# zjc263/GPU_SDR

Measured on AMD Instinct MI355X. Metric: IQ Msamples/s ingested (one synthetic 200 Msps stream per GPU), higher is better.
Workload: dtype f32 (f16 hi/lo-split MFMA, f32 accumulate)

## Files before the change

### gpu_sdr_amd/csrc/ddc_kernels.h

```cpp
#pragma once
#include <hip/hip_runtime.h>

#include <vector>

#include "dev_owner.h"

#ifndef GSDR_NO_PK
#define GSDR_NO_PK __attribute__((target("no-packed-fp32-ops")))
#endif

namespace gsdr {

struct Switches {
    bool ddc_mfma = true;
    bool ddc_few = true;
    bool ddc_pipe = true;
    int ddc_k = -1;
    int ddc_waves = 0;
    int ddc_nch = 0;
    unsigned ddc_lds = 0;
    int ddc_prefetch = 1;
    bool ddc_autotune = true;
    int mfma_asm = 4;
    int mfma_tt = 1;
    int mfma_pk = 32;
    int mfma_w = 4;
    int mfma_rt = 0;
    bool mfma_w8 = true;
    int mfma_prec = -1;
    int mfma_3m = -1;
    int mfma_3m_rot = -1;
    int mfma_fold = -1;
    int mfma_timing = 0;
    bool noise_fft = true;
    bool tones_fft = true;
    bool pfb_lds = true;
    int pfb_bluestein = -1;
    int pfb_cu = -1;
    bool pfb_direct = true;
    int pfb_col = -1;
    int pfb_cu_nt = 0;
    bool pfb_teams = true;
    bool pfb_radix8 = true;
    int pfb_fr = 0;
    int pfb_wide = -1;
    int mix_few = 32;
    bool chirp_split = true;
    bool pipe_queues = true;
    bool pipe_overlap = true;
    int pipe_streams = 3;
};
Switches read_switches();

struct DdcShape {
    int N;
    int Npad;
    int TW;
    int M;
    int nblk;
    int nch;
    int cbase, crem;
    int g_off;
    unsigned rate;
    unsigned long long idx0;
    unsigned long long rate_magic;
    double inv_rate;
    unsigned m_mod_rate;
    long long total;
    long long xlast;
    int prefetch;
};

struct DdcLaunch {
    const float2 *x;
    const float *taps_t;
    const float *taps_p;
    const float2 *btab;
    const double2 *wk;
    const double2 *wrem;
    const unsigned *fmod;
    float2 *out;
    float2 *tails;
    int tails_nch;
    const float2 *carry_in;
    float2 *carry_out;
    DdcShape sh;
    unsigned lds_bytes;
    bool pipe;
    bool few;
};

hipError_t launch_ddc(int F, int K, const DdcLaunch &a, hipStream_t st, hipEvent_t stop);
const char *ddc_few_kernel_name();
hipError_t launch_mix(int K, const DdcLaunch &a, int mix_few, hipStream_t st);

hipError_t launch_ddc_flat_main(int F, int PK, const DdcLaunch &a, hipStream_t st);
const char *ddc_kernel_name();
const char *ddc_flat_kernel_name();
const char *mix_kernel_name(int n_tones, int tw, long long total, int K, int mix_few);
hipError_t launch_widen_sc16(const void *in, float2 *out, long long n, float scale, int cus, hipStream_t st);
hipError_t launch_narrow_sc16(const float2 *in, void *out, long long n, float gain, unsigned long long *clipped, int cus,
                              hipStream_t st);

struct MfmaShape {
    int N;
    int NT32;
    int ntg;
    int ntq;
    int ngt;
    int M;
    int MF;
    int F;
    int nk8;
    int nout;
    int woff;
    int carry_len;
    long long tail0;
    long long nx;
    unsigned rate;
    unsigned long long rate_magic;
    double inv_rate;
    unsigned m_mod_rate;
    unsigned idx_base;
    int seg_k;
    float unscale;
    int rt;
    int timing_mode;
};

struct MfmaLaunch {
    const float2 *x;
    const float2 *head;
    const float2 *tail;
    const float *taps;
    const uint4 *bfrag;
    const float2 *ptab;
    const float2 *dtab;
    const unsigned *fmod;
    const unsigned *segmax;
    float2 *out;
    const uint4 *img;
    const uint4 *bfrag3;
    const float4 *ptab3;
    MfmaShape sh;
};

struct MfmaPlan {
    int TT, PK;
    int ntg, nk8, MF, M;
    unsigned rate;
    bool x16;
};

void mfma_build_tables(const MfmaPlan &pl, const std::vector<unsigned> &fmod_in, const float *window,
                       std::vector<uint4> &bfrag, std::vector<float2> &ptab,
                       std::vector<float2> &dtab, std::vector<float> &taps,
                       std::vector<unsigned> &fmod, float &unscale);
void mfma_build_tables3(const MfmaPlan &pl, int span, const std::vector<unsigned> &fmod, std::vector<uint4> &bfrag3,
                        std::vector<float4> &ptab3);
void mfma_build_tables3f(const MfmaPlan &pl, const std::vector<unsigned> &fmod, std::vector<uint4> &bfrag3,
                         std::vector<float4> &ptab3);
struct StageLaunch {
    const float2 *x;
    long long n;
    const float2 *b;
    long long nb;
    float2 *b_dst;
    unsigned *seg, *seg_clear;
    int nseg_alloc;
    long long seg_len;
    float2 *head_cur;
    long long head_n;
    float2 *head_next;
    int carry_len;
    float2 *tail;
    long long tail0;
};
hipError_t launch_absmax(const StageLaunch &s, hipStream_t st);
enum class MfmaKernel { AsmRing, Cxx, AsmRing16, AsmRing16W8, AsmRing16P, AsmRing16P3, AsmRing16P3R2, AsmRing16P3F };
hipError_t launch_ddc_mfma(MfmaKernel kind, int TT, int PK, int W, const MfmaLaunch &a, hipStream_t st);
const char *ddc_mfma_kernel_name(MfmaKernel kind);

struct FftPlan {
    int n = 0;
    int m = 0;
    int n_radices = 0;
    int radices[32] = {};
    DevBuf<float2> d_tw;
    DevBuf<float2> d_chirp;
    DevBuf<float2> d_bhat;
};
int fft_plan_build(FftPlan &pl, int n);
hipError_t fft_forward(const FftPlan &pl, float2 *src, float2 *dst, float2 *tmp, int batch, hipStream_t st);
hipError_t launch_pfb_filter(const float2 *raw, const float *window, int nfft, int avg, int frames_n, float2 *frames,
                             hipStream_t st);
hipError_t launch_pfb_select(const float2 *spectra, int nfft, int frames_n, const int *sel, int n_out, float2 *out, hipStream_t st);
hipError_t launch_pfb_average(const float2 *frames, long long n_frames, int n_ch, int k, int kind, int count, const float2 *acc_in,
                              float2 *acc_out, float2 *out, hipStream_t st);
const char *fft_kernel_name();
constexpr int kPfbLdsMaxN = 8192;
constexpr int kPfbLdsMaxPrime = 127;
constexpr int kPfbLdsTwMaxN = 4096;
constexpr int kPfbLdsMaxBytes = (2 * kPfbLdsMaxN + kPfbLdsMaxPrime + 1) * 8;
int pfb_lds_plan(int n, int *radices16, bool radix8);
hipError_t launch_pfb_lds(const float2 *carry, int new_0, const float2 *in, const float *window, const float2 *tw,
                          int nfft, int avg, int frames_n, const int *sel, int n_out, float2 *out,
                          float2 *carry_out, int spare_begin, int spare_n, long long window_len, hipStream_t st,
                          const FftPlan *blue, const Switches &sw, const char **kernel);
bool pfb_cu_fits(int nfft, int avg, int len, const Switches &sw);
struct PfbChoice {
    bool cu;
    int threads;
    int G;
    int twl;
    size_t lds;
    int b_off, b_len, col, direct, dir_s, dir_gs, teams;
};
PfbChoice pfb_choose(int nfft, int avg, const FftPlan *blue, int frames_n, int n_out, int cus, const Switches &sw);
const char *pfb_kernel_name(const PfbChoice &c);

struct ChirpShape {
    unsigned long long num_steps, length, period;
    unsigned chirpness;
    int f0;
};

hipError_t launch_chirp_demod(const float2 *in, float2 *out, long long n,
                              unsigned long long index0, const ChirpShape &cs, hipStream_t st);
hipError_t launch_chirp_lockin(const float2 *carry, int carry_len, const float2 *in,
                               const float *profile, int ppt, int valid, float2 *out,
                               unsigned long long index0, const ChirpShape &cs, hipStream_t st,
                               bool split, float2 *partial, int partial_cap);
hipError_t launch_warm(hipStream_t st);
hipError_t launch_tones_synth(float2 *out, long long n, unsigned long long start, unsigned rate, const unsigned *fmod,
                              const float2 *q0, const float2 *btab, const float2 *ctab, int n_tones, hipStream_t st);
hipError_t launch_tones_synth_sc16(void *out, long long n, unsigned long long start, unsigned rate, const unsigned *fmod,
                                   const float2 *q0, const float2 *btab, const float2 *ctab, int n_tones, float gain,
                                   unsigned long long *clipped, hipStream_t st);
const char *chirp_demod_kernel_name();
const char *chirp_lockin_kernel_name();

hipError_t launch_source_tones(float2 *out, long long n, long long start, unsigned rate,
                               const unsigned *fmod_dev, const float *ampl_dev,
                               const float *phase_dev, int n_tones, float sigma,
                               unsigned long long seed, hipStream_t st);
hipError_t launch_source_chirp(float2 *out, long long n, unsigned long long index0,
                               const ChirpShape &cs, float scale, hipStream_t st);
hipError_t launch_source_chirp_sc16(void *out, long long n, unsigned long long index0, const ChirpShape &cs, float scale,
                                    float gain, unsigned long long *clipped, hipStream_t st);

}
```

### gpu_sdr_amd/csrc/ddc_mfma.hip

```cpp
#include <cmath>
#include <cstdlib>
#include <type_traits>
#include <vector>

#include "ddc_device.h"
#include "ddc_mfma_ring_gen.h"
#include "ddc_mfma_ring16_gen.h"
#include "ddc_mfma_ring16w8_gen.h"
#include "ddc_mfma_ring16p_gen.h"
#include "ddc_mfma_ring16p3_gen.h"
#include "ddc_mfma_ring16p3r2_gen.h"
#include "ddc_mfma_ring16p3f_gen.h"

namespace gsdr {

typedef _Float16 half2v __attribute__((ext_vector_type(2)));
typedef _Float16 half4v __attribute__((ext_vector_type(4)));
typedef _Float16 half8 __attribute__((ext_vector_type(8)));
typedef float float2v __attribute__((ext_vector_type(2)));
typedef float float4u __attribute__((ext_vector_type(4), aligned(8)));
typedef float float4v __attribute__((ext_vector_type(4)));
typedef float float16v __attribute__((ext_vector_type(16)));

namespace {

struct Frag {
    half8 hi, lo;
};

__device__ __forceinline__ float mul_legacy(float x, float h) {
    float r;
    asm("v_mul_legacy_f32 %0, %1, %2" : "=v"(r) : "v"(x), "v"(h));
    return r;
}

__device__ __forceinline__ void split_pair(float xr, float xi, float hs, half2v &hi, half2v &lo) {
#pragma clang fp contract(off)
    const float2v v = {mul_legacy(xr, hs), mul_legacy(xi, hs)};
    hi = __builtin_convertvector(v, half2v);
    const float2v res = v - __builtin_convertvector(hi, float2v);
    lo = __builtin_convertvector(res, half2v);
}

__device__ __forceinline__ Frag make_frag(const float4v xa, const float4v xb, const float4v hs) {
    half2v h0, h1, h2, h3, l0, l1, l2, l3;
    split_pair(xa.x, xa.y, hs.x, h0, l0);
    split_pair(xa.z, xa.w, hs.y, h1, l1);
    split_pair(xb.x, xb.y, hs.z, h2, l2);
    split_pair(xb.z, xb.w, hs.w, h3, l3);
    Frag f;
    const half4v ha = __builtin_shufflevector(h0, h1, 0, 1, 2, 3);
    const half4v hb = __builtin_shufflevector(h2, h3, 0, 1, 2, 3);
    const half4v la = __builtin_shufflevector(l0, l1, 0, 1, 2, 3);
    const half4v lb = __builtin_shufflevector(l2, l3, 0, 1, 2, 3);
    f.hi = __builtin_shufflevector(ha, hb, 0, 1, 2, 3, 4, 5, 6, 7);
    f.lo = __builtin_shufflevector(la, lb, 0, 1, 2, 3, 4, 5, 6, 7);
    return f;
}

}

__device__ __forceinline__ float bits_to_float(unsigned u) { return __builtin_bit_cast(float, u); }
__device__ __forceinline__ unsigned float_to_bits(float f) { return __builtin_bit_cast(unsigned, f); }
__device__ __forceinline__ void workgroup_sync() {
    __builtin_amdgcn_fence(__ATOMIC_RELEASE, "workgroup");
    __builtin_amdgcn_s_barrier();
    __builtin_amdgcn_fence(__ATOMIC_ACQUIRE, "workgroup");
}
__device__ __forceinline__ unsigned lane_xor(unsigned v, int d) {
    const int lane = (int)__builtin_amdgcn_mbcnt_hi(~0u, __builtin_amdgcn_mbcnt_lo(~0u, 0u));
    return (unsigned)__builtin_amdgcn_ds_bpermute((lane ^ d) << 2, (int)v);
}

__device__ __forceinline__ unsigned fresh_tid() {
    unsigned tid = threadIdx.x;
    asm volatile("" : "+v"(tid));
    return tid;
}
#define GSDR_SGPR(v) "s"(__builtin_amdgcn_readfirstlane((int)(v)))
#define GSDR_SGPR_PAIR(name, v) [name##_lo] GSDR_SGPR((unsigned)(v)), [name##_hi] GSDR_SGPR((unsigned)((v) >> 32))

#ifdef GSDR_TIMING_BUILD
__device__ __forceinline__ bool timing_no_stores(const MfmaShape &sh) { return (sh.timing_mode & 1) != 0; }
__device__ __forceinline__ bool timing_one_block(const MfmaShape &sh) { return (sh.timing_mode & 2) != 0; }
#else
__device__ __forceinline__ bool timing_no_stores(const MfmaShape &) { return false; }
__device__ __forceinline__ bool timing_one_block(const MfmaShape &) { return false; }
#endif

#ifdef GSDR_STAMP_BUILD
__device__ unsigned long long *g_stamp_buf = nullptr;
__device__ __forceinline__ void stamp(int slot) {
    if (g_stamp_buf && threadIdx.x == 0) {
        unsigned long long t = __builtin_amdgcn_s_memrealtime();
        if (slot == 2) {
            unsigned xcc, hwid;
            asm volatile("s_getreg_b32 %0, hwreg(HW_REG_XCC_ID)" : "=s"(xcc));
            asm volatile("s_getreg_b32 %0, hwreg(HW_REG_HW_ID)" : "=s"(hwid));
            t = (xcc & 0xfu) | ((unsigned long long)hwid << 8);
        }
        g_stamp_buf[8 * (size_t)blockIdx.x + slot] = t;
    }
}
#else
__device__ __forceinline__ void stamp(int) {}
#endif

__device__ __forceinline__ unsigned wave_max_u32(unsigned v) {
    int x = (int)v;
#define GSDR_DPP_MAX(ctrl, row_mask)                                                          \
    {                                                                                         \
        const unsigned o = (unsigned)__builtin_amdgcn_update_dpp(0, x, ctrl, row_mask, 0xf, false); \
        x = (int)((unsigned)x > o ? (unsigned)x : o);                                         \
    }
    GSDR_DPP_MAX(0xB1, 0xf);
    GSDR_DPP_MAX(0x4E, 0xf);
    GSDR_DPP_MAX(0x141, 0xf);
    GSDR_DPP_MAX(0x140, 0xf);
    GSDR_DPP_MAX(0x142, 0xa);
    GSDR_DPP_MAX(0x143, 0xc);
#undef GSDR_DPP_MAX
    return (unsigned)__builtin_amdgcn_readlane(x, 63);
}

__device__ __forceinline__ void row_segments(const MfmaShape &sh, int o, int &q0, int &q1) {
    const int oc = o < sh.nout ? o : sh.nout - 1;
    q0 = oc;
    q1 = oc + sh.F - 1;
    if (sh.seg_k > 1) {
        q0 /= sh.seg_k;
        q1 /= sh.seg_k;
    }
}
__device__ __forceinline__ unsigned row_max_bits(const MfmaLaunch &a, int o) {
    int q0, q1;
    row_segments(a.sh, o, q0, q1);
    const int span = q1 - q0;
    unsigned v[8];
#pragma unroll
    for (int i = 0; i < 8; ++i) v[i] = a.segmax[q0 + (i < span ? i : span)];
    unsigned m = 0;
#pragma unroll
    for (int i = 0; i < 8; ++i) m = m > v[i] ? m : v[i];
    return m;
}
__device__ __forceinline__ int scale_exp_of(unsigned m) {
    int se = 140 - (int)((m >> 23) & 0xffu);
    return se > 100 ? 100 : (se < -100 ? -100 : se);
}
__device__ __forceinline__ int row_scale_exp(const MfmaLaunch &a, int o) { return scale_exp_of(row_max_bits(a, o)); }
constexpr int kScaleFromTable = 0x7fffffff;
__device__ __forceinline__ float exp2_bits(int e) { return __builtin_bit_cast(float, (unsigned)(127 + e) << 23); }

__device__ __forceinline__ float2 tile_phasor(const MfmaLaunch &a, int gt, unsigned fm) {
    const MfmaShape &sh = a.sh;
    const unsigned long long s_tile = mod_rate(
        (unsigned long long)sh.idx_base + (unsigned long long)(gt * 32) * sh.m_mod_rate, sh.rate, sh.rate_magic);
    const unsigned long long ph = mod_rate((unsigned long long)fm * s_tile, sh.rate, sh.rate_magic);
    double bre, bim;
    exact_phasor(ph, sh.inv_rate, bre, bim);
    return make_float2((float)bre, (float)bim);
}

__device__ __forceinline__ void store_tile(const MfmaLaunch &a, int gt, int n, int hh, int se_self,
                                           const float16v &accr, const float16v &acci) {
    const MfmaShape &sh = a.sh;
    const int Np = sh.NT32 * 32;
    const unsigned fm = a.fmod[n];
    float2 d[16];
#pragma unroll
    for (int i = 0; i < 16; ++i) d[i] = a.dtab[(size_t)((i & 3) + 8 * (i >> 2) + 4 * hh) * Np + n];
    asm volatile("" ::: "memory");
    const float2 base = tile_phasor(a, gt, fm);
#pragma unroll
    for (int i = 0; i < 16; ++i) {
        const int row = (i & 3) + 8 * (i >> 2) + 4 * hh;
        const int se = __builtin_amdgcn_ds_bpermute(row << 2, se_self);
        const float inv = exp2_bits(-se) * sh.unscale;
        const float dx = d[i].x * inv, dy = d[i].y * inv;
        const float rr = base.x * dx - base.y * dy, ri = base.x * dy + base.y * dx;
        float2 y;
        y.x = accr[i] * rr - acci[i] * ri;
        y.y = accr[i] * ri + acci[i] * rr;
        const int orow = gt * 32 + row;
        if (orow < sh.nout && n < sh.N) a.out[(size_t)orow * sh.N + n] = y;
    }
}

template <int TT>
__device__ __forceinline__ void store_rows(const MfmaLaunch &a, int gt, int n0, int hh, int se_self,
                                           const float16v (&accr)[TT], const float16v (&acci)[TT]) {
#pragma unroll
    for (int tt = 0; tt < TT; ++tt) {
        const int n = n0 + tt * 32;
        store_tile(a, gt, n, hh, se_self, accr[tt], acci[tt]);
    }
}

__device__ __forceinline__ void wg_barrier() {
    asm volatile("s_waitcnt lgkmcnt(0)\n\ts_barrier" ::: "memory");
}

template <int TT, int PK, int W>
__global__ __launch_bounds__(64 * W, TT == 1 ? 2 : 1) void ddc_mfma_kernel(const MfmaLaunch a) {
    constexpr int KS = PK / 8;
    constexpr int SPW = KS / W;
    static_assert(KS % W == 0 && SPW >= 1, "every wave produces whole k-steps");
    __shared__ uint4 ring[2][KS][2][64];
    const MfmaShape &sh = a.sh;
    const int lane = threadIdx.x & 63;
    const int wave = __builtin_amdgcn_readfirstlane((int)(threadIdx.x >> 6));
    const int r = lane & 31, hh = lane >> 5;
    const int xcd = blockIdx.x & 7, q = blockIdx.x >> 3;
    const int gt = (q / sh.ntq) * 8 + xcd;
    if (gt >= sh.ngt) return;
    const int tg_raw = (q % sh.ntq) * W + wave;
    const bool active = tg_raw < sh.ntg;
    const int tg = active ? tg_raw : sh.ntg - 1;

    half8 Bf[TT][KS][2][2];
#pragma unroll
    for (int tt = 0; tt < TT; ++tt)
#pragma unroll
        for (int ks = 0; ks < KS; ++ks)
#pragma unroll
            for (int c = 0; c < 2; ++c)
#pragma unroll
                for (int sp = 0; sp < 2; ++sp) {
                    const size_t at = ((((size_t)(tg * TT + tt) * KS + ks) * 2 + c) * 2 + sp) * 64 + lane;
                    const uint4 v = a.bfrag[at];
                    Bf[tt][ks][c][sp] = __builtin_bit_cast(half8, v);
                }

    const int o = gt * 32 + r;
    const int se = row_scale_exp(a, o);
    const float S = exp2_bits(se);
    const int oc = o < sh.nout ? o : sh.nout - 1;
    const float2 *xbase = gt == 0 ? a.head + sh.carry_len
                                  : (gt == sh.ngt - 1 ? a.tail - sh.tail0 : a.x);
    const float2 *xrow = xbase + ((long long)(oc + sh.woff) * sh.M + 4 * hh);
    const float *tp = a.taps + 4 * hh;

    const int nhi = (sh.nk8 + KS - 1) / KS;
    float4v xa[SPW], xb[SPW], hv[SPW];
    auto gload = [&](int blk) {
        const int bc = blk < nhi ? blk : nhi - 1;
#pragma unroll
        for (int j = 0; j < SPW; ++j) {
            const int k = bc * KS + wave + j * W;
            hv[j] = *reinterpret_cast<const float4v *>(tp + 8 * k);
            const float4u *p = reinterpret_cast<const float4u *>(xrow + 8 * k);
            xa[j] = p[0];
            xb[j] = p[1];
        }
    };
    auto produce = [&](int slot) {
#pragma unroll
        for (int j = 0; j < SPW; ++j) {
            const int ks = wave + j * W;
            const Frag f = make_frag(xa[j], xb[j], hv[j] * S);
            ring[slot][ks][0][lane] = __builtin_bit_cast(uint4, f.hi);
            ring[slot][ks][1][lane] = __builtin_bit_cast(uint4, f.lo);
        }
    };

    float16v accr[TT], acci[TT];
#pragma unroll
    for (int tt = 0; tt < TT; ++tt)
#pragma unroll
        for (int i = 0; i < 16; ++i) accr[tt][i] = acci[tt][i] = 0.f;

    const int Np = sh.NT32 * 32;
    const int n0 = tg * TT * 32 + r;
    const float2 *pp = a.ptab + n0;

    gload(0);
    produce(0);
    gload(1);
    for (int hi = 0; hi < nhi; ++hi) {
        const int slot = hi & 1;
        wg_barrier();
        half8 fh[KS], fl[KS];
#pragma unroll
        for (int ks = 0; ks < KS; ++ks) {
            fh[ks] = __builtin_bit_cast(half8, ring[slot][ks][0][lane]);
            fl[ks] = __builtin_bit_cast(half8, ring[slot][ks][1][lane]);
        }
        float2 P[TT];
#pragma unroll
        for (int tt = 0; tt < TT; ++tt) P[tt] = pp[(size_t)hi * Np + tt * 32];
        produce(slot ^ 1);
        gload(hi + 2);
        __builtin_amdgcn_sched_barrier(0);
        float16v Cr[TT], Ci[TT];
#pragma unroll
        for (int ks = 0; ks < KS; ++ks) {
            const float16v zero = {0};
#pragma unroll
            for (int tt = 0; tt < TT; ++tt) {
                float16v cr = ks == 0 ? zero : Cr[tt], ci = ks == 0 ? zero : Ci[tt];
                cr = __builtin_amdgcn_mfma_f32_32x32x16_f16(fh[ks], Bf[tt][ks][0][0], cr, 0, 0, 0);
                ci = __builtin_amdgcn_mfma_f32_32x32x16_f16(fh[ks], Bf[tt][ks][1][0], ci, 0, 0, 0);
                cr = __builtin_amdgcn_mfma_f32_32x32x16_f16(fh[ks], Bf[tt][ks][0][1], cr, 0, 0, 0);
                ci = __builtin_amdgcn_mfma_f32_32x32x16_f16(fh[ks], Bf[tt][ks][1][1], ci, 0, 0, 0);
                cr = __builtin_amdgcn_mfma_f32_32x32x16_f16(fl[ks], Bf[tt][ks][0][0], cr, 0, 0, 0);
                ci = __builtin_amdgcn_mfma_f32_32x32x16_f16(fl[ks], Bf[tt][ks][1][0], ci, 0, 0, 0);
                Cr[tt] = cr;
                Ci[tt] = ci;
            }
        }
        __builtin_amdgcn_sched_barrier(0);
        asm volatile("s_nop 15\n\ts_nop 15");
        __builtin_amdgcn_sched_barrier(0);
#pragma unroll
        for (int tt = 0; tt < TT; ++tt)
// ... 204 lines not shown
                 :
                 : [xo] "v"(xo), [to] "v"(to), [po] "v"(po), [bo] "v"(bo), [lane16] "v"(rd16), [wr16] "v"(wr16),
                   [accaddr] "v"(accaddr), GSDR_SGPR_PAIR(xb, xb), GSDR_SGPR_PAIR(tp, tpb), GSDR_SGPR_PAIR(pp, ppb),
                   GSDR_SGPR_PAIR(bf, bfb), [pstride] GSDR_SGPR((unsigned)Np * 8u), [nhi] GSDR_SGPR(nhi),
                   [first] GSDR_SGPR(first), [sgo] "v"(sgo), [sgn] "v"(sgn), [seaddr] "v"(seaddr),
                   GSDR_SGPR_PAIR(sg, sgb)
                 : GSDR_MFMA_RING16_CLOBBERS);
    stamp(3);
    if (active && !timing_no_stores(sh)) {
        const unsigned tid2 = fresh_tid();
        const int lane2 = (int)(tid2 & 63u);
        ring16_epilogue(a, lds, gt, tg, wave, lane2, (int)(lds_scale[tid2] >> 23) - 127);
    }
}

__global__ __launch_bounds__(256, 2) __attribute__((target("no-packed-fp32-ops"))) void ddc_mfma_ring16_kernel(
    const MfmaLaunch a) {
    constexpr int W = 4;
    __shared__ uint4 lds[2048];
    __shared__ unsigned lds_scale[256];
    static_assert(sizeof(uint4) * 2048 >= GSDR_MFMA_RING16_BYTES, "ring fits");
    const MfmaShape &sh = a.sh;
    const int wave = __builtin_amdgcn_readfirstlane((int)(threadIdx.x >> 6));
    const int xcd = blockIdx.x & 7, q = blockIdx.x >> 3;
    const int rt = sh.rt > 1 ? 2 : 1;
    const int gt0 = (q / sh.ntq) * rt * 8 + xcd;
    if (gt0 >= sh.ngt) return;
    const int tg_raw = (q % sh.ntq) * W + wave;
    const bool active = tg_raw < sh.ntg;
    const int tg = active ? tg_raw : sh.ntg - 1;
    stamp(0);
    stamp(2);
    ring16_tile(a, lds, lds_scale, gt0, 1, tg, wave, active);
    if (rt > 1 && gt0 + 8 < sh.ngt) {
        workgroup_sync();
        ring16_tile(a, lds, lds_scale, gt0 + 8, 0, tg, wave, active);
    }
    stamp(1);
}

#ifdef GSDR_STAMP_BUILD
extern "C" int gsdr_debug_set_stamp_buffer(void *dev_ptr) {
    unsigned long long *p = (unsigned long long *)dev_ptr;
    return hipMemcpyToSymbol(HIP_SYMBOL(g_stamp_buf), &p, sizeof(p)) == hipSuccess ? 0 : -1;
}
#endif

__global__ __launch_bounds__(512, 2) __attribute__((target("no-packed-fp32-ops"))) void ddc_mfma_ring16w8_kernel(
    const MfmaLaunch a) {
    constexpr int KS = 4, W = 8;
    __shared__ uint4 lds[4096];
    __shared__ unsigned lds_scale[512];
    static_assert(sizeof(uint4) * 4096 >= GSDR_MFMA_RING16W8_BYTES, "ring fits");
    const MfmaShape &sh = a.sh;
    const int wave = __builtin_amdgcn_readfirstlane((int)(threadIdx.x >> 6));
    const int ntq8 = (sh.ntg + W - 1) / W;
    const int xcd = blockIdx.x & 7, q = blockIdx.x >> 3;
    const int gt = (q / ntq8) * 8 + xcd;
    if (gt >= sh.ngt) return;
    stamp(0);
    stamp(2);
    const int tg_raw = (q % ntq8) * W + wave;
    const bool active = tg_raw < sh.ntg;
    const int tg = active ? tg_raw : sh.ntg - 1;
    const int Np = sh.NT32 * 32;
    const int nhi = timing_one_block(sh) ? 1 : (sh.nk8 + KS - 1) / KS;
    const unsigned tid = fresh_tid();
    const int lane = (int)(tid & 63u);
    const int r = lane & 31, hh = lane >> 5;
    const int kw = wave & 3;
    int q0, q1;
    row_segments(sh, gt * 32 + r, q0, q1);
    const unsigned sgo = (unsigned)q0 * 4u, sgn = (unsigned)(q1 - q0);
    const unsigned long long sgb = (unsigned long long)a.segmax;
    const unsigned seaddr = (unsigned)(unsigned long long)(__attribute__((address_space(3))) char *)lds_scale + tid * 4u;
    const unsigned to = (unsigned)((4 * hh + 8 * kw) * 4);
    const unsigned po = (unsigned)(tg * 32 + (lane & 15)) * 8u;
    const unsigned bo = (unsigned)tg * (KS * 4 * 1024u) + (unsigned)lane * 16u;
    const unsigned lds_base = (unsigned)(unsigned long long)(__attribute__((address_space(3))) char *)lds;
    const unsigned rd16 = lds_base + (unsigned)(lane >> 5) * 2048u + (unsigned)(lane & 15) * 16u +
                          (unsigned)((lane >> 4) & 1) * 512u;
    const unsigned wr16 = lds_base + (unsigned)lane * 16u + (unsigned)kw * 2048u;
    const unsigned accaddr = lds_base + (unsigned)wave * 8192u + (unsigned)lane * 16u;
    const unsigned long long tpb = (unsigned long long)a.taps, ppb = (unsigned long long)a.ptab,
                             bfb = (unsigned long long)a.bfrag;
    const int o = gt * 32 + r;
    const int oc = o < sh.nout ? o : sh.nout - 1;
    const float2 *xbase;
    long long xshift;
    if (gt == 0) {
        xbase = a.head;
        xshift = sh.carry_len;
    } else if (gt == sh.ngt - 1) {
        xbase = a.tail;
        xshift = -sh.tail0;
    } else {
        xbase = a.x;
        xshift = 0;
    }
    const unsigned xo = (unsigned)((((long long)(oc + sh.woff) * sh.M + xshift) + 4 * hh + 8 * kw) * 8);
    const unsigned long long xb = (unsigned long long)xbase;
    asm volatile(GSDR_MFMA_RING16W8_TEXT
                 :
                 : [xo] "v"(xo), [to] "v"(to), [po] "v"(po), [bo] "v"(bo), [lane16] "v"(rd16), [wr16] "v"(wr16),
                   [accaddr] "v"(accaddr), GSDR_SGPR_PAIR(xb, xb), GSDR_SGPR_PAIR(tp, tpb), GSDR_SGPR_PAIR(pp, ppb),
                   GSDR_SGPR_PAIR(bf, bfb), [pstride] GSDR_SGPR((unsigned)Np * 8u), [nhi] GSDR_SGPR(nhi),
                   [role] GSDR_SGPR(wave >> 2), [sgo] "v"(sgo), [sgn] "v"(sgn), [seaddr] "v"(seaddr),
                   GSDR_SGPR_PAIR(sg, sgb)
                 : GSDR_MFMA_RING16W8_CLOBBERS);
    if (active && !timing_no_stores(sh)) {
        const unsigned tid2 = fresh_tid();
        const int lane2 = (int)(tid2 & 63u);
        const int se_self = (int)(lds_scale[tid2] >> 23) - 127;
        float16v accr, acci;
        const float4v *acc = reinterpret_cast<const float4v *>(lds) + wave * 512 + lane2;
#pragma unroll
        for (int qd = 0; qd < 4; ++qd) {
            const float4v vr = acc[qd * 64], vi = acc[(qd + 4) * 64];
#pragma unroll
            for (int j = 0; j < 4; ++j) {
                accr[qd * 4 + j] = vr[j];
                acci[qd * 4 + j] = vi[j];
            }
        }
        store_tile16(a, gt, tg, lane2, se_self, accr, acci);
    }
    stamp(1);
}

__global__ __launch_bounds__(256) __attribute__((target("no-packed-fp32-ops"))) void ddc_convert_kernel(const MfmaLaunch a, uint4 *__restrict__ img, int nhi) {
    const MfmaShape &sh = a.sh;
    const int lane = threadIdx.x & 63, wave = threadIdx.x >> 6;
    const int r = lane & 31, hh = lane >> 5;
    const int gt = blockIdx.x / nhi, blk = blockIdx.x - gt * nhi;
    const int o = gt * 32 + r;
    const float S = exp2_bits(row_scale_exp(a, o));
    const int oc = o < sh.nout ? o : sh.nout - 1;
    const float2 *xbase = gt == 0 ? a.head + sh.carry_len : (gt == sh.ngt - 1 ? a.tail - sh.tail0 : a.x);
    const int k = blk * 4 + wave;
    const float4u *px = reinterpret_cast<const float4u *>(xbase + ((long long)(oc + sh.woff) * sh.M + 4 * hh + 8 * k));
    const float4v xa = px[0], xb = px[1];
    const float4v hv = *reinterpret_cast<const float4v *>(a.taps + 8 * k + 4 * hh);
    const Frag f = make_frag(xa, xb, hv * S);
    uint4 *dst = img + ((size_t)blockIdx.x * 8 + 2 * wave) * 64 + lane;
    dst[0] = __builtin_bit_cast(uint4, f.hi);
    dst[64] = __builtin_bit_cast(uint4, f.lo);
}

__device__ __forceinline__ __attribute__((target("no-packed-fp32-ops"))) void ring16p_tile(
    const MfmaLaunch &a, uint4 *lds, int gt, int first, int tg, int wave, bool active) {
    constexpr int KS = 4;
    const MfmaShape &sh = a.sh;
    const int Np = sh.NT32 * 32;
    const int nhi = (sh.nk8 + KS - 1) / KS;
    const int lane = (int)(fresh_tid() & 63u);
    const unsigned po = (unsigned)(tg * 32 + (lane & 15)) * 8u;
    const unsigned bo = (unsigned)tg * (KS * 4 * 1024u) + (unsigned)lane * 16u;
    const unsigned lds_base = (unsigned)(unsigned long long)(__attribute__((address_space(3))) char *)lds;
    const unsigned rd16 = lds_base + (unsigned)(lane >> 5) * 2048u + (unsigned)(lane & 15) * 16u +
                          (unsigned)((lane >> 4) & 1) * 512u;
    const unsigned io_hi = (unsigned)wave * 2048u + (unsigned)lane * 16u, io_lo = io_hi + 1024u;
    const unsigned wrs = lds_base + (unsigned)wave * 2048u;
    const unsigned accaddr = lds_base + (unsigned)wave * 8192u + (unsigned)lane * 16u;
    const unsigned long long ibb = (unsigned long long)(a.img + (size_t)gt * nhi * 512), ppb = (unsigned long long)a.ptab,
                             bfb = (unsigned long long)a.bfrag;
    asm volatile(GSDR_MFMA_RING16P_TEXT
                 :
                 : [io_hi] "v"(io_hi), [io_lo] "v"(io_lo), [po] "v"(po), [bo] "v"(bo), [lane16] "v"(rd16),
                   [accaddr] "v"(accaddr), GSDR_SGPR_PAIR(ib, ibb), [wrs] GSDR_SGPR(wrs), GSDR_SGPR_PAIR(pp, ppb),
                   GSDR_SGPR_PAIR(bf, bfb), [pstride] GSDR_SGPR((unsigned)Np * 8u), [nhi] GSDR_SGPR(nhi),
                   [first] GSDR_SGPR(first)
                 : GSDR_MFMA_RING16P_CLOBBERS);
    if (active) ring16_epilogue(a, lds, gt, tg, wave, (int)(fresh_tid() & 63u), kScaleFromTable);
}

__global__ __launch_bounds__(256, 2) __attribute__((target("no-packed-fp32-ops"))) void ddc_mfma_ring16p_kernel(
    const MfmaLaunch a) {
    constexpr int W = 4;
    __shared__ uint4 lds[2048];
    static_assert(sizeof(uint4) * 2048 >= GSDR_MFMA_RING16P_BYTES, "ring fits");
    const MfmaShape &sh = a.sh;
    const int wave = __builtin_amdgcn_readfirstlane((int)(threadIdx.x >> 6));
    const int xcd = blockIdx.x & 7, q = blockIdx.x >> 3;
    const int gt0 = (q / sh.ntq) * 8 + xcd;
    if (gt0 >= sh.ngt) return;
    const int tg_raw = (q % sh.ntq) * W + wave;
    const bool active = tg_raw < sh.ntg;
    const int tg = active ? tg_raw : sh.ntg - 1;
    ring16p_tile(a, lds, gt0, 1, tg, wave, active);
}

__device__ __forceinline__ void split_one(float v, _Float16 &hi, _Float16 &lo) {
#pragma clang fp contract(off)
    hi = (_Float16)v;
    lo = (_Float16)(v - (float)hi);
}

__global__ __launch_bounds__(128) __attribute__((target("no-packed-fp32-ops"))) void ddc_convert3_kernel(const MfmaLaunch a, uint4 *__restrict__ img, int nhi) {
    const MfmaShape &sh = a.sh;
    const int l = threadIdx.x & 63, rh = threadIdx.x >> 6;
    const int r = 16 * rh + (l & 15), g = l >> 4;
    const int gt = blockIdx.x / nhi, blk = blockIdx.x - gt * nhi;
    const int o = gt * 32 + r;
    const float S = exp2_bits(row_scale_exp(a, o));
    const int oc = o < sh.nout ? o : sh.nout - 1;
    const float2 *xbase = gt == 0 ? a.head + sh.carry_len : (gt == sh.ngt - 1 ? a.tail - sh.tail0 : a.x);
    const int k0 = blk * 32 + 8 * g;
    const float4u *px = reinterpret_cast<const float4u *>(xbase + ((long long)(oc + sh.woff) * sh.M + k0));
    const float4v x0 = px[0], x1 = px[1], x2 = px[2], x3 = px[3];
    const float4v h0 = *reinterpret_cast<const float4v *>(a.taps + k0) * S;
    const float4v h1 = *reinterpret_cast<const float4v *>(a.taps + k0 + 4) * S;
    const float xr[8] = {x0.x, x0.z, x1.x, x1.z, x2.x, x2.z, x3.x, x3.z};
    const float xi[8] = {x0.y, x0.w, x1.y, x1.w, x2.y, x2.w, x3.y, x3.w};
    const float hs[8] = {h0.x, h0.y, h0.z, h0.w, h1.x, h1.y, h1.z, h1.w};
    half8 hi[3], lo[3];
#pragma unroll
    for (int j = 0; j < 8; ++j) {
#pragma clang fp contract(off)
        const float pa = mul_legacy(xr[j], hs[j]), pb = mul_legacy(xi[j], hs[j]);
        const float ps = pa + pb;
        _Float16 h, w;
        split_one(ps, h, w);
        hi[0][j] = h;
        lo[0][j] = w;
        split_one(pa, h, w);
        hi[1][j] = h;
        lo[1][j] = w;
        split_one(pb, h, w);
        hi[2][j] = h;
        lo[2][j] = w;
    }
    uint4 *dst = img + (size_t)blockIdx.x * (GSDR_MFMA_RING16P3_SLOT / 16) + rh * 64 + l;
#pragma unroll
    for (int c = 0; c < 3; ++c) {
        dst[(4 * c) * 64] = __builtin_bit_cast(uint4, hi[c]);
        dst[(4 * c + 2) * 64] = __builtin_bit_cast(uint4, lo[c]);
    }
}

static_assert(GSDR_MFMA_RING16P3R2_SLOT == GSDR_MFMA_RING16P3_SLOT, "one image format for both three-product loops");

template <bool kPairs>
__device__ __forceinline__ __attribute__((target("no-packed-fp32-ops"))) void ring16p3_tile(
    const MfmaLaunch &a, uint4 *lds, int gt, int tg, int wave, bool active) {
    constexpr int KS = 4;
    constexpr unsigned kImages = kPairs ? 24 : 12;
    const MfmaShape &sh = a.sh;
    const int Np = sh.NT32 * 32;
    const int nhi = (sh.nk8 + KS - 1) / KS;
    const int lane = (int)(fresh_tid() & 63u);
    const unsigned po = (unsigned)(tg * 32 + (lane & 15)) * 16u;
    const unsigned bo = (unsigned)tg * (kImages * 1024u) + (unsigned)lane * 16u;
    const unsigned lds_base = (unsigned)(unsigned long long)(__attribute__((address_space(3))) char *)lds;
    const unsigned rd16 = lds_base + (unsigned)lane * 16u;
    const unsigned io0 = (unsigned)wave * 3072u + (unsigned)lane * 16u, io1 = io0 + 1024u, io2 = io0 + 2048u;
    const unsigned wrs = lds_base + (unsigned)wave * 3072u;
    const unsigned accaddr = lds_base + (unsigned)wave * 8192u + (unsigned)lane * 16u;
    const unsigned long long ibb = (unsigned long long)(a.img + (size_t)gt * nhi * (GSDR_MFMA_RING16P3_SLOT / 16)),
                             ppb = (unsigned long long)a.ptab3, bfb = (unsigned long long)a.bfrag3;
#define GSDR_RING16P3_OPERANDS                                                                                     \
    [io0] "v"(io0), [io1] "v"(io1), [io2] "v"(io2), [po] "v"(po), [bo] "v"(bo), [lane16] "v"(rd16),                \
        [accaddr] "v"(accaddr), GSDR_SGPR_PAIR(ib, ibb), [wrs] GSDR_SGPR(wrs), GSDR_SGPR_PAIR(pp, ppb),            \
        GSDR_SGPR_PAIR(bf, bfb), [pstride] GSDR_SGPR((unsigned)Np * 16u), [nhi] GSDR_SGPR(nhi)
    if constexpr (kPairs)
        asm volatile(GSDR_MFMA_RING16P3R2_TEXT : : GSDR_RING16P3_OPERANDS : GSDR_MFMA_RING16P3R2_CLOBBERS);
    else
        asm volatile(GSDR_MFMA_RING16P3_TEXT : : GSDR_RING16P3_OPERANDS : GSDR_MFMA_RING16P3_CLOBBERS);
#undef GSDR_RING16P3_OPERANDS
    if (active) ring16_epilogue(a, lds, gt, tg, wave, (int)(fresh_tid() & 63u), kScaleFromTable);
}

__global__ __launch_bounds__(256, 2) __attribute__((target("no-packed-fp32-ops"))) void ddc_mfma_ring16p3_kernel(
    const MfmaLaunch a) {
    constexpr int W = 4;
    __shared__ uint4 lds[GSDR_MFMA_RING16P3_BYTES / 16];
    static_assert(GSDR_MFMA_RING16P3_BYTES >= 4 * 8192, "the accumulators fit");
    const MfmaShape &sh = a.sh;
    const int wave = __builtin_amdgcn_readfirstlane((int)(threadIdx.x >> 6));
    const int xcd = blockIdx.x & 7, q = blockIdx.x >> 3;
    const int gt0 = (q / sh.ntq) * 8 + xcd;
    if (gt0 >= sh.ngt) return;
    const int tg_raw = (q % sh.ntq) * W + wave;
    const bool active = tg_raw < sh.ntg;
    const int tg = active ? tg_raw : sh.ntg - 1;
    ring16p3_tile<false>(a, lds, gt0, tg, wave, active);
}

__global__ __launch_bounds__(256, 2) __attribute__((target("no-packed-fp32-ops"))) void ddc_mfma_ring16p3r2_kernel(
    const MfmaLaunch a) {
    constexpr int W = 4;
    __shared__ uint4 lds[GSDR_MFMA_RING16P3R2_BYTES / 16];
    static_assert(GSDR_MFMA_RING16P3R2_BYTES >= 4 * 8192, "the accumulators fit");
    const MfmaShape &sh = a.sh;
    const int wave = __builtin_amdgcn_readfirstlane((int)(threadIdx.x >> 6));
    const int xcd = blockIdx.x & 7, q = blockIdx.x >> 3;
    const int gt0 = (q / sh.ntq) * 8 + xcd;
    if (gt0 >= sh.ngt) return;
    const int tg_raw = (q % sh.ntq) * W + wave;
    const bool active = tg_raw < sh.ntg;
    const int tg = active ? tg_raw : sh.ntg - 1;
    ring16p3_tile<true>(a, lds, gt0, tg, wave, active);
}

__global__ __launch_bounds__(128) __attribute__((target("no-packed-fp32-ops"))) void ddc_convert3f_kernel(const MfmaLaunch a, uint4 *__restrict__ img, int nhi, int nspan) {
    const MfmaShape &sh = a.sh;
    const int l = threadIdx.x & 63, rh = threadIdx.x >> 6;
    const int r = 16 * rh + (l & 15), g = l >> 4;
    const int gt = blockIdx.x / nspan, sp = blockIdx.x - gt * nspan;
    const int o = gt * 32 + r;
    const float S = exp2_bits(row_scale_exp(a, o));
    const int oc = o < sh.nout ? o : sh.nout - 1;
    const float2 *xbase = gt == 0 ? a.head + sh.carry_len : (gt == sh.ngt - 1 ? a.tail - sh.tail0 : a.x);
    const float2 *xrow = xbase + (long long)(oc + sh.woff) * sh.M;
    const int k0 = sp * 64 + 8 * g;
    const int k1 = sp * 64 + 56 - 8 * g;
    const bool whole = 2 * sp + 1 < nhi;
    const float4u *px = reinterpret_cast<const float4u *>(xrow + k0);
    const float4v x0 = px[0], x1 = px[1], x2 = px[2], x3 = px[3];
    const float4v h0 = *reinterpret_cast<const float4v *>(a.taps + k0) * S;
    const float4v h1 = *reinterpret_cast<const float4v *>(a.taps + k0 + 4) * S;
    const float4v zero = {0.f, 0.f, 0.f, 0.f};
    float4v y0 = zero, y1 = zero, y2 = zero, y3 = zero, g0 = zero, g1 = zero;
    if (whole) {
        const float4u *py = reinterpret_cast<const float4u *>(xrow + k1);
        y0 = py[0], y1 = py[1], y2 = py[2], y3 = py[3];
        g0 = *reinterpret_cast<const float4v *>(a.taps + k1) * S;
        g1 = *reinterpret_cast<const float4v *>(a.taps + k1 + 4) * S;
    }
    const float xr[8] = {x0.x, x0.z, x1.x, x1.z, x2.x, x2.z, x3.x, x3.z};
    const float xi[8] = {x0.y, x0.w, x1.y, x1.w, x2.y, x2.w, x3.y, x3.w};
    const float hs[8] = {h0.x, h0.y, h0.z, h0.w, h1.x, h1.y, h1.z, h1.w};
    const float yr[8] = {y0.x, y0.z, y1.x, y1.z, y2.x, y2.z, y3.x, y3.z};
    const float yi[8] = {y0.y, y0.w, y1.y, y1.w, y2.y, y2.w, y3.y, y3.w};
    const float gs[8] = {g0.x, g0.y, g0.z, g0.w, g1.x, g1.y, g1.z, g1.w};
    half8 hi[4], lo[4];
#pragma unroll
    for (int j = 0; j < 8; ++j) {
#pragma clang fp contract(off)
        const float pa = mul_legacy(xr[j], hs[j]), pb = mul_legacy(xi[j], hs[j]);
        const float qa = whole ? mul_legacy(yr[7 - j], gs[7 - j]) : 0.f, qb = whole ? mul_legacy(yi[7 - j], gs[7 - j]) : 0.f;
        const float u[4] = {pa + qa, pb - qb, pa + pb, qa + qb};
#pragma unroll
        for (int c = 0; c < 4; ++c) {
            _Float16 h, w;
            split_one(u[c], h, w);
            hi[c][j] = h;
            lo[c][j] = w;
        }
    }
    uint4 *dst = img + (size_t)blockIdx.x * (GSDR_MFMA_RING16P3F_SLOT / 16) + rh * 64 + l;
#pragma unroll
    for (int c = 0; c < 4; ++c) {
        dst[(4 * c) * 64] = __builtin_bit_cast(uint4, hi[c]);
        dst[(4 * c + 2) * 64] = __builtin_bit_cast(uint4, lo[c]);
    }
}

__device__ __forceinline__ __attribute__((target("no-packed-fp32-ops"))) void ring16p3f_tile(
    const MfmaLaunch &a, uint4 *lds, int gt, int tg, int wave, bool active) {
    const MfmaShape &sh = a.sh;
    const int Np = sh.NT32 * 32;
    const int nspan = ((sh.nk8 + 3) / 4 + 1) / 2;
    const int lane = (int)(fresh_tid() & 63u);
    const unsigned po = (unsigned)(tg * 32 + (lane & 15)) * 16u;
    const unsigned bo = (unsigned)tg * (16u * 1024u) + (unsigned)lane * 16u;
    const unsigned lds_base = (unsigned)(unsigned long long)(__attribute__((address_space(3))) char *)lds;
    const unsigned rd16 = lds_base + (unsigned)lane * 16u;
    const unsigned io0 = (unsigned)wave * 4096u + (unsigned)lane * 16u, io1 = io0 + 1024u, io2 = io0 + 2048u, io3 = io0 + 3072u;
    const unsigned wrs = lds_base + (unsigned)wave * 4096u;
    const unsigned accaddr = lds_base + (unsigned)wave * 8192u + (unsigned)lane * 16u;
    const unsigned long long ibb = (unsigned long long)(a.img + (size_t)gt * nspan * (GSDR_MFMA_RING16P3F_SLOT / 16)),
                             ppb = (unsigned long long)a.ptab3, bfb = (unsigned long long)a.bfrag3;
    asm volatile(GSDR_MFMA_RING16P3F_TEXT
                 :
                 : [io0] "v"(io0), [io1] "v"(io1), [io2] "v"(io2), [io3] "v"(io3), [po] "v"(po), [bo] "v"(bo),
                   [lane16] "v"(rd16), [accaddr] "v"(accaddr), GSDR_SGPR_PAIR(ib, ibb), [wrs] GSDR_SGPR(wrs),
                   GSDR_SGPR_PAIR(pp, ppb), GSDR_SGPR_PAIR(bf, bfb), [pstride] GSDR_SGPR((unsigned)Np * 16u),
                   [nhi] GSDR_SGPR(nspan)
                 : GSDR_MFMA_RING16P3F_CLOBBERS);
    if (active) ring16_epilogue(a, lds, gt, tg, wave, (int)(fresh_tid() & 63u), kScaleFromTable);
}

__global__ __launch_bounds__(256, 2) __attribute__((target("no-packed-fp32-ops"))) void ddc_mfma_ring16p3f_kernel(
    const MfmaLaunch a) {
    constexpr int W = 4;
    __shared__ uint4 lds[GSDR_MFMA_RING16P3F_BYTES / 16];
    static_assert(GSDR_MFMA_RING16P3F_BYTES >= 4 * 8192, "the accumulators fit");
    static_assert(2 * GSDR_MFMA_RING16P3F_BYTES <= 160 * 1024, "two workgroups per compute unit");
    const MfmaShape &sh = a.sh;
    const int wave = __builtin_amdgcn_readfirstlane((int)(threadIdx.x >> 6));
    const int xcd = blockIdx.x & 7, q = blockIdx.x >> 3;
    const int gt0 = (q / sh.ntq) * 8 + xcd;
    if (gt0 >= sh.ngt) return;
    const int tg_raw = (q % sh.ntq) * W + wave;
    const bool active = tg_raw < sh.ntg;
    const int tg = active ? tg_raw : sh.ntg - 1;
    ring16p3f_tile(a, lds, gt0, tg, wave, active);
}

constexpr int kStageChunk = 2048;
constexpr int kStageSlots = kStageChunk / 64 + 3;
struct StageShape {
    unsigned seg_len;
    unsigned seg_magic;
    unsigned main_blocks;
};

__device__ __forceinline__ unsigned finite_bits(float v) {
    const unsigned b = __builtin_bit_cast(unsigned, v) & 0x7fffffffu;
    return b < 0x7f800000u ? b : 0u;
}

__global__ __launch_bounds__(256) void absmax_kernel(const StageLaunch s, const StageShape g) {
    constexpr int kStageCopies = 8;
    __shared__ unsigned slot[kStageSlots * kStageCopies];
    for (long long i = (long long)blockIdx.x * 256 + threadIdx.x; i < s.nseg_alloc; i += (long long)gridDim.x * 256)
        s.seg_clear[i] = 0u;
    for (int i = threadIdx.x; i < kStageSlots * kStageCopies; i += 256) slot[i] = 0u;
    const bool region_a = blockIdx.x < g.main_blocks;
    const float2 *src = region_a ? s.x : s.b;
    const long long cnt = region_a ? s.n : s.nb;
    const long long tbase = region_a ? s.nb : 0;
    const long long c0 = (long long)(region_a ? blockIdx.x : blockIdx.x - g.main_blocks) * kStageChunk;
    const long long c1 = c0 + kStageChunk < cnt ? c0 + kStageChunk : cnt;
    const int lane = threadIdx.x & 63, wave = threadIdx.x >> 6;
    const unsigned long long t0 = (unsigned long long)(tbase + c0);
    const unsigned seg0 = (unsigned)(t0 / g.seg_len);
    const unsigned rem0 = (unsigned)(t0 - (unsigned long long)seg0 * g.seg_len);
    const bool copies = region_a ? ((s.head_cur && c0 < s.head_n) || (s.head_next && c1 > s.n - s.carry_len) ||
                                    (s.tail && c1 > s.tail0))
                                 : s.b_dst != nullptr;
    __syncthreads();
    const long long w0 = c0 + 512 * wave;
    float4u v[4];
#pragma unroll
    for (int k = 0; k < 4; ++k) {
        const long long i = w0 + 2 * lane + 128 * k;
        if (i + 1 < c1) {
            v[k] = *reinterpret_cast<const float4u *>(src + i);
        } else if (i < c1) {
            const float2 w = src[i];
            v[k] = float4u{w.x, w.y, 0.f, 0.f};
        } else {
            v[k] = float4u{0.f, 0.f, 0.f, 0.f};
        }
    }
    const bool long_segments = g.seg_len >= 512u;
    unsigned m_lo = 0, m_hi = 0;
    const unsigned wrem = rem0 + 512u * (unsigned)wave;
#pragma unroll
    for (int k = 0; k < 4; ++k) {
        const long long i = w0 + 2 * lane + 128 * k;
        const unsigned b0 = finite_bits(v[k].x), b1 = finite_bits(v[k].y), b2 = finite_bits(v[k].z), b3 = finite_bits(v[k].w);
        const unsigned ma = b0 > b1 ? b0 : b1, mb = b2 > b3 ? b2 : b3;
        const unsigned oa = wrem + 2u * (unsigned)lane + 128u * (unsigned)k, ob = oa + 1u;
        if (long_segments) {
            const unsigned first = wrem / g.seg_len;
            const unsigned edge = (first + 1u) * g.seg_len;
            if (oa < edge) m_lo = m_lo > ma ? m_lo : ma; else m_hi = m_hi > ma ? m_hi : ma;
            if (ob < edge) m_lo = m_lo > mb ? m_lo : mb; else m_hi = m_hi > mb ? m_hi : mb;
        } else {
            if (ma) atomicMax(&slot[__umulhi(oa, g.seg_magic) * kStageCopies + (lane & (kStageCopies - 1))], ma);
            if (mb) atomicMax(&slot[__umulhi(ob, g.seg_magic) * kStageCopies + (lane & (kStageCopies - 1))], mb);
        }
        if (copies) {
#pragma unroll
            for (int e = 0; e < 2; ++e) {
                const long long ie = i + e;
                if (ie < c1) {
                    const float2 w2 = e ? make_float2(v[k].z, v[k].w) : make_float2(v[k].x, v[k].y);
                    if (region_a) {
                        if (s.head_cur && ie < s.head_n) s.head_cur[s.carry_len + ie] = w2;
                        if (s.head_next && ie >= s.n - s.carry_len) s.head_next[ie - (s.n - s.carry_len)] = w2;
                        if (s.tail && ie >= s.tail0) s.tail[ie - s.tail0] = w2;
                    } else {
                        s.b_dst[ie] = w2;
                    }
                }
            }
        }
    }
    if (long_segments) {
        const unsigned first = wrem / g.seg_len;
        m_lo = wave_max_u32(m_lo);
        m_hi = wave_max_u32(m_hi);
        if (lane == 0) {
            if (m_lo) atomicMax(&slot[first * kStageCopies], m_lo);
            if (m_hi) atomicMax(&slot[(first + 1u) * kStageCopies], m_hi);
        }
    }
    __syncthreads();
    if (threadIdx.x < kStageSlots) {
        unsigned m = 0;
#pragma unroll
        for (int c = 0; c < kStageCopies; ++c) {
            const unsigned t = slot[threadIdx.x * kStageCopies + c];
            m = m > t ? m : t;
        }
        if (m) atomicMax(&s.seg[seg0 + threadIdx.x], m);
    }
}

namespace {

unsigned short to_half_bits(float v) {
    const _Float16 h = (_Float16)v;
    unsigned short b;
    __builtin_memcpy(&b, &h, 2);
    return b;
}
float from_half_bits(unsigned short b) {
    _Float16 h;
    __builtin_memcpy(&h, &b, 2);
    return (float)h;
}

void host_phasor(unsigned long long ph, unsigned rate, double &re, double &im) {
    const double ang = 2.0 * M_PI * ((double)ph / (double)rate);
    re = std::cos(ang);
    im = -std::sin(ang);
}

unsigned ring_grid(int ngt, int cols, int rt) {
    const int gt8 = ((ngt + 7) / 8 + rt - 1) / rt;
    const long long grid = (long long)gt8 * 8 * cols;
    return grid < 1 || grid > 0x7fffffffLL ? 0u : (unsigned)grid;
}

template <int TT, int PK, int W>
hipError_t launch_tpw(const MfmaLaunch &a, hipStream_t st) {
    const unsigned grid = ring_grid(a.sh.ngt, a.sh.ntq, 1);
    if (!grid) return hipErrorInvalidValue;
    hipLaunchKernelGGL((ddc_mfma_kernel<TT, PK, W>), dim3(grid), dim3(64 * W), 0, st, a);
    return hipGetLastError();
}

template <int TT, int PK>
hipError_t launch_tp(int W, const MfmaLaunch &a, hipStream_t st) {
    switch (W) {
        case 2: return launch_tpw<TT, PK, 2>(a, st);
        case 4: if constexpr (PK >= 32) return launch_tpw<TT, PK, 4>(a, st);
        default: return hipErrorInvalidValue;
    }
}

}

void mfma_build_tables(const MfmaPlan &pl, const std::vector<unsigned> &fmod_in, const float *window,
                       std::vector<uint4> &bfrag, std::vector<float2> &ptab,
                       std::vector<float2> &dtab, std::vector<float> &taps,
                       std::vector<unsigned> &fmod, float &unscale) {
    const int KS = pl.PK / 8;
    const int tiles = pl.ntg * pl.TT, Np = tiles * 32;
    const unsigned rate = pl.rate;
    fmod.assign(Np, 0u);
    for (size_t n = 0; n < fmod_in.size() && n < (size_t)Np; ++n) fmod[n] = fmod_in[n];
    bfrag.assign((size_t)tiles * KS * 4 * 64, uint4{0, 0, 0, 0});
    if (pl.x16) {
        for (int T = 0; T < tiles; ++T)
            for (int k2 = 0; k2 < 2; ++k2)
                for (int th = 0; th < 2; ++th)
                    for (int lane = 0; lane < 64; ++lane) {
                        const unsigned long long fm = fmod[(size_t)T * 32 + 16 * th + (lane & 15)];
                        unsigned short img[2][2][8];
                        for (int j = 0; j < 8; ++j) {
                            const int lo = 16 * k2 + 4 * (lane >> 4) + (j >> 1);
                            double wr, wi;
                            host_phasor((fm * (unsigned long long)lo) % rate, rate, wr, wi);
                            const float v[2] = {(j & 1) ? (float)-wi : (float)wr, (j & 1) ? (float)wr : (float)wi};
                            for (int c = 0; c < 2; ++c) {
                                const unsigned short hb = to_half_bits(v[c]);
                                img[c][0][j] = hb;
                                img[c][1][j] = to_half_bits(v[c] - from_half_bits(hb));
                            }
                        }
                        for (int c = 0; c < 2; ++c)
                            for (int sp = 0; sp < 2; ++sp) {
                                uint4 w;
                                __builtin_memcpy(&w, img[c][sp], 16);
                                const int f = ((k2 * 2 + th) * 2 + c) * 2 + sp;
                                bfrag[((size_t)T * 16 + f) * 64 + lane] = w;
                            }
                    }
    } else
    for (int T = 0; T < tiles; ++T)
        for (int ks = 0; ks < KS; ++ks)
            for (int lane = 0; lane < 64; ++lane) {
                const int r = lane & 31, hh = lane >> 5;
                const unsigned long long fm = fmod[(size_t)T * 32 + r];
                unsigned short img[2][2][8];
                for (int j = 0; j < 8; ++j) {
                    const int lo = 8 * ks + 4 * hh + (j >> 1);
                    double wr, wi;
                    host_phasor((fm * (unsigned long long)lo) % rate, rate, wr, wi);
                    const float v[2] = {(j & 1) ? (float)-wi : (float)wr, (j & 1) ? (float)wr : (float)wi};
                    for (int c = 0; c < 2; ++c) {
                        const unsigned short hb = to_half_bits(v[c]);
                        img[c][0][j] = hb;
                        img[c][1][j] = to_half_bits(v[c] - from_half_bits(hb));
                    }
                }
                for (int c = 0; c < 2; ++c)
                    for (int sp = 0; sp < 2; ++sp) {
                        uint4 w;
                        __builtin_memcpy(&w, img[c][sp], 16);
                        bfrag[((((size_t)T * KS + ks) * 2 + c) * 2 + sp) * 64 + lane] = w;
                    }
            }
    const int nhi = (pl.nk8 + KS - 1) / KS;
    ptab.resize((size_t)nhi * Np);
    for (int hi = 0; hi < nhi; ++hi)
        for (int n = 0; n < Np; ++n) {
            double re, im;
            host_phasor(((unsigned long long)fmod[n] * (((unsigned long long)hi * pl.PK) % rate)) % rate, rate, re, im);
            ptab[(size_t)hi * Np + n] = make_float2((float)re, (float)im);
        }
    dtab.resize((size_t)32 * Np);
    for (int row = 0; row < 32; ++row)
        for (int n = 0; n < Np; ++n) {
            double re, im;
            host_phasor(((unsigned long long)fmod[n] * (((unsigned long long)row * pl.M) % rate)) % rate, rate, re, im);
            dtab[(size_t)row * Np + n] = make_float2((float)re, (float)im);
        }
    float hmax = 0.f;
    for (int t = 0; t < pl.MF; ++t) hmax = std::fmax(hmax, std::fabs(window[t]));
    int eh = 0;
    if (hmax > 0.f) {
        (void)std::frexp(hmax, &eh);
    }
    unscale = std::ldexp(1.f, eh);
    taps.assign((size_t)nhi * pl.PK + 8, 0.f);
    for (int t = 0; t < pl.MF; ++t) taps[t] = std::ldexp(window[t], -eh);
}

void mfma_build_tables3(const MfmaPlan &pl, int span, const std::vector<unsigned> &fmod, std::vector<uint4> &bfrag3,
                        std::vector<float4> &ptab3) {
    const int tiles = pl.ntg * pl.TT, Np = tiles * 32;
    const unsigned rate = pl.rate;
    const int nimg = 12 * span;
    bfrag3.assign((size_t)tiles * nimg * 64, uint4{0, 0, 0, 0});
    for (int T = 0; T < tiles; ++T)
        for (int half = 0; half < span; ++half)
            for (int th = 0; th < 2; ++th)
                for (int lane = 0; lane < 64; ++lane) {
                    const unsigned long long fm = fmod[(size_t)T * 32 + 16 * th + (lane & 15)];
                    unsigned short img[3][2][8];
                    for (int j = 0; j < 8; ++j) {
                        const int lo = 32 * half + 8 * (lane >> 4) + j;
                        double wr, wi;
                        host_phasor((fm * (unsigned long long)lo) % rate, rate, wr, wi);
                        const float v[3] = {(float)wr, (float)(wi - wr), (float)(wr + wi)};
                        for (int c = 0; c < 3; ++c) {
                            const unsigned short hb = to_half_bits(v[c]);
                            img[c][0][j] = hb;
                            img[c][1][j] = to_half_bits(v[c] - from_half_bits(hb));
                        }
                    }
                    for (int c = 0; c < 3; ++c)
                        for (int sp = 0; sp < 2; ++sp) {
                            uint4 w;
                            __builtin_memcpy(&w, img[c][sp], 16);
                            const int f = half * 12 + (c * 2 + th) * 2 + sp;
                            bfrag3[((size_t)T * nimg + f) * 64 + lane] = w;
                        }
                }
    const int nrow = ((pl.nk8 + 3) / 4 + span - 1) / span;
    ptab3.assign((size_t)(nrow + 1) * Np, make_float4(0.f, 0.f, 0.f, 0.f));
    for (int row = 0; row < nrow; ++row)
        for (int n = 0; n < Np; ++n) {
            double re, im;
            host_phasor(((unsigned long long)fmod[n] * (((unsigned long long)row * 32 * span) % rate)) % rate, rate, re, im);
            ptab3[(size_t)row * Np + n] = make_float4((float)re, (float)im, (float)(re - im), (float)(re + im));
        }
}

void mfma_build_tables3f(const MfmaPlan &pl, const std::vector<unsigned> &fmod, std::vector<uint4> &bfrag3,
                         std::vector<float4> &ptab3) {
    const int tiles = pl.ntg * pl.TT, Np = tiles * 32;
    const unsigned long long rate2 = 2ULL * pl.rate;
    auto half_phasor = [&](unsigned long long ph2, double &re, double &im) {
        const double ang = M_PI * ((double)ph2 / (double)pl.rate);
        re = std::cos(ang);
        im = -std::sin(ang);
    };
    bfrag3.assign((size_t)tiles * 16 * 64, uint4{0, 0, 0, 0});
    for (int T = 0; T < tiles; ++T)
        for (int th = 0; th < 2; ++th)
            for (int lane = 0; lane < 64; ++lane) {
                const unsigned long long fm = fmod[(size_t)T * 32 + 16 * th + (lane & 15)];
                unsigned short img[4][2][8];
                for (int jj = 0; jj < 8; ++jj) {
                    const int j = 8 * (lane >> 4) + jj;
                    double wr, wi;
                    half_phasor((fm * (unsigned long long)(63 - 2 * j)) % rate2, wr, wi);
                    const double c = wr, d = -wi;
                    const float v[4] = {(float)c, (float)d, (float)(c + d), (float)(c - d)};
                    for (int u = 0; u < 4; ++u) {
                        const unsigned short hb = to_half_bits(v[u]);
                        img[u][0][jj] = hb;
                        img[u][1][jj] = to_half_bits(v[u] - from_half_bits(hb));
                    }
                }
                for (int u = 0; u < 4; ++u)
                    for (int sp = 0; sp < 2; ++sp) {
                        uint4 w;
                        __builtin_memcpy(&w, img[u][sp], 16);
                        bfrag3[((size_t)T * 16 + (u * 2 + th) * 2 + sp) * 64 + lane] = w;
                    }
            }
    const int nrow = ((pl.nk8 + 3) / 4 + 1) / 2;
    ptab3.assign((size_t)(nrow + 1) * Np, make_float4(0.f, 0.f, 0.f, 0.f));
    for (int row = 0; row < nrow; ++row)
        for (int n = 0; n < Np; ++n) {
            const unsigned long long t2 = (128ULL * (unsigned long long)row + 63ULL) % rate2;
            double re, im;
            half_phasor((unsigned long long)(((unsigned __int128)fmod[n] * t2) % rate2), re, im);
            ptab3[(size_t)row * Np + n] = make_float4((float)re, (float)im, (float)(im - re), (float)(re + im));
        }
}

hipError_t launch_absmax(const StageLaunch &s, hipStream_t st) {
    if (!s.x || s.n < 1 || s.nb < 0 || (s.nb > 0 && !s.b) || s.carry_len < 0 || s.carry_len > s.n || s.head_n < 0 ||
        s.head_n > s.n || s.tail0 < 0 || s.tail0 > s.n || !s.seg || !s.seg_clear || s.seg_len < 64 ||
        s.seg_len > 0x7fffffffLL || s.nseg_alloc < 1)
        return hipErrorInvalidValue;
    const long long nseg = (s.nb + s.n + s.seg_len - 1) / s.seg_len;
    if (nseg > s.nseg_alloc) return hipErrorInvalidValue;
    StageShape g{};
    g.seg_len = (unsigned)s.seg_len;
    g.seg_magic = (unsigned)(0x100000000ULL / (unsigned long long)s.seg_len + 1ULL);
    const long long ba = (s.n + kStageChunk - 1) / kStageChunk, bb = (s.nb + kStageChunk - 1) / kStageChunk;
    if (ba + bb > 0x7fffffffLL) return hipErrorInvalidValue;
    g.main_blocks = (unsigned)ba;
    hipLaunchKernelGGL(absmax_kernel, dim3((unsigned)(ba + bb)), dim3(256), 0, st, s, g);
    return hipGetLastError();
}

hipError_t launch_ddc_mfma(MfmaKernel kind, int TT, int PK, int W, const MfmaLaunch &a, hipStream_t st) {
    const MfmaShape &sh = a.sh;
    if (sh.N < 1 || sh.nout < 1 || sh.M < 1 || sh.MF < 1 || sh.nk8 != (sh.MF + 7) / 8 ||
        sh.ngt != (sh.nout + 31) / 32 || sh.ntg < 1 || W < 1 || sh.ntq != (sh.ntg + W - 1) / W ||
        sh.NT32 != sh.ntg * TT || sh.N > sh.NT32 * 32 || sh.rate < 1 ||
        (long long)(sh.nout - 1 + sh.woff) * sh.M + sh.MF > sh.nx ||
        (long long)sh.woff * sh.M + sh.carry_len < 0 || (sh.woff < 0 && -sh.woff > 32) ||
        !a.x || !a.head || !a.tail || !a.out || !a.bfrag || !a.ptab || !a.dtab || !a.taps ||
        !a.fmod || !a.segmax || sh.seg_k < 1 || sh.F < 1 || sh.F > 8 || sh.MF != sh.M * sh.F)
        return hipErrorInvalidValue;
    const long long reach = (long long)((sh.nk8 + PK / 8 - 1) / (PK / 8)) * PK;
    if (a.x != a.tail && sh.ngt > 2 && (long long)(32 * (sh.ngt - 1) - 1 + sh.woff) * sh.M + reach > sh.nx)
        return hipErrorInvalidValue;
    if (sh.ngt > 1 && (long long)(32 * (sh.ngt - 1) + sh.woff) * sh.M < sh.tail0) return hipErrorInvalidValue;
    if (kind == MfmaKernel::Cxx) {
        if (TT == 2 && PK == 32) return launch_tp<2, 32>(W, a, st);
        if (TT == 1 && PK == 32) return launch_tp<1, 32>(W, a, st);
        if (TT == 2 && PK == 16) return launch_tp<2, 16>(W, a, st);
        if (TT == 1 && PK == 16) return launch_tp<1, 16>(W, a, st);
        return hipErrorInvalidValue;
    }
    if (TT != 1 || PK != 32 || W != 4) return hipErrorInvalidValue;
    unsigned grid = 0;
    switch (kind) {
        case MfmaKernel::AsmRing16P:
        case MfmaKernel::AsmRing16P3:
        case MfmaKernel::AsmRing16P3R2: {
            const bool three = kind != MfmaKernel::AsmRing16P;
            if (!a.img || (three && (!a.bfrag3 || !a.ptab3))) return hipErrorInvalidValue;
            const int nhi = (sh.nk8 + 3) / 4;
            const long long cgrid = (long long)sh.ngt * nhi;
            grid = ring_grid(sh.ngt, sh.ntq, 1);
            if (cgrid < 1 || cgrid > 0x7fffffffLL || !grid) return hipErrorInvalidValue;
            uint4 *img = const_cast<uint4 *>(a.img);
            if (three)
                hipLaunchKernelGGL(ddc_convert3_kernel, dim3((unsigned)cgrid), dim3(128), 0, st, a, img, nhi);
            else
                hipLaunchKernelGGL(ddc_convert_kernel, dim3((unsigned)cgrid), dim3(256), 0, st, a, img, nhi);
            const hipError_t e = hipGetLastError();
            if (e != hipSuccess) return e;
            if (kind == MfmaKernel::AsmRing16P3R2)
                hipLaunchKernelGGL(ddc_mfma_ring16p3r2_kernel, dim3(grid), dim3(256), 0, st, a);
            else if (three)
                hipLaunchKernelGGL(ddc_mfma_ring16p3_kernel, dim3(grid), dim3(256), 0, st, a);
            else
                hipLaunchKernelGGL(ddc_mfma_ring16p_kernel, dim3(grid), dim3(256), 0, st, a);
            return hipGetLastError();
        }
        case MfmaKernel::AsmRing16P3F: {
            if (!a.img || !a.bfrag3 || !a.ptab3) return hipErrorInvalidValue;
            const int nhi = (sh.nk8 + 3) / 4, nspan = (nhi + 1) / 2;
            const long long cgrid = (long long)sh.ngt * nspan;
            grid = ring_grid(sh.ngt, sh.ntq, 1);
            if (cgrid < 1 || cgrid > 0x7fffffffLL || !grid) return hipErrorInvalidValue;
            hipLaunchKernelGGL(ddc_convert3f_kernel, dim3((unsigned)cgrid), dim3(128), 0, st, a, const_cast<uint4 *>(a.img),
                               nhi, nspan);
            const hipError_t e = hipGetLastError();
            if (e != hipSuccess) return e;
            hipLaunchKernelGGL(ddc_mfma_ring16p3f_kernel, dim3(grid), dim3(256), 0, st, a);
            return hipGetLastError();
        }
        case MfmaKernel::AsmRing16W8:
            if (!(grid = ring_grid(sh.ngt, (sh.ntg + 7) / 8, 1))) return hipErrorInvalidValue;
            hipLaunchKernelGGL(ddc_mfma_ring16w8_kernel, dim3(grid), dim3(512), 0, st, a);
            return hipGetLastError();
        case MfmaKernel::AsmRing16:
        case MfmaKernel::AsmRing:
            if (sh.rt < 0 || sh.rt > 8 || !(grid = ring_grid(sh.ngt, sh.ntq, sh.rt > 1 ? sh.rt : 1)))
                return hipErrorInvalidValue;
            if (kind == MfmaKernel::AsmRing16)
                hipLaunchKernelGGL(ddc_mfma_ring16_kernel, dim3(grid), dim3(256), 0, st, a);
            else
                hipLaunchKernelGGL(ddc_mfma_ring_kernel, dim3(grid), dim3(256), 0, st, a);
            return hipGetLastError();
        default:
            return hipErrorInvalidValue;
    }
}

const char *ddc_mfma_kernel_name(MfmaKernel kind) {
    switch (kind) {
        case MfmaKernel::AsmRing16P:
        case MfmaKernel::AsmRing16P3:
        case MfmaKernel::AsmRing16P3R2:
        case MfmaKernel::AsmRing16P3F: return "ddc_mfma_ring16p_kernel";
        case MfmaKernel::AsmRing16W8: return "ddc_mfma_ring16w8_kernel";
        case MfmaKernel::AsmRing16: return "ddc_mfma_ring16_kernel";
        case MfmaKernel::AsmRing: return "ddc_mfma_ring_kernel";
        default: return "ddc_mfma_kernel";
    }
}

}
```

### gpu_sdr_amd/csrc/demod.cpp

```cpp
#include <hip/hip_runtime.h>

#include <cmath>
#include <cstdio>
#include <cstdlib>
#include <cstring>
#include <string>
#include <utility>
#include <vector>

#include <unistd.h>

#include "host_util.h"

extern char **environ;

using gsdr::ChirpShape;
using gsdr::chirp_shape;
using gsdr::create_error;
using gsdr::DdcLaunch;
using gsdr::DdcShape;
using gsdr::device_cus;
using gsdr::mod_rate;
using gsdr::phasor;

std::string &gsdr::create_error() {
    thread_local std::string msg;
    return msg;
}

namespace {

constexpr int kMaxF = 8;
constexpr int kMaxEvents = 8192;
constexpr int kPipeStreams = 3;
constexpr int kChirpPartials = 16384;
constexpr int kStageSets = kPipeStreams + 1;
constexpr int kScaleSlots = kPipeStreams + 2;

}

gsdr::Switches gsdr::read_switches() {
    auto is_set = [](const char *name) {
        const char *v = std::getenv(name);
        return v && *v ? v : nullptr;
    };
    auto env = [&](const char *name, int unset) {
        const char *v = is_set(name);
        return v ? std::atoi(v) : unset;
    };
    Switches s;
    s.ddc_mfma = env("GSDR_DDC_MFMA", 1) != 0;
    s.ddc_few = env("GSDR_DDC_FEW", 1) != 0;
    s.ddc_pipe = env("GSDR_DDC_PIPE", 1) != 0;
    s.ddc_k = env("GSDR_DDC_K", -1);
    s.ddc_waves = env("GSDR_DDC_WAVES_PER_SIMD", 0);
    if (s.ddc_waves <= 0 && is_set("GSDR_DDC_WAVES_PER_SIMD")) s.ddc_waves = 4;
    s.ddc_nch = env("GSDR_DDC_NCH", 0);
    s.ddc_lds = (unsigned)env("GSDR_DDC_LDS", 0);
    s.ddc_prefetch = env("GSDR_DDC_PREFETCH", 1);
    s.ddc_autotune = env("GSDR_DDC_AUTOTUNE", 1) != 0;
    s.mfma_asm = env("GSDR_MFMA_ASM", 4);
    s.mfma_tt = env("GSDR_MFMA_TT", 1) == 2 ? 2 : 1;
    s.mfma_pk = env("GSDR_MFMA_PK", 32) == 16 ? 16 : 32;
    s.mfma_w = env("GSDR_MFMA_W", 4) == 2 ? 2 : 4;
    s.mfma_rt = env("GSDR_MFMA_RT", 0);
    if (s.mfma_rt < 0 || s.mfma_rt > 2) s.mfma_rt = 0;
    s.mfma_w8 = env("GSDR_MFMA_W8", 1) != 0;
    s.mfma_prec = env("GSDR_MFMA_PREC", -1);
    s.mfma_3m = env("GSDR_MFMA_3M", -1);
    s.mfma_3m_rot = env("GSDR_MFMA_3M_ROT", -1);
    s.mfma_fold = env("GSDR_MFMA_FOLD", -1);
    s.mfma_timing = env("GSDR_MFMA_TIMING", 0);
    s.noise_fft = env("GSDR_NOISE_FFT", 1) != 0;
    s.tones_fft = env("GSDR_TONES_FFT", 1) != 0;
    s.pfb_lds = env("GSDR_PFB_LDS", 1) != 0;
    s.pfb_bluestein = is_set("GSDR_PFB_BLUESTEIN") ? env("GSDR_PFB_BLUESTEIN", 0) != 0 : -1;
    s.pfb_cu = env("GSDR_PFB_CU", -1);
    s.pfb_direct = env("GSDR_PFB_DIRECT", 1) != 0;
    s.pfb_col = env("GSDR_PFB_COL", -1);
    if (s.pfb_col > 0) s.pfb_col = 1;
    s.pfb_cu_nt = env("GSDR_PFB_CU_NT", 0);
    s.pfb_teams = env("GSDR_PFB_TEAMS", 1) != 0;
    s.pfb_radix8 = env("GSDR_PFB_RADIX8", 1) != 0;
    s.pfb_fr = env("GSDR_PFB_FR", 0);
    s.pfb_wide = env("GSDR_PFB_WIDE", -1);
    s.mix_few = env("GSDR_MIX_FEW", 32);
    s.chirp_split = env("GSDR_CHIRP_SPLIT", 1) != 0;
    s.pipe_queues = env("GSDR_PIPE_QUEUES", 1) != 0;
    s.pipe_overlap = env("GSDR_PIPE_OVERLAP", 1) != 0;
    s.pipe_streams = env("GSDR_PIPE_STREAMS", kPipeStreams);
    if (s.pipe_streams < 1 || s.pipe_streams > kPipeStreams) s.pipe_streams = kPipeStreams;
    return s;
}

struct gsdr_demod {
    gsdr::Switches sw;
    int mode = GSDR_NODSP;
    int device = -1;
    std::string err;
    gsdr::Stream stream;
    gsdr::Stream s_up, s_down;
    gsdr::Stream s_main[kPipeStreams];

    int N = 0;
    int ddc_channels = 0;
    long long L = 0;
    long long decim = 0;
    long long capacity = 0;
    float fcut = 0.f;

    gsdr::DevBuf<float2> d_in, d_out;
    float sc16_scale = 1.0f / 32768.0f;
    gsdr::DevBuf<gsdr_sc16> d_in16;
    gsdr::DevBuf<float2> d_wide;
    int cus = 256;
    struct Slot {
        gsdr::DevBuf<float2> d_in, d_out;
        gsdr::DevBuf<gsdr_sc16> d_in16;
        gsdr::Event up, done, down;
        hipEvent_t wait_ev = nullptr;
        int n = 0;
    } slot[GSDR_PIPELINE_DEPTH];
    bool pipe_ready = false;
    int pipe_head = 0, pipe_count = 0;

    int F = 0, K = 16, M = 0, Npad = 0, TW = 0, R = 0;
    unsigned nco_rate = 1;
    unsigned long long idx = 0;
    int target_waves = 4096;
    int simds = 1024;
    int nch_max = 1;
    int tails_nch = 0;
    double waves_ratio = 1.3;
    std::vector<float> window;
    gsdr::DevBuf<float> d_taps_t;
    gsdr::DevBuf<float> d_taps_p;
    bool pipe = false;
    int pad = 0;
    gsdr::DevBuf<float2> d_stage;
    gsdr::DevBuf<float2> d_btab;
    gsdr::DevBuf<double2> d_wk, d_wrem;
    gsdr::DevBuf<unsigned> d_fmod;
    gsdr::DevBuf<float2> d_tails;
    gsdr::DevBuf<float2> d_carry[2];
    int parity = 0;
    bool mfma = false;
    bool few = false;
    int mf_TT = 1, mf_PK = 32, mf_W = 4;
    gsdr::MfmaKernel mf_kind = gsdr::MfmaKernel::AsmRing;
    gsdr::MfmaShape mf{};
    int last_rt = 0;
    bool prec = false;
    gsdr::DevBuf<uint4> d_img[kStageSets];
    bool mac3 = false;
    bool rot2 = false;
    bool fold = false;
    gsdr::DevBuf<uint4> d_bfrag3;
    gsdr::DevBuf<float4> d_ptab3;
    gsdr::DevBuf<uint4> d_bfrag;
    gsdr::DevBuf<float2> d_ptab, d_dtab;
    gsdr::DevBuf<float> d_mtaps;
    gsdr::DevBuf<unsigned> d_mfmod;
    gsdr::DevBuf<unsigned> d_segmax;
    int seg_k = 1, nseg_alloc = 0;
    gsdr::DevBuf<float2> d_head[kStageSets];
    gsdr::DevBuf<float2> d_tail[kStageSets];
    gsdr::Event ev_abs[4];
    std::vector<hipStream_t> dirty;
    gsdr::Event ev_join;
    bool pipe_overlap = false;
    unsigned long long pipe_seq = 0;
    unsigned long long call_no = 0;
    std::vector<int> bins;
    int nfft = 0, batching = 0;
    gsdr_buffer_helper bh{};
    gsdr::DevBuf<float2> d_win[kStageSets];
    unsigned long long win_seq = 0;
    long long prev_spare_begin = 0, prev_spare_samples = 0;
    bool noise_fft = false;
    gsdr::FftPlan fft{};
    gsdr::DevBuf<float2> d_fft_a, d_fft_b;
    gsdr::DevBuf<float2> d_fft_c;
    gsdr::DevBuf<float> d_fft_win;
    gsdr_param_c pc{};
    std::vector<int> pc_wave_type, pc_freq, pc_chirp_f, pc_swipe_s;
    std::vector<float> pc_chirp_t;
    bool pfb_lds = false;
    bool pfb_blue = false;
    gsdr::DevBuf<float2> d_pfb_tw;
    gsdr::DevBuf<int> d_pfb_sel;
    gsdr::DevBuf<float2> d_pfb_carry[kStageSets];
    int avg_k = 1, avg_kind = GSDR_AVERAGE_COMPLEX;
    int avg_count = 0;
    unsigned long long avg_seq = 0;
    gsdr::DevBuf<float2> d_avg_frames;
    gsdr::DevBuf<float2> d_avg_acc[2];
    ChirpShape cs{};
    int ppt = 0;
    gsdr_vna_helper vh{};
    gsdr::DevBuf<float> d_profile;
    gsdr::DevBuf<float2> d_chirp_part;
    gsdr::DevBuf<float2> d_ccarry[2];
    int cparity = 0;
    int carry_len = 0;
    unsigned long long last_index = 0;

    bool prof = false;
    int prof_every = 1;
    unsigned long long prof_seen = 0;
    std::vector<std::pair<gsdr::Event, gsdr::Event>> ev_pool;
    size_t ev_used = 0;
    const char *kernel_name = "none";
};

namespace {

#define HIPCHK(h, expr)                                                                   \
    do {                                                                                  \
        hipError_t e_ = (expr);                                                           \
        if (e_ != hipSuccess) {                                                           \
            (h)->err = std::string(#expr) + ": " + hipGetErrorString(e_);                 \
            return -1;                                                                    \
        }                                                                                 \
    } while (0)

int fail_create(gsdr_demod *h, const std::string &msg) {
    create_error() = msg;
    if (h) gsdr_demod_close(h);
    return -1;
}

int build_nco_tables(gsdr_demod *h, const std::vector<long long> &tone, unsigned rate) {
    const int Npad = h->Npad, K = h->K;
    std::vector<unsigned> fmod(Npad, 0u);
    std::vector<float2> btab((size_t)K * Npad);
    std::vector<double2> wk(Npad), wrem(Npad);
    for (int n = 0; n < Npad; ++n) {
        const unsigned long long fm = n < h->ddc_channels ? mod_rate(tone[n], rate) : 0u;
        fmod[n] = (unsigned)fm;
        for (int lo = 0; lo < K; ++lo) {
            double re, im;
            phasor((fm * (unsigned long long)lo) % rate, rate, re, im);
            btab[(size_t)lo * Npad + n] = make_float2((float)re, (float)im);
        }
        double re, im;
        phasor((fm * (unsigned long long)K) % rate, rate, re, im);
        wk[n] = make_double2(re, im);
        phasor((fm * (unsigned long long)h->R) % rate, rate, re, im);
        wrem[n] = make_double2(re, im);
    }
    HIPCHK(h, h->d_fmod.upload(fmod));
    HIPCHK(h, h->d_btab.upload(btab));
    HIPCHK(h, h->d_wk.upload(wk));
    HIPCHK(h, h->d_wrem.upload(wrem));
    return 0;
}

int upload_taps_transposed(gsdr_demod *h) {
    std::vector<float> t((size_t)h->M * h->F);
    for (int j = 0; j < h->F; ++j)
        for (int m = 0; m < h->M; ++m) t[(size_t)m * h->F + j] = h->window[(size_t)j * h->M + m];
    HIPCHK(h, h->d_taps_t.upload(t));
    if (h->pipe) {
        const int FP = h->F == 3 ? 4 : h->F;
        std::vector<float> p((size_t)(h->M + h->pad + 2) * FP, 0.f);
        for (int j = 0; j < h->F; ++j)
            for (int m = 0; m < h->M; ++m) p[(size_t)m * FP + j] = h->window[(size_t)j * h->M + m];
        HIPCHK(h, h->d_taps_p.upload(p));
    }
    return 0;
}

long long balanced_near(long long want, int nblk, long long cap) {
    if (want < 1) want = 1;
    if (want > cap) want = cap;
    long long lo = want - want / 5, hi = want + want / 5;
    if (lo < 1) lo = 1;
    if (hi > cap) hi = cap;
    long long best_nch = want;
    double best = -1.0;
    for (long long nch = lo; nch <= hi; ++nch) {
        const long long longest = (nblk + nch - 1) / nch;
        const double balance = ((double)nblk / (double)nch) / (double)longest;
        const double score = balance - 0.05 * std::fabs((double)(nch - want)) / (double)want;
        if (score > best) {
            best = score;
            best_nch = nch;
        }
    }
    return best_nch;
}

int pick_chunks(const gsdr_demod *h, int nblk) {
    if (nblk <= 0) return 1;
    const int TW = h->TW > 0 ? h->TW : 1;
    const long long cap = (h->F > 1) ? nblk / (h->F - 1) : nblk;
    if (cap < 1) return 1;
    long long nch = h->sw.ddc_nch > 0
                        ? (h->sw.ddc_nch < cap ? h->sw.ddc_nch : cap)
                        : balanced_near((long long)(h->waves_ratio * h->target_waves) / TW, nblk, cap);
    if (h->tails_nch > 0 && nch > h->tails_nch) nch = h->tails_nch;
    return (int)(nch < 1 ? 1 : nch);
}

int setup_ddc_common(gsdr_demod *h, int F, int M, unsigned rate,
                     const std::vector<long long> &tone, int max_nblk, bool allow_flat = true) {
    h->F = F;
    h->M = M;
    h->nco_rate = rate;
    if (h->ddc_channels <= 0) h->ddc_channels = h->N;
    h->Npad = ((h->ddc_channels + 63) / 64) * 64;
    h->TW = h->Npad / 64;
    h->pipe = allow_flat && h->sw.ddc_pipe && F <= 4 && !h->sw.ddc_mfma;
    if (h->pipe) {
        int forced = h->sw.ddc_k;
        if (forced != 12 && forced != 16 && forced != 20 && forced != 40) forced = 0;
        double best = 1e300;
        for (int k : {40, 20, 16, 12}) {
            if (forced && forced != k) continue;
            const long long nsub = (M + k - 1) / k;
            const double cost = (double)nsub * (k + 3.3);
            if (cost < best) {
                best = cost;
                h->K = k;
            }
        }
        const int nsub = (M + h->K - 1) / h->K;
        h->pad = nsub * h->K - M;
        h->R = M - (nsub - 1) * h->K;
    } else {
        h->K = h->sw.ddc_k == 32 ? 32 : 16;
        h->R = M % h->K;
    }
    h->simds = device_cus() * 4;
    h->target_waves = h->simds * (h->sw.ddc_waves > 0 ? h->sw.ddc_waves : h->pipe ? 6 : 4);
    {
        const long long cap = (F > 1) ? max_nblk / (F - 1) : max_nblk;
        long long worst = (long long)(1.7 * 1.2 * h->target_waves) / h->TW + 2;
        if (h->sw.ddc_nch > worst) worst = h->sw.ddc_nch;
        if (worst > cap) worst = cap;
        h->tails_nch = (int)(worst < 1 ? 1 : worst);
    }
    h->waves_ratio = 1.3;
    h->nch_max = pick_chunks(h, max_nblk);
    if (build_nco_tables(h, tone, rate)) return -1;
    if (upload_taps_transposed(h)) return -1;
    const size_t tail_elems = (size_t)(h->tails_nch + 1) * (size_t)(F > 1 ? F - 1 : 1) * h->Npad;
    HIPCHK(h, h->d_tails.alloc_zeroed(tail_elems));
    return 0;
}

void set_tables(const gsdr_demod *h, DdcLaunch &a) {
    a.taps_t = h->d_taps_t;
    a.taps_p = h->d_taps_p;
    a.btab = h->d_btab;
    a.wk = h->d_wk;
    a.wrem = h->d_wrem;
    a.fmod = h->d_fmod;
    a.lds_bytes = h->sw.ddc_lds;
    a.sh.prefetch = h->sw.ddc_prefetch;
}

void finish_shape(DdcShape &sh) {
    sh.cbase = sh.nblk / (sh.nch > 0 ? sh.nch : 1);
    sh.crem = sh.nblk % (sh.nch > 0 ? sh.nch : 1);
    sh.rate_magic = 0xffffffffffffffffULL / sh.rate;
    sh.inv_rate = 1.0 / (double)sh.rate;
    sh.m_mod_rate = (unsigned)sh.M % sh.rate;
}

bool prec_pays(const gsdr_demod *h, long long ngt, bool overlap) {
    const long long wgs4 = ((ngt + 7) / 8) * 8 * h->mf.ntq;
    const long long nhi = (h->mf.nk8 + 3) / 4;
    return h->sw.mfma_prec == 1 ||
           (h->sw.mfma_prec < 0 && (wgs4 >= 4LL * (h->simds / 2) || (overlap && wgs4 >= h->simds / 4 && nhi >= 32)));
}

constexpr long long kMac3MinBlocks = 94;
bool mac3_chosen(const gsdr_demod *h, bool images, long long nhi) {
    return images && (h->sw.mfma_3m == 1 || (h->sw.mfma_3m < 0 && nhi >= kMac3MinBlocks));
}

constexpr long long kRot2MinBlocks = 94;
bool rot2_chosen(const gsdr_demod *h, bool mac3, long long nhi) {
    return mac3 && nhi >= 1 && (h->sw.mfma_3m_rot == 2 || (h->sw.mfma_3m_rot < 0 && nhi >= kRot2MinBlocks));
}

constexpr long long kFoldMinBlocks = 94;
bool fold_chosen(const gsdr_demod *h, bool rot2, long long nhi) {
    return rot2 && (h->sw.mfma_fold == 1 || (h->sw.mfma_fold < 0 && nhi >= kFoldMinBlocks));
}

int setup_mfma(gsdr_demod *h, bool direct, const std::vector<long long> &tone) {
    const int F = h->F, M = h->M;
    const unsigned rate = h->nco_rate;
    h->mf_TT = h->sw.mfma_tt;
    h->mf_PK = h->sw.mfma_pk;
    h->mf_W = h->sw.mfma_w;
    if (h->mf_W > h->mf_PK / 8) h->mf_W = h->mf_PK / 8;
    const int asm_kind = h->sw.mfma_asm;
    const bool asm_shape = h->mf_TT == 1 && h->mf_PK == 32 && h->mf_W == 4;
    h->mf_kind = gsdr::MfmaKernel::Cxx;
    if (asm_kind == 2 && asm_shape) h->mf_kind = gsdr::MfmaKernel::AsmRing;
    if (asm_kind == 4 && asm_shape) h->mf_kind = gsdr::MfmaKernel::AsmRing16;
    if (asm_kind == 5 && asm_shape) h->mf_kind = gsdr::MfmaKernel::AsmRing16W8;
    gsdr::MfmaPlan pl{};
    pl.TT = h->mf_TT;
    pl.PK = h->mf_PK;
    pl.M = M;
    pl.MF = M * F;
    pl.nk8 = (pl.MF + 7) / 8;
    pl.rate = rate;
    pl.x16 = h->mf_kind == gsdr::MfmaKernel::AsmRing16 || h->mf_kind == gsdr::MfmaKernel::AsmRing16W8;
    const int nt32 = (h->ddc_channels + 31) / 32;
    pl.ntg = (nt32 + pl.TT - 1) / pl.TT;
    std::vector<unsigned> fmod_in(h->ddc_channels);
    for (int n = 0; n < h->ddc_channels; ++n) fmod_in[n] = mod_rate(tone[n], rate);
    std::vector<uint4> bfrag;
    std::vector<float2> ptab, dtab;
    std::vector<float> taps;
    std::vector<unsigned> fmod;
    float unscale = 1.f;
    gsdr::mfma_build_tables(pl, fmod_in, h->window.data(), bfrag, ptab, dtab, taps, fmod, unscale);
    HIPCHK(h, h->d_bfrag.upload(bfrag));
    HIPCHK(h, h->d_ptab.upload(ptab));
    HIPCHK(h, h->d_dtab.upload(dtab));
    HIPCHK(h, h->d_mtaps.upload(taps));
    HIPCHK(h, h->d_mfmod.upload(fmod));
    {
        h->seg_k = M >= 64 ? 1 : (64 + M - 1) / M;
        const long long t_max = direct ? (long long)(F - 1) * M + h->L : 2LL * h->nfft * h->batching;
        const long long seg_len = (long long)h->seg_k * M;
        h->nseg_alloc = (int)((t_max + seg_len - 1) / seg_len) + 2;
        HIPCHK(h, h->d_segmax.alloc_zeroed((size_t)kScaleSlots * h->nseg_alloc));
    }
    gsdr::MfmaShape &sh = h->mf;
    sh.N = h->ddc_channels;
    sh.NT32 = pl.ntg * pl.TT;
    sh.ntg = pl.ntg;
    sh.ntq = (pl.ntg + h->mf_W - 1) / h->mf_W;
    sh.M = M;
    sh.MF = pl.MF;
    sh.F = F;
    sh.nk8 = pl.nk8;
    sh.woff = direct ? -(F - 1) : 0;
    sh.carry_len = direct ? (F - 1) * M : 0;
    sh.rate = rate;
    sh.rate_magic = 0xffffffffffffffffULL / rate;
    sh.inv_rate = 1.0 / (double)rate;
    sh.m_mod_rate = (unsigned)M % rate;
    sh.unscale = unscale;
#ifdef GSDR_TIMING_BUILD
    sh.timing_mode = h->sw.mfma_timing;
#else
    sh.timing_mode = 0;
#endif
    sh.rt = h->sw.mfma_rt;
    if (direct) {
        const size_t reach = (size_t)((pl.nk8 + pl.PK / 8 - 1) / (pl.PK / 8)) * pl.PK;
        const size_t head_n = (size_t)sh.carry_len + 32u * (size_t)M + reach + 8;
        const size_t tail_n = (size_t)(32 + F) * (size_t)M + reach + 8;
        for (int i = 0; i < kStageSets; ++i) {
            HIPCHK(h, h->d_head[i].alloc_zeroed(head_n));
            HIPCHK(h, h->d_tail[i].alloc_zeroed(tail_n));
        }
    }
    if (h->mf_kind == gsdr::MfmaKernel::AsmRing16) {
        const long long max_rows = direct ? h->L / M : (long long)h->batching;
        const long long ngt_max = (max_rows + 31) / 32;
        const long long nhi = (pl.nk8 + 3) / 4;
        bool want = prec_pays(h, ngt_max, true);
        const bool mac3 = mac3_chosen(h, want, nhi);
        const bool fold = fold_chosen(h, rot2_chosen(h, mac3, nhi), nhi);
        const size_t img_n = fold ? (size_t)ngt_max * (size_t)((nhi + 1) / 2) * 1024
                                  : (size_t)ngt_max * (size_t)nhi * (mac3 ? 768 : 512);
        if (want && img_n * sizeof(uint4) > (size_t)8 << 30) want = false;
        for (int i = 0; i < kStageSets && want; ++i) HIPCHK(h, h->d_img[i].alloc(img_n));
        h->prec = want;
        h->mac3 = want && mac3;
        h->rot2 = rot2_chosen(h, h->mac3, nhi);
        h->fold = fold_chosen(h, h->rot2, nhi);
        if (h->mac3) {
            std::vector<uint4> bfrag3;
            std::vector<float4> ptab3;
            if (h->fold)
                gsdr::mfma_build_tables3f(pl, fmod, bfrag3, ptab3);
            else
                gsdr::mfma_build_tables3(pl, h->rot2 ? 2 : 1, fmod, bfrag3, ptab3);
            HIPCHK(h, h->d_bfrag3.upload(bfrag3));
            HIPCHK(h, h->d_ptab3.upload(ptab3));
        }
    }
    h->mfma = true;
    h->kernel_name = gsdr::ddc_mfma_kernel_name(h->mac3 ? gsdr::MfmaKernel::AsmRing16P3 : h->mf_kind);
    return 0;
}

int enqueue_mfma(gsdr_demod *h, const float2 *in, float2 *raw, long long raw_new0, long long nx,
                 int nout, unsigned idx_base, float2 *out, hipStream_t st, const float2 *spare_src = nullptr,
                 long long spare_n = 0);

template <typename Keep>
int join_streams(gsdr_demod *h, hipStream_t st, Keep keep) {
    size_t w = 0;
    for (size_t i = 0; i < h->dirty.size(); ++i) {
        hipStream_t s = h->dirty[i];
        if (s == st || keep(s)) {
            h->dirty[w++] = s;
            continue;
        }
        if (!h->ev_join) HIPCHK(h, hipEventCreateWithFlags(h->ev_join.out(), hipEventDisableTiming));
        if (hipEventRecord(h->ev_join, s) != hipSuccess) {
            (void)hipGetLastError();
            continue;
        }
        HIPCHK(h, hipStreamWaitEvent(st, h->ev_join, 0));
    }
    h->dirty.resize(w);
    bool have = false;
    for (hipStream_t s : h->dirty) have |= (s == st);
    if (!have) h->dirty.push_back(st);
    return 0;
}

int record_begin(gsdr_demod *h, hipStream_t st, hipEvent_t *stop) {
    *stop = nullptr;
    if (!h->prof || h->ev_used >= (size_t)kMaxEvents) return 0;
    if (h->prof_seen++ % (unsigned long long)h->prof_every != 0) return 0;
    if (h->ev_used == h->ev_pool.size()) {
        gsdr::Event a, b;
        HIPCHK(h, hipEventCreate(a.out()));
        HIPCHK(h, hipEventCreate(b.out()));
        h->ev_pool.emplace_back(std::move(a), std::move(b));
    }
    HIPCHK(h, hipEventRecord(h->ev_pool[h->ev_used].first, st));
    *stop = h->ev_pool[h->ev_used].second;
    h->ev_used++;
    return 0;
}


int autotune_chunks(gsdr_demod *h, int nblk) {
    h->waves_ratio = 1.3;
    if (!h->pipe || h->sw.ddc_nch > 0 || !h->sw.ddc_autotune || nblk < 1) {
        h->nch_max = pick_chunks(h, nblk);
        return 0;
    }
    const size_t n_in = (size_t)nblk * h->M + h->pad + 8;
    const size_t n_out = (size_t)nblk * h->ddc_channels;
    gsdr::DevBuf<float2> x, y;
    HIPCHK(h, x.alloc(n_in));
    if (y.alloc(n_out) != hipSuccess) {
        h->err = "autotune scratch allocation failed";
        return -1;
    }
    (void)hipMemset(x, 0x3c, n_in * sizeof(float2));
    gsdr::Event e0, e1;
    (void)hipEventCreate(e0.out());
    (void)hipEventCreate(e1.out());
    const double cand[] = {0.8, 1.0, 1.3, 1.7};
    double best_ms = 1e30, best_ratio = 1.3;
    int rc = 0;
    for (double r : cand) {
        h->waves_ratio = r;
        DdcLaunch a{};
        a.x = x;
        set_tables(h, a);
        a.out = y;
        a.tails = h->d_tails;
        a.tails_nch = h->tails_nch;
        a.pipe = true;
        a.sh.N = h->ddc_channels;
        a.sh.Npad = h->Npad;
        a.sh.TW = h->TW;
        a.sh.rate = h->nco_rate;
        a.sh.M = h->M;
        a.sh.nblk = nblk;
        a.sh.nch = pick_chunks(h, nblk);
        a.sh.xlast = (long long)nblk * h->M + h->pad - 4;
        finish_shape(a.sh);
        float ms = 0.f;
        for (int it = 0; it < 4 && !rc; ++it) {
            if (it == 1) rc |= hipEventRecord(e0, h->stream) != hipSuccess;
            rc |= gsdr::launch_ddc(h->F, h->K, a, h->stream, nullptr) != hipSuccess;
        }
        rc |= hipEventRecord(e1, h->stream) != hipSuccess;
        rc |= hipEventSynchronize(e1) != hipSuccess;
        if (rc || hipEventElapsedTime(&ms, e0, e1) != hipSuccess) {
            rc = 1;
            break;
        }
        if (ms < best_ms) {
            best_ms = ms;
            best_ratio = r;
        }
    }
    if (rc) {
        h->err = "autotune launch failed";
        return -1;
    }
    h->waves_ratio = best_ratio;
    h->nch_max = pick_chunks(h, nblk);
    return 0;
}

int enqueue_mfma(gsdr_demod *h, const float2 *in, float2 *raw, long long raw_new0, long long nx,
                 int nout, unsigned idx_base, float2 *out, hipStream_t st, const float2 *spare_src,
                 long long spare_n) {
    const int cur = (int)(h->call_no % kScaleSlots), next = (int)((h->call_no + 1) % kScaleSlots);
    const int hs = (int)(h->call_no % kStageSets), hs_next = (int)((h->call_no + 1) % kStageSets);
    gsdr::MfmaLaunch a{};
    a.sh = h->mf;
    a.sh.nout = nout;
    a.sh.ngt = (nout + 31) / 32;
    a.sh.nx = nx;
    a.sh.idx_base = idx_base;
    a.sh.seg_k = h->seg_k;
    gsdr::StageLaunch sg{};
    sg.x = in;
    sg.n = h->L;
    sg.seg = h->d_segmax + (size_t)cur * h->nseg_alloc;
    sg.seg_clear = h->d_segmax + (size_t)next * h->nseg_alloc;
    sg.nseg_alloc = h->nseg_alloc;
    sg.seg_len = (long long)h->seg_k * a.sh.M;
    if (h->mac3) a.sh.rt = 1;
    if (a.sh.rt == 0) {
        const int nblk = (a.sh.nk8 + 3) / 4;
        const long long wgs = (long long)a.sh.ngt * a.sh.ntq;
        a.sh.rt = h->pipe_overlap && nblk <= 32 && wgs >= 512 && wgs < 1024 ? 2 : 1;
    }
    h->last_rt = a.sh.rt;
    if (raw) {
        if (spare_n != raw_new0) {
            h->err = "raw window bookkeeping out of step";
            return -1;
        }
        sg.b = spare_src;
        sg.nb = spare_n;
        sg.b_dst = raw;
        sg.head_cur = raw + raw_new0;
        sg.head_n = h->L;
        sg.tail0 = h->L;
        HIPCHK(h, gsdr::launch_absmax(sg, st));
        if (h->pipe_overlap) HIPCHK(h, hipEventRecord(h->ev_abs[h->pipe_seq % 4], st));
        a.x = a.head = a.tail = raw;
        a.sh.tail0 = 0;
    } else {
        const int cl = a.sh.carry_len;
        const long long t0 = a.sh.ngt > 1 ? (long long)(32 * (a.sh.ngt - 1) + a.sh.woff) * a.sh.M : h->L;
        const int ks = h->mf_PK / 8;
        long long head_n = 32LL * a.sh.M + (long long)((a.sh.nk8 + ks - 1) / ks) * h->mf_PK + 8;
        if (head_n > h->L) head_n = h->L;
        sg.b = h->d_head[hs];
        sg.nb = cl;
        sg.head_cur = h->d_head[hs];
        sg.head_n = head_n;
        sg.head_next = h->d_head[hs_next];
        sg.carry_len = cl;
        sg.tail = h->d_tail[hs];
        sg.tail0 = t0;
        HIPCHK(h, gsdr::launch_absmax(sg, st));
        if (h->pipe_overlap) HIPCHK(h, hipEventRecord(h->ev_abs[h->pipe_seq % 4], st));
        a.x = in;
        a.head = h->d_head[hs];
        a.tail = h->d_tail[hs];
        a.sh.tail0 = t0;
    }
    a.taps = h->d_mtaps;
    a.bfrag = h->d_bfrag;
    a.ptab = h->d_ptab;
    a.dtab = h->d_dtab;
    a.fmod = h->d_mfmod;
    a.segmax = sg.seg;
    a.out = out;
    hipEvent_t stop = nullptr;
    if (record_begin(h, st, &stop)) return -1;
    gsdr::MfmaKernel kind = h->mf_kind;
    if (h->mac3) {
        kind = h->fold ? gsdr::MfmaKernel::AsmRing16P3F
                       : (h->rot2 ? gsdr::MfmaKernel::AsmRing16P3R2 : gsdr::MfmaKernel::AsmRing16P3);
        a.img = h->d_img[hs];
        a.bfrag3 = h->d_bfrag3;
        a.ptab3 = h->d_ptab3;
    } else if (kind == gsdr::MfmaKernel::AsmRing16 && h->prec && a.sh.rt <= 1 && prec_pays(h, a.sh.ngt, h->pipe_overlap)) {
        kind = gsdr::MfmaKernel::AsmRing16P;
        a.img = h->d_img[hs];
    } else if (kind == gsdr::MfmaKernel::AsmRing16 && !h->pipe_overlap && h->sw.mfma_w8) {
        const long long wgs4 = (long long)((a.sh.ngt + 7) / 8) * 8 * a.sh.ntq;
        const long long wgs8 = (long long)((a.sh.ngt + 7) / 8) * 8 * ((a.sh.ntg + 7) / 8);
        if (a.sh.rt <= 1 && wgs4 > h->simds / 4 && wgs4 <= h->simds / 2 && wgs8 <= h->simds / 4)
            kind = gsdr::MfmaKernel::AsmRing16W8;
    }
    h->kernel_name = gsdr::ddc_mfma_kernel_name(kind);
    HIPCHK(h, gsdr::launch_ddc_mfma(kind, h->mf_TT, h->mf_PK, h->mf_W, a, st));
    if (stop) HIPCHK(h, hipEventRecord(stop, st));
    h->call_no++;
    return 0;
}

int enqueue_direct(gsdr_demod *h, const float2 *in, float2 *out, hipStream_t st) {
    DdcLaunch a{};
    a.x = in;
    set_tables(h, a);
    a.pipe = h->pipe && h->decim > 0 && h->L >= 4;
    a.few = h->few;
    a.out = out;
    a.sh.N = h->N;
    a.sh.Npad = h->Npad;
    a.sh.TW = h->TW;
    a.sh.rate = h->nco_rate;
    a.sh.idx0 = h->idx;
    a.sh.g_off = 0;
    long long ret;
    hipEvent_t stop = nullptr;
    if (h->decim > 0 && h->mfma) {
        const unsigned rate = h->nco_rate;
        const unsigned back = (unsigned)(((unsigned long long)(h->F - 1) * h->M) % rate);
        const unsigned idx_base = (unsigned)((h->idx + rate - back) % rate);
        if (enqueue_mfma(h, in, nullptr, 0, h->L, (int)(h->L / h->M), idx_base, out, st)) return -1;
        ret = (long long)h->N * (h->L / h->M);
    } else if (h->decim > 0) {
        a.tails = h->d_tails;
        a.tails_nch = h->tails_nch;
        a.carry_in = h->d_carry[h->parity];
        a.carry_out = h->d_carry[h->parity ^ 1];
        a.sh.M = h->M;
        a.sh.nblk = (int)(h->L / h->M);
        a.sh.nch = h->nch_max;
        a.sh.xlast = h->L - 4;
        if (a.pipe && h->pad > 0) {
            HIPCHK(h, hipMemcpyAsync(h->d_stage, in, (size_t)h->L * sizeof(float2),
                                     hipMemcpyDeviceToDevice, st));
            a.x = h->d_stage;
            a.sh.xlast = h->L + h->pad - 4;
        }
        finish_shape(a.sh);
        if (record_begin(h, st, &stop)) return -1;
        HIPCHK(h, gsdr::launch_ddc(h->F, h->K, a, st, stop));
        h->parity ^= 1;
        ret = (long long)h->N * (h->L / h->M);
    } else {
        a.sh.M = h->K;
        a.sh.total = h->L;
        a.sh.nblk = (int)((h->L + h->K - 1) / h->K);
        long long nch = h->target_waves / h->TW;
        if (nch < 1) nch = 1;
        if (nch > a.sh.nblk) nch = a.sh.nblk;
        a.sh.nch = (int)nch;
        finish_shape(a.sh);
        if (record_begin(h, st, &stop)) return -1;
        HIPCHK(h, gsdr::launch_mix(h->K, a, h->sw.mix_few, st));
        if (stop) HIPCHK(h, hipEventRecord(stop, st));
        ret = (long long)h->N * h->L;
    }
    h->idx = (h->idx + (unsigned long long)h->L) % h->nco_rate;
    return (int)ret;
}

int enqueue_noise_fft(gsdr_demod *h, const float2 *in, float2 *out, hipStream_t st) {
    const int cb = h->bh.current_batch;
    float2 *win = h->d_win[h->win_seq % kStageSets];
    if (h->prev_spare_samples > 0)
        HIPCHK(h, hipMemcpyAsync(win, h->d_win[(h->win_seq + kStageSets - 1) % kStageSets] + h->prev_spare_begin,
                                 (size_t)h->prev_spare_samples * sizeof(float2), hipMemcpyDeviceToDevice, st));
    HIPCHK(h, hipMemcpyAsync(win + h->bh.new_0, in, (size_t)h->L * sizeof(float2), hipMemcpyDeviceToDevice, st));
    if (cb > 0) {
        hipEvent_t stop = nullptr;
        if (record_begin(h, st, &stop)) return -1;
        HIPCHK(h, gsdr::launch_pfb_filter(win, h->d_fft_win, h->nfft, h->F, cb, h->d_fft_a, st));
        if (h->d_fft_c) {
            HIPCHK(h, gsdr::fft_forward(h->fft, h->d_fft_a, h->d_fft_c, h->d_fft_b, cb, st));
            HIPCHK(h, gsdr::launch_pfb_select(h->d_fft_c, h->nfft, cb, h->d_pfb_sel, h->ddc_channels, out, st));
        } else {
            HIPCHK(h, gsdr::fft_forward(h->fft, h->d_fft_a, out, h->d_fft_b, cb, st));
        }
        if (stop) HIPCHK(h, hipEventRecord(stop, st));
    }
    h->prev_spare_begin = h->bh.spare_begin;
    h->prev_spare_samples = h->bh.spare_samples > 0 ? h->bh.spare_samples : 0;
    h->win_seq++;
    const int ret = h->ddc_channels * cb;
    gsdr_buffer_helper_update(&h->bh);
    return ret;
}

int enqueue_pfb_lds(gsdr_demod *h, const float2 *in, float2 *out, hipStream_t st) {
    const int cb = h->bh.current_batch;
    const float2 *carry = h->d_pfb_carry[h->win_seq % kStageSets];
    float2 *carry_out = h->d_pfb_carry[(h->win_seq + 1) % kStageSets];
    const int spare_n = h->bh.spare_samples > 0 ? h->bh.spare_samples : 0;
    if (spare_n > h->nfft * h->F) {
        h->err = "PFB carry larger than a window";
        return -1;
    }
    const int *sel = h->mode == GSDR_NOISE ? nullptr : h->d_pfb_sel;
    const long long wlen = (long long)h->bh.new_0 + h->L;
    const gsdr::FftPlan *blue = h->pfb_blue ? &h->fft : nullptr;
    const float2 *tw = h->pfb_blue ? h->fft.d_tw : h->d_pfb_tw;
    hipEvent_t stop = nullptr;
    if (record_begin(h, st, &stop)) return -1;
    HIPCHK(h, gsdr::launch_pfb_lds(carry, h->bh.new_0, in, h->d_fft_win, tw, h->nfft, h->F, cb, sel, h->ddc_channels, out,
                                   carry_out, h->bh.spare_begin, spare_n, wlen, st, blue, h->sw, &h->kernel_name));
    if (stop) HIPCHK(h, hipEventRecord(stop, st));
    h->win_seq++;
    const int ret = h->ddc_channels * cb;
    gsdr_buffer_helper_update(&h->bh);
    return ret;
}

int enqueue_pfb(gsdr_demod *h, const float2 *in, float2 *out, hipStream_t st) {
    if (h->pfb_lds) return enqueue_pfb_lds(h, in, out, st);
    if (h->noise_fft) return enqueue_noise_fft(h, in, out, st);
    const int cb = h->bh.current_batch;
    float2 *win = h->d_win[h->win_seq % kStageSets];
    const float2 *spare = h->prev_spare_samples > 0
                              ? h->d_win[(h->win_seq + kStageSets - 1) % kStageSets] + h->prev_spare_begin
                              : nullptr;
    if (!(cb > 0 && h->mfma)) {
        if (spare)
            HIPCHK(h, hipMemcpyAsync(win, spare, (size_t)h->prev_spare_samples * sizeof(float2),
                                     hipMemcpyDeviceToDevice, st));
        HIPCHK(h, hipMemcpyAsync(win + h->bh.new_0, in, (size_t)h->L * sizeof(float2),
                                 hipMemcpyDeviceToDevice, st));
        if (h->pipe_overlap) HIPCHK(h, hipEventRecord(h->ev_abs[h->pipe_seq % 4], st));
    }
    if (cb > 0 && h->mfma) {
        if (enqueue_mfma(h, in, win, h->bh.new_0, (long long)(cb + h->F - 1) * h->M, cb, 0u, out, st, spare,
                         h->prev_spare_samples))
            return -1;
    } else if (cb > 0) {
        DdcLaunch a{};
        a.x = win;
        set_tables(h, a);
        a.out = out;
        a.tails = h->d_tails;
        a.tails_nch = h->tails_nch;
        a.carry_in = nullptr;
        a.carry_out = nullptr;
        a.sh.N = h->ddc_channels;
        a.sh.Npad = h->Npad;
        a.sh.TW = h->TW;
        a.sh.rate = h->nco_rate;
        a.sh.idx0 = 0;
        a.sh.M = h->M;
        a.sh.nblk = cb + h->F - 1;
        a.pipe = h->pipe;
        a.sh.xlast = (long long)a.sh.nblk * h->M + h->pad - 4;
        a.sh.g_off = h->F - 1;
        const int nch = pick_chunks(h, a.sh.nblk);
        a.sh.nch = nch;
        finish_shape(a.sh);
        hipEvent_t stop = nullptr;
        if (record_begin(h, st, &stop)) return -1;
        HIPCHK(h, gsdr::launch_ddc(h->F, h->K, a, st, stop));
    }
    h->prev_spare_begin = h->bh.spare_begin;
    h->prev_spare_samples = h->bh.spare_samples > 0 ? h->bh.spare_samples : 0;
    h->win_seq++;
    const int ret = h->ddc_channels * cb;
    gsdr_buffer_helper_update(&h->bh);
    return ret;
}

int enqueue_pfb_average(gsdr_demod *h, const float2 *in, float2 *out, hipStream_t st) {
    const int cb = h->bh.current_batch;
    const size_t ev0 = h->ev_used;
    if (enqueue_pfb(h, in, h->d_avg_frames, st) < 0) return -1;
    if (cb <= 0) return 0;
    const long long rows = ((long long)h->avg_count + cb) / h->avg_k;
    HIPCHK(h, gsdr::launch_pfb_average(h->d_avg_frames, cb, h->ddc_channels, h->avg_k, h->avg_kind, h->avg_count,
                                       h->d_avg_acc[h->avg_seq % 2], h->d_avg_acc[(h->avg_seq + 1) % 2], out, st));
    if (h->ev_used > ev0) HIPCHK(h, hipEventRecord(h->ev_pool[h->ev_used - 1].second, st));
    h->avg_seq++;
    h->avg_count = (int)(((long long)h->avg_count + cb) % h->avg_k);
    return (int)(rows * h->ddc_channels);
}

int enqueue_chirp(gsdr_demod *h, const float2 *in, float2 *out, hipStream_t st) {
    hipEvent_t stop = nullptr;
    int ret;
    if (h->decim <= 0) {
        if (record_begin(h, st, &stop)) return -1;
        HIPCHK(h, gsdr::launch_chirp_demod(in, out, h->L, h->last_index, h->cs, st));
        if (stop) HIPCHK(h, hipEventRecord(stop, st));
        ret = (int)h->L;
    } else {
        const int valid = h->vh.valid_size;
        const unsigned long long idx0 =
            (h->last_index + h->cs.period - (unsigned long long)h->carry_len % h->cs.period) %
            h->cs.period;
        if (record_begin(h, st, &stop)) return -1;
        HIPCHK(h, gsdr::launch_chirp_lockin(h->d_ccarry[h->cparity], h->carry_len, in,
                                            h->d_profile, h->ppt, valid, out, idx0, h->cs, st, h->sw.chirp_split,
                                            h->d_chirp_part, h->d_chirp_part ? kChirpPartials : 0));
        if (stop) HIPCHK(h, hipEventRecord(stop, st));
        const int new0 = h->vh.new0;
        if (new0 > 0) {
            const long long from_in = (long long)new0 <= h->L ? new0 : h->L;
            const long long from_carry = new0 - from_in;
            float2 *dst = h->d_ccarry[h->cparity ^ 1];
            if (from_carry > 0)
                HIPCHK(h, hipMemcpyAsync(dst, h->d_ccarry[h->cparity] + (h->carry_len - from_carry),
                                         (size_t)from_carry * sizeof(float2),
                                         hipMemcpyDeviceToDevice, st));
            HIPCHK(h, hipMemcpyAsync(dst + from_carry, in + (h->L - from_in),
                                     (size_t)from_in * sizeof(float2), hipMemcpyDeviceToDevice,
                                     st));
            h->cparity ^= 1;
        }
        h->carry_len = new0;
        gsdr_vna_helper_update(&h->vh);
        ret = valid;
    }
    h->last_index = (h->last_index + (unsigned long long)h->L) % h->cs.period;
    return ret;
}


int refuse(gsdr_demod *h, const char *msg) {
    h->err = msg;
    return -1;
}

int setup_direct(gsdr_demod *h, const gsdr_param_c *p) {
    const gsdr::Switches &sw = h->sw;
    if (p->rate <= 0) return refuse(h, "rate must be positive");
    if (!(p->n_freq >= h->N && p->freq)) return refuse(h, "DIRECT needs one frequency per wave_type entry");
    const std::vector<long long> tone(p->freq, p->freq + h->N);
    if (h->decim <= 0) {
        h->F = 1;
        h->M = 1;
        h->window.assign(1, 1.f);
        if (setup_ddc_common(h, 1, 1, (unsigned)p->rate, tone, 1, false)) return -1;
        h->kernel_name = gsdr::mix_kernel_name(h->N, h->TW, h->L, h->K, sw.mix_few);
        h->capacity = (long long)h->N * h->L;
        return 0;
    }
    if (h->L % h->decim != 0) return refuse(h, "buffer_len must be a multiple of decim (ref: fir.cu:20)");
    if (p->pf_average < 1 || p->pf_average > kMaxF) return refuse(h, "pf_average must be in [1,8] for DIRECT with decimation");
    if (h->decim > 0x7fffffffLL / p->pf_average) return refuse(h, "decim*pf_average overflows");
    const int F = (int)p->pf_average, M = (int)h->decim;
    h->window.resize((size_t)M * F);
    gsdr_make_sinc_window(M * F, (float)(0.75 / (M * 2)), h->window.data());
    if (setup_ddc_common(h, F, M, (unsigned)p->rate, tone, (int)(h->L / M))) return -1;
    if (h->pipe && h->pad > 0 && h->d_stage.alloc_zeroed((size_t)h->L + h->pad) != hipSuccess)
        return refuse(h, "staging allocation failed");
    h->kernel_name = h->pipe ? gsdr::ddc_flat_kernel_name() : gsdr::ddc_kernel_name();
    for (auto &c : h->d_carry)
        if (c.alloc_zeroed((size_t)(F > 1 ? F - 1 : 1) * h->Npad) != hipSuccess) return refuse(h, "carry allocation failed");
    h->few = sw.ddc_mfma && sw.ddc_few && !h->pipe && M >= 512 && h->N <= 32 && h->TW == 1;
    if (h->few) h->kernel_name = gsdr::ddc_few_kernel_name();
    if (!h->few && sw.ddc_mfma && h->L / M >= F - 1 && h->L >= 4 && F <= 33 && (M * F + 31) / 32 * 32 - M * F <= M &&
        setup_mfma(h, true, tone))
        return -1;
    if (!h->mfma && autotune_chunks(h, (int)(h->L / M))) return -1;
    h->capacity = (long long)h->N * (h->L / M);
    return 0;
}

int setup_pfb_lds(gsdr_demod *h, bool noise, int F, const std::vector<long long> &tone, long long blue_m) {
    h->pfb_lds = true;
    h->pfb_blue = blue_m > 0;
    h->F = F;
    h->M = h->nfft;
    std::vector<float2> tw((size_t)h->nfft);
    for (int k = 0; k < h->nfft; ++k) {
        const double a = -2.0 * M_PI * (double)k / (double)h->nfft;
        tw[(size_t)k] = make_float2((float)std::cos(a), (float)std::sin(a));
    }
    const std::vector<int> sel(tone.begin(), tone.end());
    bool ok = h->d_pfb_tw.upload(tw) == hipSuccess && h->d_fft_win.upload(h->window) == hipSuccess &&
              (noise || h->d_pfb_sel.upload(sel) == hipSuccess);
    if (ok && h->pfb_blue) ok = gsdr::fft_plan_build(h->fft, h->nfft) == 0 && h->fft.m == (int)blue_m;
    for (int i = 0; i < kStageSets && ok; ++i) ok = h->d_pfb_carry[i].alloc_zeroed((size_t)h->nfft * F + 8) == hipSuccess;
    if (!ok) return refuse(h, "PFB allocation failed");
    h->kernel_name = gsdr::pfb_kernel_name(gsdr::pfb_choose(h->nfft, F, h->pfb_blue ? &h->fft : nullptr,
                                                            (int)(h->L / h->nfft), h->ddc_channels, device_cus(), h->sw));
    return 0;
}

int setup_pfb_global(gsdr_demod *h, bool tones_global, int F, const std::vector<long long> &tone) {
    h->noise_fft = true;
// ... 443 lines not shown
                while (ok && pending-- > 0) ok = gsdr_demod_wait(twin) >= 0;
            };
            if (ok && (what & GSDR_PREPARE_PIPELINE_HOST))
                rehearse_submit([&] { return gsdr_demod_submit(twin, pin_in, pin_out); }, 2 * GSDR_PIPELINE_DEPTH + 2);
            const gsdr_sc16 *pin_in16 = reinterpret_cast<const gsdr_sc16 *>(pin_in);
            if (ok && sc16 && (what & GSDR_PREPARE_HOST))
                for (int k = 0; k < 2 && ok; ++k) ok = gsdr_demod_process_sc16(twin, pin_in16, pin_out) >= 0;
            if (ok && sc16 && (what & GSDR_PREPARE_PIPELINE_HOST))
                rehearse_submit([&] { return gsdr_demod_submit_sc16(twin, pin_in16, pin_out); }, GSDR_PIPELINE_DEPTH + 2);
        }
        if (!ok) h->err = std::string("rehearsal failed: ") + (twin ? twin->err : create_error());
        if (pin_in) (void)hipHostFree(pin_in);
        if (pin_out) (void)hipHostFree(pin_out);
        if (twin) gsdr_demod_close(twin);
        if (!ok) return -1;
    }
    return 0;
}

static int submit_begin(gsdr_demod *h, const void *in, const void *out, gsdr_demod::Slot **slot) {
    if (refuse_null(h, in, out)) return -1;
    if (h->pipe_count >= GSDR_PIPELINE_DEPTH) {
        h->err = "pipeline full: call gsdr_demod_wait() first";
        return -1;
    }
    if (h->device >= 0) HIPCHK(h, hipSetDevice(h->device));
    if (pipeline_init(h)) return -1;
    *slot = &h->slot[(h->pipe_head + h->pipe_count) % GSDR_PIPELINE_DEPTH];
    return 0;
}

static int submit_end(gsdr_demod *h, gsdr_demod::Slot &sl, hipEvent_t wait_ev, int n) {
    sl.wait_ev = wait_ev;
    sl.n = n;
    h->pipe_count++;
    return 0;
}

static int submit_host(gsdr_demod *h, const gsdr_c64 *in_host, const gsdr_sc16 *in16_host, gsdr_c64 *out_host) {
    gsdr_demod::Slot *slot = nullptr;
    if (submit_begin(h, in16_host ? (const void *)in16_host : in_host, out_host, &slot)) return -1;
    auto &sl = *slot;
    if (slot_buffers(h, sl, true, true, in16_host != nullptr)) return -1;
    if (in16_host) {
        HIPCHK(h, hipMemcpyAsync(sl.d_in16, in16_host, (size_t)h->L * sizeof(gsdr_sc16), hipMemcpyHostToDevice, h->s_up));
        HIPCHK(h, gsdr::launch_widen_sc16(sl.d_in16, sl.d_in, h->L, h->sc16_scale, h->cus, h->s_up));
    } else {
        HIPCHK(h, hipMemcpyAsync(sl.d_in, in_host, (size_t)h->L * sizeof(float2), hipMemcpyHostToDevice, h->s_up));
    }
    HIPCHK(h, hipEventRecord(sl.up, h->s_up));
    const int n = pipeline_compute(h, sl, sl.up, sl.d_in, sl.d_out);
    if (n < 0) return -1;
    HIPCHK(h, hipStreamWaitEvent(h->s_down, sl.done, 0));
    if (n > 0)
        HIPCHK(h, hipMemcpyAsync(out_host, sl.d_out, (size_t)n * sizeof(float2), hipMemcpyDeviceToHost, h->s_down));
    HIPCHK(h, hipEventRecord(sl.down, h->s_down));
    return submit_end(h, sl, sl.down, n);
}

int gsdr_demod_submit(gsdr_demod *h, const gsdr_c64 *in_host, gsdr_c64 *out_host) {
    return submit_host(h, in_host, nullptr, out_host);
}

int gsdr_demod_submit_sc16(gsdr_demod *h, const gsdr_sc16 *in_host, gsdr_c64 *out_host) {
    return submit_host(h, nullptr, in_host, out_host);
}

static int submit_device(gsdr_demod *h, const gsdr_c64 *in_dev, const gsdr_sc16 *in16_dev, gsdr_c64 *out_dev) {
    gsdr_demod::Slot *slot = nullptr;
    if (submit_begin(h, in16_dev ? (const void *)in16_dev : in_dev, out_dev, &slot)) return -1;
    auto &sl = *slot;
    float2 *out = reinterpret_cast<float2 *>(out_dev);
    int n;
    if (!in16_dev) {
        n = pipeline_compute(h, sl, nullptr, reinterpret_cast<const float2 *>(in_dev), out);
    } else if (h->mode == GSDR_NODSP) {
        n = pipeline_compute(h, sl, nullptr, nullptr, out, in16_dev);
    } else {
        if (slot_buffers(h, sl, true, false, false)) return -1;
        HIPCHK(h, gsdr::launch_widen_sc16(in16_dev, sl.d_in, h->L, h->sc16_scale, h->cus, h->s_up));
        HIPCHK(h, hipEventRecord(sl.up, h->s_up));
        n = pipeline_compute(h, sl, sl.up, sl.d_in, out);
    }
    if (n < 0) return -1;
    return submit_end(h, sl, sl.done, n);
}

int gsdr_demod_submit_device(gsdr_demod *h, const gsdr_c64 *in_dev, gsdr_c64 *out_dev) {
    return submit_device(h, in_dev, nullptr, out_dev);
}

int gsdr_demod_submit_device_sc16(gsdr_demod *h, const gsdr_sc16 *in_dev, gsdr_c64 *out_dev) {
    return submit_device(h, nullptr, in_dev, out_dev);
}

int gsdr_demod_wait(gsdr_demod *h) {
    if (!h) return -1;
    if (h->pipe_count == 0) return -2;
    if (h->device >= 0) HIPCHK(h, hipSetDevice(h->device));
    auto &sl = h->slot[h->pipe_head];
    const hipError_t e = hipEventSynchronize(sl.wait_ev);
    h->pipe_head = (h->pipe_head + 1) % GSDR_PIPELINE_DEPTH;
    h->pipe_count--;
    if (e != hipSuccess) {
        h->err = std::string("hipEventSynchronize: ") + hipGetErrorString(e);
        return -1;
    }
    return sl.n;
}

void gsdr_demod_close(gsdr_demod *h) {
    if (!h) return;
    if (h->device >= 0) (void)hipSetDevice(h->device);
    if (h->stream) (void)hipStreamSynchronize(h->stream);
    for (int i = 0; i < kPipeStreams; ++i)
        if (h->s_main[i]) (void)hipStreamSynchronize(h->s_main[i]);
    if (h->s_up) (void)hipStreamSynchronize(h->s_up);
    if (h->s_down) (void)hipStreamSynchronize(h->s_down);
    delete h;
}

int gsdr_demod_set_sc16_scale(gsdr_demod *h, float scale) {
    if (!h) return -1;
    if (!std::isfinite(scale) || !(scale > 0.f)) {
        h->err = "sc16 scale must be finite and > 0";
        return -1;
    }
    h->sc16_scale = scale;
    return 0;
}

float gsdr_demod_sc16_scale(const gsdr_demod *h) { return h ? h->sc16_scale : 0.f; }

int gsdr_demod_set_frame_average(gsdr_demod *h, int k, int kind) {
    if (!h) return -1;
    if (h->mode != GSDR_TONES && h->mode != GSDR_NOISE) {
        h->err = "frame average: only TONES and NOISE handles have frames to average";
        return -1;
    }
    if (k < 1 || k > GSDR_FRAME_AVERAGE_MAX) {
        h->err = "frame average: k must be in [1, " + std::to_string(GSDR_FRAME_AVERAGE_MAX) + "]";
        return -1;
    }
    if (kind != GSDR_AVERAGE_COMPLEX && kind != GSDR_AVERAGE_POWER) {
        h->err = "frame average: kind must be GSDR_AVERAGE_COMPLEX (0) or GSDR_AVERAGE_POWER (1)";
        return -1;
    }
    if (h->win_seq > 0 || h->pipe_count > 0) {
        h->err = "frame average: must be set before the first buffer goes through the handle";
        return -1;
    }
    if (h->device >= 0) HIPCHK(h, hipSetDevice(h->device));
    if (k > 1) {
        if (!h->d_avg_frames) HIPCHK(h, h->d_avg_frames.alloc((size_t)h->ddc_channels * (size_t)h->batching));
        for (auto &p : h->d_avg_acc) {
            if (!p) HIPCHK(h, p.alloc((size_t)h->ddc_channels));
            HIPCHK(h, hipMemset(p, 0, (size_t)h->ddc_channels * sizeof(float2)));
        }
    }
    const long long capacity = (long long)h->ddc_channels * ((h->batching + k - 1) / k);
    if (capacity > h->capacity) {
        h->d_out.reset();
        h->d_in.reset();
        for (auto &sl : h->slot) sl.d_out.reset();
    }
    h->avg_k = k;
    h->avg_kind = kind;
    h->avg_count = 0;
    h->capacity = capacity;
    return 0;
}

int gsdr_demod_frame_average(const gsdr_demod *h, int *kind) {
    if (kind) *kind = h ? h->avg_kind : GSDR_AVERAGE_COMPLEX;
    return h ? h->avg_k : 0;
}

int gsdr_frame_average_device(const gsdr_c64 *frames_dev, int n_frames, int n_ch, int k, int kind, int count,
                              const gsdr_c64 *acc_in_dev, gsdr_c64 *acc_out_dev, gsdr_c64 *out_dev, void *hip_stream) {
    const char *bad = nullptr;
    if (n_frames < 0 || n_ch < 1) bad = "n_frames must be >= 0 and n_ch >= 1";
    else if (k < 1 || k > GSDR_FRAME_AVERAGE_MAX) bad = "k must be in [1, 1048576]";
    else if (kind != GSDR_AVERAGE_COMPLEX && kind != GSDR_AVERAGE_POWER) bad = "kind must be GSDR_AVERAGE_COMPLEX or GSDR_AVERAGE_POWER";
    else if (count < 0 || count >= k) bad = "count must be in [0, k)";
    else if (!acc_out_dev || (n_frames > 0 && !frames_dev) || (count > 0 && !acc_in_dev) ||
             (((long long)count + n_frames) / k > 0 && !out_dev)) bad = "null buffer";
    else if (((uintptr_t)frames_dev | (uintptr_t)acc_in_dev | (uintptr_t)acc_out_dev | (uintptr_t)out_dev) & 7) bad = "pointers must be 8-byte aligned";
    if (bad) {
        create_error() = std::string("gsdr_frame_average_device: ") + bad;
        return -1;
    }
    const hipError_t e = gsdr::launch_pfb_average(reinterpret_cast<const float2 *>(frames_dev), n_frames, n_ch, k, kind, count,
                                                  reinterpret_cast<const float2 *>(acc_in_dev), reinterpret_cast<float2 *>(acc_out_dev),
                                                  reinterpret_cast<float2 *>(out_dev), (hipStream_t)hip_stream);
    if (e != hipSuccess) {
        create_error() = std::string("gsdr_frame_average_device: ") + hipGetErrorString(e);
        return -1;
    }
    return (int)(((long long)count + n_frames) / k);
}

void gsdr_note_error_(const char *msg) { create_error() = msg ? msg : ""; }

int gsdr_widen_sc16_device(const gsdr_sc16 *in_dev, gsdr_c64 *out_dev, long long n, float scale, void *hip_stream) {
    if (n < 0 || (n > 0 && (!in_dev || !out_dev))) {
        create_error() = "gsdr_widen_sc16_device: null buffer";
        return -1;
    }
    const hipError_t e = gsdr::launch_widen_sc16(in_dev, reinterpret_cast<float2 *>(out_dev), n, scale, device_cus(),
                                                 (hipStream_t)hip_stream);
    if (e != hipSuccess) {
        create_error() = std::string("gsdr_widen_sc16_device: ") + hipGetErrorString(e);
        return -1;
    }
    return 0;
}

int gsdr_pfb_lds_stages(int fft_tones, int *radices) {
    int tmp[16];
    const int n = gsdr::pfb_lds_plan(fft_tones, tmp, gsdr::read_switches().pfb_radix8);
    if (radices)
        for (int i = 0; i < n && i < 16; ++i) radices[i] = tmp[i];
    return n;
}

int gsdr_demod_mode(const gsdr_demod *h) { return h ? h->mode : -1; }
int gsdr_demod_channels(const gsdr_demod *h) { return h ? h->N : 0; }
long long gsdr_demod_out_capacity(const gsdr_demod *h) { return h ? h->capacity : 0; }
float gsdr_demod_fcut(const gsdr_demod *h) { return h ? h->fcut : 0.f; }

int gsdr_demod_get_window(const gsdr_demod *h, float *w, int cap) {
    if (!h) return 0;
    const int n = (int)h->window.size();
    if (w)
        for (int i = 0; i < n && i < cap; ++i) w[i] = h->window[i];
    return n;
}

int gsdr_demod_get_bins(const gsdr_demod *h, int *bins, int cap) {
    if (!h) return 0;
    const int n = (int)h->bins.size();
    if (bins)
        for (int i = 0; i < n && i < cap; ++i) bins[i] = h->bins[i];
    return n;
}

void gsdr_demod_profile_enable(gsdr_demod *h, int enable) {
    if (!h) return;
    h->prof = enable != 0;
    h->prof_every = enable > 1 ? enable : 1;
    h->prof_seen = 0;
    h->ev_used = 0;
}

int gsdr_demod_profile_read(gsdr_demod *h, double *total_ms) {
    if (total_ms) *total_ms = 0.0;
    if (!h || h->ev_used == 0) return 0;
    if (h->device >= 0) (void)hipSetDevice(h->device);
    double sum = 0.0;
    int n = 0;
    for (size_t i = 0; i < h->ev_used; ++i) {
        if (hipEventSynchronize(h->ev_pool[i].second) != hipSuccess) continue;
        float ms = 0.f;
        if (hipEventElapsedTime(&ms, h->ev_pool[i].first, h->ev_pool[i].second) == hipSuccess) {
            sum += ms;
            n++;
        }
    }
    if (total_ms) *total_ms = sum;
    return n;
}

const char *gsdr_demod_kernel_name(const gsdr_demod *h) { return h ? h->kernel_name : "none"; }

void gsdr_reload_env(void) {}

const char *gsdr_build_info(void) {
#ifdef GSDR_TIMING_BUILD
    return "abi 1; arch gfx950; timing_build 1";
#else
    return "abi 1; arch gfx950; timing_build 0";
#endif
}

int gsdr_demod_describe(const gsdr_demod *h, char *buf, int cap) {
    if (!h || !buf || cap < 1) return 0;
    static const char *modes[] = {"TONES", "CHIRP", "NOISE", "RAMP", "NODSP", "SWONLY", "DIRECT"};
    std::string s = "{\"mode\": \"";
    s += (h->mode >= 0 && h->mode <= 6) ? modes[h->mode] : "?";
    s += "\", \"kernel\": \"";
    s += h->kernel_name;
    s += "\", \"family\": \"";
    s += h->pfb_lds ? (h->pfb_blue ? "polyphase filter + Bluestein (two fp32 Stockham FFTs) inside the LDS + bin selection, one launch"
                                   : "polyphase filter + fp32 Stockham FFT inside the LDS + bin selection, one launch") :
         h->noise_fft ? "fp32 Stockham FFT behind the polyphase filter" : h->mfma ? "f16 MFMA, hi/lo split" : (h->mode == GSDR_CHIRP ? "fp32 VALU, integer phase" : (h->pipe ? "packed fp32 VALU" : "fp32 VALU"));
    s += "\", \"channels\": " + std::to_string(h->ddc_channels > 0 ? h->ddc_channels : h->N);
    s += ", \"row_tiles_per_workgroup\": " + std::to_string(h->mfma ? h->last_rt : 0);
    s += ", \"complex_mac\": " + std::to_string(h->mfma && h->mac3 ? 3 : 4);
    s += ", \"complex_mac_min_blocks\": " + std::to_string(kMac3MinBlocks);
    s += ", \"rotation_blocks\": " + std::to_string(h->mfma && h->mac3 && h->rot2 ? 2 : 1);
    s += ", \"rotation_min_blocks\": " + std::to_string(kRot2MinBlocks);
    s += ", \"fold\": " + std::to_string(h->mfma && h->mac3 && h->rot2 && h->fold ? 1 : 0);
    s += ", \"fold_min_blocks\": " + std::to_string(kFoldMinBlocks);
    s += ", \"pipeline_streams\": " + std::to_string(h->sw.pipe_streams);
    s += ", \"frame_average\": " + std::to_string(h->avg_k);
    s += std::string(", \"frame_average_kind\": \"") + (h->avg_kind == GSDR_AVERAGE_POWER ? "power" : "complex") + "\"";
    s += ", \"timing_build\": ";
#ifdef GSDR_TIMING_BUILD
    s += "1";
#else
    s += "0";
#endif
    s += ", \"env\": {";
    bool first = true;
    for (char **e = environ; e && *e; ++e) {
        if (std::strncmp(*e, "GSDR_", 5) != 0) continue;
        const char *eq = std::strchr(*e, '=');
        if (!eq) continue;
        std::string k(*e, eq - *e), v(eq + 1);
        for (auto &c : v)
            if (c == '"' || c == '\\' || (unsigned char)c < 0x20) c = '?';
        s += (first ? "\"" : ", \"") + k + "\": \"" + v + "\"";
        first = false;
    }
    s += "}}";
    const int n = (int)s.size() < cap - 1 ? (int)s.size() : cap - 1;
    std::memcpy(buf, s.data(), (size_t)n);
    buf[n] = 0;
    return n;
}

}
```

Baseline: 11920.

## Add four-product folded MFMA loop with direct-form B fragments

```diff
diff --git a/gpu_sdr_amd/csrc/ddc_kernels.h b/gpu_sdr_amd/csrc/ddc_kernels.h
--- a/gpu_sdr_amd/csrc/ddc_kernels.h
+++ b/gpu_sdr_amd/csrc/ddc_kernels.h
@@ -31,6 +31,7 @@
     int mfma_3m = -1;
     int mfma_3m_rot = -1;
     int mfma_fold = -1;
+    int mfma_fold_products = -1;
     int mfma_timing = 0;
     bool noise_fft = true;
     bool tones_fft = true;
@@ -160,6 +161,8 @@
                         std::vector<float4> &ptab3);
 void mfma_build_tables3f(const MfmaPlan &pl, const std::vector<unsigned> &fmod, std::vector<uint4> &bfrag3,
                          std::vector<float4> &ptab3);
+void mfma_build_tables4f(const MfmaPlan &pl, const std::vector<unsigned> &fmod, std::vector<uint4> &bfrag3,
+                         std::vector<float4> &ptab3);
 struct StageLaunch {
     const float2 *x;
     long long n;
@@ -177,7 +180,7 @@
     long long tail0;
 };
 hipError_t launch_absmax(const StageLaunch &s, hipStream_t st);
-enum class MfmaKernel { AsmRing, Cxx, AsmRing16, AsmRing16W8, AsmRing16P, AsmRing16P3, AsmRing16P3R2, AsmRing16P3F };
+enum class MfmaKernel { AsmRing, Cxx, AsmRing16, AsmRing16W8, AsmRing16P, AsmRing16P3, AsmRing16P3R2, AsmRing16P3F, AsmRing16P4F };
 hipError_t launch_ddc_mfma(MfmaKernel kind, int TT, int PK, int W, const MfmaLaunch &a, hipStream_t st);
 const char *ddc_mfma_kernel_name(MfmaKernel kind);
 
diff --git a/gpu_sdr_amd/csrc/ddc_mfma.hip b/gpu_sdr_amd/csrc/ddc_mfma.hip
--- a/gpu_sdr_amd/csrc/ddc_mfma.hip
+++ b/gpu_sdr_amd/csrc/ddc_mfma.hip
@@ -11,6 +11,7 @@
 #include "ddc_mfma_ring16p3_gen.h"
 #include "ddc_mfma_ring16p3r2_gen.h"
 #include "ddc_mfma_ring16p3f_gen.h"
+#include "ddc_mfma_ring16p4f_gen.h"
 
 namespace gsdr {
 
@@ -821,7 +822,8 @@
     ring16p3_tile<true>(a, lds, gt0, tg, wave, active);
 }
 
-__global__ __launch_bounds__(128) __attribute__((target("no-packed-fp32-ops"))) void ddc_convert3f_kernel(const MfmaLaunch a, uint4 *__restrict__ img, int nhi, int nspan) {
+template <bool kDirect>
+__device__ __forceinline__ __attribute__((target("no-packed-fp32-ops"))) void convert_fold(const MfmaLaunch &a, uint4 *__restrict__ img, int nhi, int nspan) {
     const MfmaShape &sh = a.sh;
     const int l = threadIdx.x & 63, rh = threadIdx.x >> 6;
     const int r = 16 * rh + (l & 15), g = l >> 4;
@@ -858,7 +860,7 @@
 #pragma clang fp contract(off)
         const float pa = mul_legacy(xr[j], hs[j]), pb = mul_legacy(xi[j], hs[j]);
         const float qa = whole ? mul_legacy(yr[7 - j], gs[7 - j]) : 0.f, qb = whole ? mul_legacy(yi[7 - j], gs[7 - j]) : 0.f;
-        const float u[4] = {pa + qa, pb - qb, pa + pb, qa + qb};
+        const float u[4] = {pa + qa, kDirect ? qb - pb : pb - qb, kDirect ? pa - qa : pa + pb, kDirect ? pb + qb : qa + qb};
 #pragma unroll
         for (int c = 0; c < 4; ++c) {
             _Float16 h, w;
@@ -875,14 +877,27 @@
     }
 }
 
+__global__ __launch_bounds__(128) __attribute__((target("no-packed-fp32-ops"))) void ddc_convert3f_kernel(const MfmaLaunch a, uint4 *__restrict__ img, int nhi, int nspan) {
+    convert_fold<false>(a, img, nhi, nspan);
+}
+
+__global__ __launch_bounds__(128) __attribute__((target("no-packed-fp32-ops"))) void ddc_convert4f_kernel(const MfmaLaunch a, uint4 *__restrict__ img, int nhi, int nspan) {
+    convert_fold<true>(a, img, nhi, nspan);
+}
+
+static_assert(GSDR_MFMA_RING16P4F_SLOT == GSDR_MFMA_RING16P3F_SLOT && GSDR_MFMA_RING16P4F_BYTES == GSDR_MFMA_RING16P3F_BYTES,
+              "one image format and one ring for both folded loops");
+
+template <bool kDirect>
 __device__ __forceinline__ __attribute__((target("no-packed-fp32-ops"))) void ring16p3f_tile(
     const MfmaLaunch &a, uint4 *lds, int gt, int tg, int wave, bool active) {
+    constexpr unsigned kImages = kDirect ? 8 : 16;
     const MfmaShape &sh = a.sh;
     const int Np = sh.NT32 * 32;
     const int nspan = ((sh.nk8 + 3) / 4 + 1) / 2;
     const int lane = (int)(fresh_tid() & 63u);
     const unsigned po = (unsigned)(tg * 32 + (lane & 15)) * 16u;
-    const unsigned bo = (unsigned)tg * (16u * 1024u) + (unsigned)lane * 16u;
+    const unsigned bo = (unsigned)tg * (kImages * 1024u) + (unsigned)lane * 16u;
     const unsigned lds_base = (unsigned)(unsigned long long)(__attribute__((address_space(3))) char *)lds;
     const unsigned rd16 = lds_base + (unsigned)lane * 16u;
     const unsigned io0 = (unsigned)wave * 4096u + (unsigned)lane * 16u, io1 = io0 + 1024u, io2 = io0 + 2048u, io3 = io0 + 3072u;
@@ -890,13 +905,16 @@
     const unsigned accaddr = lds_base + (unsigned)wave * 8192u + (unsigned)lane * 16u;
     const unsigned long long ibb = (unsigned long long)(a.img + (size_t)gt * nspan * (GSDR_MFMA_RING16P3F_SLOT / 16)),
                              ppb = (unsigned long long)a.ptab3, bfb = (unsigned long long)a.bfrag3;
-    asm volatile(GSDR_MFMA_RING16P3F_TEXT
-                 :
-                 : [io0] "v"(io0), [io1] "v"(io1), [io2] "v"(io2), [io3] "v"(io3), [po] "v"(po), [bo] "v"(bo),
-                   [lane16] "v"(rd16), [accaddr] "v"(accaddr), GSDR_SGPR_PAIR(ib, ibb), [wrs] GSDR_SGPR(wrs),
-                   GSDR_SGPR_PAIR(pp, ppb), GSDR_SGPR_PAIR(bf, bfb), [pstride] GSDR_SGPR((unsigned)Np * 16u),
-                   [nhi] GSDR_SGPR(nspan)
-                 : GSDR_MFMA_RING16P3F_CLOBBERS);
+#define GSDR_RING16P3F_OPERANDS                                                                                    \
+    [io0] "v"(io0), [io1] "v"(io1), [io2] "v"(io2), [io3] "v"(io3), [po] "v"(po), [bo] "v"(bo),                    \
+        [lane16] "v"(rd16), [accaddr] "v"(accaddr), GSDR_SGPR_PAIR(ib, ibb), [wrs] GSDR_SGPR(wrs),                 \
+        GSDR_SGPR_PAIR(pp, ppb), GSDR_SGPR_PAIR(bf, bfb), [pstride] GSDR_SGPR((unsigned)Np * 16u),                 \
+        [nhi] GSDR_SGPR(nspan)
+    if constexpr (kDirect)
+        asm volatile(GSDR_MFMA_RING16P4F_TEXT : : GSDR_RING16P3F_OPERANDS : GSDR_MFMA_RING16P4F_CLOBBERS);
+    else
+        asm volatile(GSDR_MFMA_RING16P3F_TEXT : : GSDR_RING16P3F_OPERANDS : GSDR_MFMA_RING16P3F_CLOBBERS);
+#undef GSDR_RING16P3F_OPERANDS
     if (active) ring16_epilogue(a, lds, gt, tg, wave, (int)(fresh_tid() & 63u), kScaleFromTable);
 }
 
@@ -914,7 +932,24 @@
     const int tg_raw = (q % sh.ntq) * W + wave;
     const bool active = tg_raw < sh.ntg;
     const int tg = active ? tg_raw : sh.ntg - 1;
-    ring16p3f_tile(a, lds, gt0, tg, wave, active);
+    ring16p3f_tile<false>(a, lds, gt0, tg, wave, active);
+}
+
+__global__ __launch_bounds__(256, 2) __attribute__((target("no-packed-fp32-ops"))) void ddc_mfma_ring16p4f_kernel(
+    const MfmaLaunch a) {
+    constexpr int W = 4;
+    __shared__ uint4 lds[GSDR_MFMA_RING16P4F_BYTES / 16];
+    static_assert(GSDR_MFMA_RING16P4F_BYTES >= 4 * 8192, "the accumulators fit");
+    static_assert(2 * GSDR_MFMA_RING16P4F_BYTES <= 160 * 1024, "two workgroups per compute unit");
+    const MfmaShape &sh = a.sh;
+    const int wave = __builtin_amdgcn_readfirstlane((int)(threadIdx.x >> 6));
+    const int xcd = blockIdx.x & 7, q = blockIdx.x >> 3;
+    const int gt0 = (q / sh.ntq) * 8 + xcd;
+    if (gt0 >= sh.ngt) return;
+    const int tg_raw = (q % sh.ntq) * W + wave;
+    const bool active = tg_raw < sh.ntg;
+    const int tg = active ? tg_raw : sh.ntg - 1;
+    ring16p3f_tile<true>(a, lds, gt0, tg, wave, active);
 }
 
 constexpr int kStageChunk = 2048;
@@ -1193,15 +1228,30 @@
         }
 }
 
+static void half_phasor(unsigned rate, unsigned long long ph2, double &re, double &im) {
+    const double ang = M_PI * ((double)ph2 / (double)rate);
+    re = std::cos(ang);
+    im = -std::sin(ang);
+}
+
+static void fold_span_phasors(const MfmaPlan &pl, const std::vector<unsigned> &fmod, std::vector<float4> &ptab3) {
+    const int Np = pl.ntg * pl.TT * 32;
+    const unsigned long long rate2 = 2ULL * pl.rate;
+    const int nrow = ((pl.nk8 + 3) / 4 + 1) / 2;
+    ptab3.assign((size_t)(nrow + 1) * Np, make_float4(0.f, 0.f, 0.f, 0.f));
+    for (int row = 0; row < nrow; ++row)
+        for (int n = 0; n < Np; ++n) {
+            const unsigned long long t2 = (128ULL * (unsigned long long)row + 63ULL) % rate2;
+            double re, im;
+            half_phasor(pl.rate, (unsigned long long)(((unsigned __int128)fmod[n] * t2) % rate2), re, im);
+            ptab3[(size_t)row * Np + n] = make_float4((float)re, (float)im, (float)(im - re), (float)(re + im));
+        }
+}
+
 void mfma_build_tables3f(const MfmaPlan &pl, const std::vector<unsigned> &fmod, std::vector<uint4> &bfrag3,
                          std::vector<float4> &ptab3) {
-    const int tiles = pl.ntg * pl.TT, Np = tiles * 32;
+    const int tiles = pl.ntg * pl.TT;
     const unsigned long long rate2 = 2ULL * pl.rate;
-    auto half_phasor = [&](unsigned long long ph2, double &re, double &im) {
-        const double ang = M_PI * ((double)ph2 / (double)pl.rate);
-        re = std::cos(ang);
-        im = -std::sin(ang);
-    };
     bfrag3.assign((size_t)tiles * 16 * 64, uint4{0, 0, 0, 0});
     for (int T = 0; T < tiles; ++T)
         for (int th = 0; th < 2; ++th)
@@ -1211,7 +1261,7 @@
                 for (int jj = 0; jj < 8; ++jj) {
                     const int j = 8 * (lane >> 4) + jj;
                     double wr, wi;
-                    half_phasor((fm * (unsigned long long)(63 - 2 * j)) % rate2, wr, wi);
+                    half_phasor(pl.rate, (fm * (unsigned long long)(63 - 2 * j)) % rate2, wr, wi);
                     const double c = wr, d = -wi;
                     const float v[4] = {(float)c, (float)d, (float)(c + d), (float)(c - d)};
                     for (int u = 0; u < 4; ++u) {
@@ -1227,15 +1277,38 @@
                         bfrag3[((size_t)T * 16 + (u * 2 + th) * 2 + sp) * 64 + lane] = w;
                     }
             }
-    const int nrow = ((pl.nk8 + 3) / 4 + 1) / 2;
-    ptab3.assign((size_t)(nrow + 1) * Np, make_float4(0.f, 0.f, 0.f, 0.f));
-    for (int row = 0; row < nrow; ++row)
-        for (int n = 0; n < Np; ++n) {
-            const unsigned long long t2 = (128ULL * (unsigned long long)row + 63ULL) % rate2;
-            double re, im;
-            half_phasor((unsigned long long)(((unsigned __int128)fmod[n] * t2) % rate2), re, im);
-            ptab3[(size_t)row * Np + n] = make_float4((float)re, (float)im, (float)(im - re), (float)(re + im));
-        }
+    fold_span_phasors(pl, fmod, ptab3);
+}
+
+void mfma_build_tables4f(const MfmaPlan &pl, const std::vector<unsigned> &fmod, std::vector<uint4> &bfrag3,
+                         std::vector<float4> &ptab3) {
+    const int tiles = pl.ntg * pl.TT;
+    const unsigned long long rate2 = 2ULL * pl.rate;
+    bfrag3.assign((size_t)tiles * 8 * 64, uint4{0, 0, 0, 0});
+    for (int T = 0; T < tiles; ++T)
+        for (int th = 0; th < 2; ++th)
+            for (int lane = 0; lane < 64; ++lane) {
+                const unsigned long long fm = fmod[(size_t)T * 32 + 16 * th + (lane & 15)];
+                unsigned short img[2][2][8];
+                for (int jj = 0; jj < 8; ++jj) {
+                    const int j = 8 * (lane >> 4) + jj;
+                    double wr, wi;
+                    half_phasor(pl.rate, (fm * (unsigned long long)(63 - 2 * j)) % rate2, wr, wi);
+                    const float v[2] = {(float)wr, (float)-wi};
+                    for (int u = 0; u < 2; ++u) {
+                        const unsigned short hb = to_half_bits(v[u]);
+                        img[u][0][jj] = hb;
+                        img[u][1][jj] = to_half_bits(v[u] - from_half_bits(hb));
+                    }
+                }
+                for (int u = 0; u < 2; ++u)
+                    for (int sp = 0; sp < 2; ++sp) {
+                        uint4 w;
+                        __builtin_memcpy(&w, img[u][sp], 16);
+                        bfrag3[((size_t)T * 8 + (u * 2 + th) * 2 + sp) * 64 + lane] = w;
+                    }
+            }
+    fold_span_phasors(pl, fmod, ptab3);
 }
 
 hipError_t launch_absmax(const StageLaunch &s, hipStream_t st) {
@@ -1303,17 +1376,25 @@
                 hipLaunchKernelGGL(ddc_mfma_ring16p_kernel, dim3(grid), dim3(256), 0, st, a);
             return hipGetLastError();
         }
-        case MfmaKernel::AsmRing16P3F: {
+        case MfmaKernel::AsmRing16P3F:
+        case MfmaKernel::AsmRing16P4F: {
+            const bool direct = kind == MfmaKernel::AsmRing16P4F;
             if (!a.img || !a.bfrag3 || !a.ptab3) return hipErrorInvalidValue;
             const int nhi = (sh.nk8 + 3) / 4, nspan = (nhi + 1) / 2;
             const long long cgrid = (long long)sh.ngt * nspan;
             grid = ring_grid(sh.ngt, sh.ntq, 1);
             if (cgrid < 1 || cgrid > 0x7fffffffLL || !grid) return hipErrorInvalidValue;
-            hipLaunchKernelGGL(ddc_convert3f_kernel, dim3((unsigned)cgrid), dim3(128), 0, st, a, const_cast<uint4 *>(a.img),
-                               nhi, nspan);
+            uint4 *img = const_cast<uint4 *>(a.img);
+            if (direct)
+                hipLaunchKernelGGL(ddc_convert4f_kernel, dim3((unsigned)cgrid), dim3(128), 0, st, a, img, nhi, nspan);
+            else
+                hipLaunchKernelGGL(ddc_convert3f_kernel, dim3((unsigned)cgrid), dim3(128), 0, st, a, img, nhi, nspan);
             const hipError_t e = hipGetLastError();
             if (e != hipSuccess) return e;
-            hipLaunchKernelGGL(ddc_mfma_ring16p3f_kernel, dim3(grid), dim3(256), 0, st, a);
+            if (direct)
+                hipLaunchKernelGGL(ddc_mfma_ring16p4f_kernel, dim3(grid), dim3(256), 0, st, a);
+            else
+                hipLaunchKernelGGL(ddc_mfma_ring16p3f_kernel, dim3(grid), dim3(256), 0, st, a);
             return hipGetLastError();
         }
         case MfmaKernel::AsmRing16W8:
@@ -1339,7 +1420,8 @@
         case MfmaKernel::AsmRing16P:
         case MfmaKernel::AsmRing16P3:
         case MfmaKernel::AsmRing16P3R2:
-        case MfmaKernel::AsmRing16P3F: return "ddc_mfma_ring16p_kernel";
+        case MfmaKernel::AsmRing16P3F:
+        case MfmaKernel::AsmRing16P4F: return "ddc_mfma_ring16p_kernel";
         case MfmaKernel::AsmRing16W8: return "ddc_mfma_ring16w8_kernel";
         case MfmaKernel::AsmRing16: return "ddc_mfma_ring16_kernel";
         case MfmaKernel::AsmRing: return "ddc_mfma_ring_kernel";
diff --git a/gpu_sdr_amd/csrc/ddc_mfma_ring16p4f_gen.h b/gpu_sdr_amd/csrc/ddc_mfma_ring16p4f_gen.h
--- /dev/null
+++ b/gpu_sdr_amd/csrc/ddc_mfma_ring16p4f_gen.h
@@ -0,0 +1,628 @@
+#pragma once
+#define GSDR_MFMA_RING16P4F_VB 12
+#define GSDR_MFMA_RING16P4F_SLOT 16384
+#define GSDR_MFMA_RING16P4F_BYTES 65536
+#define GSDR_MFMA_RING16P4F_TEXT \
+    "s_mov_b32 s73, m0\n\t" \
+    "s_mov_b32 s52, %[ib_lo]\n\t" \
+    "s_mov_b32 s53, %[ib_hi]\n\t" \
+    "s_mov_b32 s74, %[wrs]\n\t" \
+    "s_mov_b32 s64, %[pp_lo]\n\t" \
+    "s_mov_b32 s65, %[pp_hi]\n\t" \
+    "s_mov_b32 s56, %[bf_lo]\n\t" \
+    "s_mov_b32 s57, %[bf_hi]\n\t" \
+    "s_mov_b32 s58, %[pstride]\n\t" \
+    "s_mov_b32 s42, %[nhi]\n\t" \
+    "s_add_u32 s44, %[nhi], -1\n\t" \
+    "s_mov_b32 s43, 0\n\t" \
+    "s_mov_b32 s45, 0\n\t" \
+    "s_mov_b32 s46, 16384\n\t" \
+    "s_mov_b32 s72, 32768\n\t" \
+    "s_mov_b32 s47, 49152\n\t" \
+    "s_nop 4\n\t" \
+    "s_add_u32 s66, s56, 4096\n\t" \
+    "s_addc_u32 s67, s57, 0\n\t" \
+    "s_add_u32 s40, s64, s58\n\t" \
+    "s_addc_u32 s41, s65, 0\n\t" \
+    "s_nop 4\n\t" \
+    "global_load_dwordx4 v[140:143], %[po], s[64:65]\n\t" \
+    "global_load_dwordx4 v[144:147], %[po], s[64:65] offset:256\n\t" \
+    "global_load_dwordx4 a[0:3], %[bo], s[56:57] offset:0\n\t" \
+    "global_load_dwordx4 a[4:7], %[bo], s[56:57] offset:1024\n\t" \
+    "global_load_dwordx4 a[8:11], %[bo], s[56:57] offset:2048\n\t" \
+    "global_load_dwordx4 a[12:15], %[bo], s[56:57] offset:3072\n\t" \
+    "global_load_dwordx4 a[16:19], %[bo], s[66:67] offset:0\n\t" \
+    "global_load_dwordx4 a[20:23], %[bo], s[66:67] offset:1024\n\t" \
+    "global_load_dwordx4 a[24:27], %[bo], s[66:67] offset:2048\n\t" \
+    "global_load_dwordx4 a[28:31], %[bo], s[66:67] offset:3072\n\t" \
+    "v_mov_b32 v60, 0\n\t" \
+    "v_mov_b32 v61, 0\n\t" \
+    "v_mov_b32 v62, 0\n\t" \
+    "v_mov_b32 v63, 0\n\t" \
+    "v_mov_b32 v64, 0\n\t" \
+    "v_mov_b32 v65, 0\n\t" \
+    "v_mov_b32 v66, 0\n\t" \
+    "v_mov_b32 v67, 0\n\t" \
+    "v_mov_b32 v68, 0\n\t" \
+    "v_mov_b32 v69, 0\n\t" \
+    "v_mov_b32 v70, 0\n\t" \
+    "v_mov_b32 v71, 0\n\t" \
+    "v_mov_b32 v72, 0\n\t" \
+    "v_mov_b32 v73, 0\n\t" \
+    "v_mov_b32 v74, 0\n\t" \
+    "v_mov_b32 v75, 0\n\t" \
+    "v_mov_b32 v12, 0\n\t" \
+    "v_mov_b32 v13, 0\n\t" \
+    "v_mov_b32 v14, 0\n\t" \
+    "v_mov_b32 v15, 0\n\t" \
+    "v_mov_b32 v16, 0\n\t" \
+    "v_mov_b32 v17, 0\n\t" \
+    "v_mov_b32 v18, 0\n\t" \
+    "v_mov_b32 v19, 0\n\t" \
+    "v_mov_b32 v20, 0\n\t" \
+    "v_mov_b32 v21, 0\n\t" \
+    "v_mov_b32 v22, 0\n\t" \
+    "v_mov_b32 v23, 0\n\t" \
+    "v_mov_b32 v24, 0\n\t" \
+    "v_mov_b32 v25, 0\n\t" \
+    "v_mov_b32 v26, 0\n\t" \
+    "v_mov_b32 v27, 0\n\t" \
+    "v_mov_b32 v28, 0\n\t" \
+    "v_mov_b32 v29, 0\n\t" \
+    "v_mov_b32 v30, 0\n\t" \
+    "v_mov_b32 v31, 0\n\t" \
+    "v_mov_b32 v32, 0\n\t" \
+    "v_mov_b32 v33, 0\n\t" \
+    "v_mov_b32 v34, 0\n\t" \
+    "v_mov_b32 v35, 0\n\t" \
+    "v_mov_b32 v36, 0\n\t" \
+    "v_mov_b32 v37, 0\n\t" \
+    "v_mov_b32 v38, 0\n\t" \
+    "v_mov_b32 v39, 0\n\t" \
+    "v_mov_b32 v40, 0\n\t" \
+    "v_mov_b32 v41, 0\n\t" \
+    "v_mov_b32 v42, 0\n\t" \
+    "v_mov_b32 v43, 0\n\t" \
+    "v_mov_b32 v148, 0\n\t" \
+    "v_mov_b32 v149, 0\n\t" \
+    "v_mov_b32 v150, 0\n\t" \
+    "v_mov_b32 v151, 0\n\t" \
+    "v_mov_b32 v152, 0\n\t" \
+    "v_mov_b32 v153, 0\n\t" \
+    "v_mov_b32 v154, 0\n\t" \
+    "v_mov_b32 v155, 0\n\t" \
+    "s_min_u32 s50, s43, s44\n\t" \
+    "s_mul_i32 s51, s50, 16384\n\t" \
+    "s_add_u32 s36, s52, s51\n\t" \
+    "s_addc_u32 s37, s53, 0\n\t" \
+    "s_add_u32 s43, s43, 1\n\t" \
+    "s_nop 4\n\t" \
+    "s_add_u32 m0, s45, s74\n\t" \
+    "s_nop 0\n\t" \
+    "global_load_lds_dwordx4 %[io0], s[36:37]\n\t" \
+    "s_nop 4\n\t" \
+    "s_add_u32 m0, m0, 1024\n\t" \
+    "s_nop 0\n\t" \
+    "global_load_lds_dwordx4 %[io1], s[36:37]\n\t" \
+    "s_nop 4\n\t" \
+    "s_add_u32 m0, m0, 1024\n\t" \
+    "s_nop 0\n\t" \
+    "global_load_lds_dwordx4 %[io2], s[36:37]\n\t" \
+    "s_nop 4\n\t" \
+    "s_add_u32 m0, m0, 1024\n\t" \
+    "s_nop 0\n\t" \
+    "global_load_lds_dwordx4 %[io3], s[36:37]\n\t" \
+    "s_nop 4\n\t" \
+    "s_min_u32 s50, s43, s44\n\t" \
+    "s_mul_i32 s51, s50, 16384\n\t" \
+    "s_add_u32 s60, s52, s51\n\t" \
+    "s_addc_u32 s61, s53, 0\n\t" \
+    "s_add_u32 s43, s43, 1\n\t" \
+    "s_nop 4\n\t" \
+    "s_add_u32 m0, s46, s74\n\t" \
+    "s_nop 0\n\t" \
+    "global_load_lds_dwordx4 %[io0], s[60:61]\n\t" \
+    "s_nop 4\n\t" \
+    "s_add_u32 m0, m0, 1024\n\t" \
+    "s_nop 0\n\t" \
+    "global_load_lds_dwordx4 %[io1], s[60:61]\n\t" \
+    "s_nop 4\n\t" \
+    "s_add_u32 m0, m0, 1024\n\t" \
+    "s_nop 0\n\t" \
+    "global_load_lds_dwordx4 %[io2], s[60:61]\n\t" \
+    "s_nop 4\n\t" \
+    "s_add_u32 m0, m0, 1024\n\t" \
+    "s_nop 0\n\t" \
+    "global_load_lds_dwordx4 %[io3], s[60:61]\n\t" \
+    "s_nop 4\n\t" \
+    "s_min_u32 s50, s43, s44\n\t" \
+    "s_mul_i32 s51, s50, 16384\n\t" \
+    "s_add_u32 s76, s52, s51\n\t" \
+    "s_addc_u32 s77, s53, 0\n\t" \
+    "s_add_u32 s43, s43, 1\n\t" \
+    "s_nop 4\n\t" \
+    "s_add_u32 m0, s72, s74\n\t" \
+    "s_nop 0\n\t" \
+    "global_load_lds_dwordx4 %[io0], s[76:77]\n\t" \
+    "s_nop 4\n\t" \
+    "s_add_u32 m0, m0, 1024\n\t" \
+    "s_nop 0\n\t" \
+    "global_load_lds_dwordx4 %[io1], s[76:77]\n\t" \
+    "s_nop 4\n\t" \
+    "s_add_u32 m0, m0, 1024\n\t" \
+    "s_nop 0\n\t" \
+    "global_load_lds_dwordx4 %[io2], s[76:77]\n\t" \
+    "s_nop 4\n\t" \
+    "s_add_u32 m0, m0, 1024\n\t" \
+    "s_nop 0\n\t" \
+    "global_load_lds_dwordx4 %[io3], s[76:77]\n\t" \
+    "s_nop 4\n\t" \
+    "v_add_u32 v156, s45, %[lane16]\n\t" \
+    "v_add_u32 v157, s46, %[lane16]\n\t" \
+    "s_waitcnt vmcnt(0)\n\t" \
+    "s_barrier\n\t" \
+    "ds_read_b128 v[76:79], v156 offset:0\n\t" \
+    "ds_read_b128 v[80:83], v156 offset:1024\n\t" \
+    "ds_read_b128 v[84:87], v156 offset:2048\n\t" \
+    "ds_read_b128 v[88:91], v156 offset:3072\n\t" \
+    "s_waitcnt lgkmcnt(0)\n\t" \
+    "1:\n\t" \
+    "s_waitcnt lgkmcnt(3)\n\t" \
+    "v_mfma_f32_16x16x32_f16 v[44:47], v[84:87], a[0:3], 0\n\t" \
+    "s_min_u32 s50, s43, s44\n\t" \
+    "s_mul_i32 s51, s50, 16384\n\t" \
+    "s_add_u32 s36, s52, s51\n\t" \
+    "v_mfma_f32_16x16x32_f16 v[48:51], v[84:87], a[8:11], 0\n\t" \
+    "s_addc_u32 s37, s53, 0\n\t" \
+    "s_add_u32 s43, s43, 1\n\t" \
+    "s_waitcnt lgkmcnt(2)\n\t" \
+    "v_mfma_f32_16x16x32_f16 v[52:55], v[88:91], a[0:3], 0\n\t" \
+    "ds_read_b128 v[100:103], v156 offset:6144\n\t" \
+    "s_add_u32 m0, s47, s74\n\t" \
+    "s_nop 0\n\t" \
+    "global_load_lds_dwordx4 %[io0], s[36:37]\n\t" \
+    "v_fma_f32 v12, -v149, v60, v12\n\t" \
+    "v_fma_f32 v13, -v149, v61, v13\n\t" \
+    "v_mfma_f32_16x16x32_f16 v[56:59], v[88:91], a[8:11], 0\n\t" \
+    "v_fma_f32 v14, -v149, v62, v14\n\t" \
+    "v_fma_f32 v15, -v149, v63, v15\n\t" \
+    "s_waitcnt lgkmcnt(2)\n\t" \
+    "v_mfma_f32_16x16x32_f16 v[44:47], v[76:79], a[4:7], v[44:47]\n\t" \
+    "ds_read_b128 v[104:107], v156 offset:7168\n\t" \
+    "v_fma_f32 v16, -v153, v64, v16\n\t" \
+    "v_mfma_f32_16x16x32_f16 v[48:51], v[76:79], a[12:15], v[48:51]\n\t" \
+    "v_fma_f32 v17, -v153, v65, v17\n\t" \
+    "v_fma_f32 v18, -v153, v66, v18\n\t" \
+    "s_waitcnt lgkmcnt(2)\n\t" \
+    "v_mfma_f32_16x16x32_f16 v[52:55], v[80:83], a[4:7], v[52:55]\n\t" \
+    "v_fma_f32 v19, -v153, v67, v19\n\t" \
+    "v_mfma_f32_16x16x32_f16 v[56:59], v[80:83], a[12:15], v[56:59]\n\t" \
+    "v_fma_f32 v20, -v149, v68, v20\n\t" \
+    "v_fma_f32 v21, -v149, v69, v21\n\t" \
+    "v_mfma_f32_16x16x32_f16 v[44:47], v[76:79], a[0:3], v[44:47]\n\t" \
+    "ds_read_b128 v[92:95], v156 offset:4096\n\t" \
+    "v_fma_f32 v22, -v149, v70, v22\n\t" \
+    "v_mfma_f32_16x16x32_f16 v[48:51], v[76:79], a[8:11], v[48:51]\n\t" \
+    "v_fma_f32 v23, -v149, v71, v23\n\t" \
+    "v_fma_f32 v24, -v153, v72, v24\n\t" \
+    "v_mfma_f32_16x16x32_f16 v[52:55], v[80:83], a[0:3], v[52:55]\n\t" \
+    "ds_read_b128 v[96:99], v156 offset:5120\n\t" \
+    "s_add_u32 m0, m0, 1024\n\t" \
+    "s_nop 0\n\t" \
+    "global_load_lds_dwordx4 %[io1], s[36:37]\n\t" \
+    "v_fma_f32 v25, -v153, v73, v25\n\t" \
+    "v_mfma_f32_16x16x32_f16 v[56:59], v[80:83], a[8:11], v[56:59]\n\t" \
+    "v_fma_f32 v26, -v153, v74, v26\n\t" \
+    "v_fma_f32 v27, -v153, v75, v27\n\t" \
+    "s_waitcnt lgkmcnt(3)\n\t" \
+    "v_mfma_f32_16x16x32_f16 v[44:47], v[100:103], a[16:19], v[44:47]\n\t" \
+    "v_fma_f32 v28, v148, v60, v28\n\t" \
+    "v_mfma_f32_16x16x32_f16 v[48:51], v[100:103], a[24:27], v[48:51]\n\t" \
+    "v_fma_f32 v29, v148, v61, v29\n\t" \
+    "v_fma_f32 v30, v148, v62, v30\n\t" \
+    "s_waitcnt lgkmcnt(2)\n\t" \
+    "v_mfma_f32_16x16x32_f16 v[52:55], v[104:107], a[16:19], v[52:55]\n\t" \
+    "ds_read_b128 v[116:119], v156 offset:10240\n\t" \
+    "v_fma_f32 v31, v148, v63, v31\n\t" \
+    "v_mfma_f32_16x16x32_f16 v[56:59], v[104:107], a[24:27], v[56:59]\n\t" \
+    "v_fma_f32 v32, v152, v64, v32\n\t" \
+    "v_fma_f32 v33, v152, v65, v33\n\t" \
+    "s_waitcnt lgkmcnt(2)\n\t" \
+    "v_mfma_f32_16x16x32_f16 v[44:47], v[92:95], a[20:23], v[44:47]\n\t" \
+    "ds_read_b128 v[120:123], v156 offset:11264\n\t" \
+    "v_fma_f32 v34, v152, v66, v34\n\t" \
+    "v_mfma_f32_16x16x32_f16 v[48:51], v[92:95], a[28:31], v[48:51]\n\t" \
+    "v_fma_f32 v35, v152, v67, v35\n\t" \
+    "v_fma_f32 v36, v148, v68, v36\n\t" \
+    "s_waitcnt lgkmcnt(2)\n\t" \
+    "v_mfma_f32_16x16x32_f16 v[52:55], v[96:99], a[20:23], v[52:55]\n\t" \
+    "s_add_u32 m0, m0, 1024\n\t" \
+    "s_nop 0\n\t" \
+    "global_load_lds_dwordx4 %[io2], s[36:37]\n\t" \
+    "v_fma_f32 v37, v148, v69, v37\n\t" \
+    "v_mfma_f32_16x16x32_f16 v[56:59], v[96:99], a[28:31], v[56:59]\n\t" \
+    "v_fma_f32 v38, v148, v70, v38\n\t" \
+    "v_fma_f32 v39, v148, v71, v39\n\t" \
+    "v_mfma_f32_16x16x32_f16 v[44:47], v[92:95], a[16:19], v[44:47]\n\t" \
+    "ds_read_b128 v[108:111], v156 offset:8192\n\t" \
+    "v_fma_f32 v40, v152, v72, v40\n\t" \
+    "v_mfma_f32_16x16x32_f16 v[48:51], v[92:95], a[24:27], v[48:51]\n\t" \
+    "v_fma_f32 v41, v152, v73, v41\n\t" \
+    "v_fma_f32 v42, v152, v74, v42\n\t" \
+    "v_mfma_f32_16x16x32_f16 v[52:55], v[96:99], a[16:19], v[52:55]\n\t" \
+    "ds_read_b128 v[112:115], v156 offset:9216\n\t" \
+    "v_fma_f32 v43, v152, v75, v43\n\t" \
+    "v_mfma_f32_16x16x32_f16 v[56:59], v[96:99], a[24:27], v[56:59]\n\t" \
+    "s_waitcnt lgkmcnt(3)\n\t" \
+    "v_mfma_f32_16x16x32_f16 v[60:63], v[116:119], a[16:19], 0\n\t" \
+    "v_mfma_f32_16x16x32_f16 v[64:67], v[116:119], a[24:27], 0\n\t" \
+    "s_waitcnt lgkmcnt(2)\n\t" \
+    "v_mfma_f32_16x16x32_f16 v[68:71], v[120:123], a[16:19], 0\n\t" \
+    "ds_read_b128 v[132:135], v156 offset:14336\n\t" \
+    "s_add_u32 m0, m0, 1024\n\t" \
+    "s_nop 0\n\t" \
+    "global_load_lds_dwordx4 %[io3], s[36:37]\n\t" \
+    "s_waitcnt vmcnt(4)\n\t" \
+    "v_fma_f32 v12, v140, v44, v12\n\t" \
+    "v_fma_f32 v13, v140, v45, v13\n\t" \
+    "v_mfma_f32_16x16x32_f16 v[72:75], v[120:123], a[24:27], 0\n\t" \
+    "v_fma_f32 v14, v140, v46, v14\n\t" \
+    "v_fma_f32 v15, v140, v47, v15\n\t" \
+    "s_waitcnt lgkmcnt(2)\n\t" \
+    "v_mfma_f32_16x16x32_f16 v[60:63], v[108:111], a[20:23], v[60:63]\n\t" \
+    "ds_read_b128 v[136:139], v156 offset:15360\n\t" \
+    "global_load_dwordx4 v[148:151], %[po], s[40:41]\n\t" \
+    "global_load_dwordx4 v[152:155], %[po], s[40:41] offset:256\n\t" \
+    "v_fma_f32 v16, v144, v48, v16\n\t" \
+    "v_mfma_f32_16x16x32_f16 v[64:67], v[108:111], a[28:31], v[64:67]\n\t" \
+    "s_add_u32 s64, s40, s58\n\t" \
+    "s_addc_u32 s65, s41, 0\n\t" \
+    "v_fma_f32 v17, v144, v49, v17\n\t" \
+    "v_fma_f32 v18, v144, v50, v18\n\t" \
+    "s_waitcnt lgkmcnt(2)\n\t" \
+    "v_mfma_f32_16x16x32_f16 v[68:71], v[112:115], a[20:23], v[68:71]\n\t" \
+    "v_fma_f32 v19, v144, v51, v19\n\t" \
+    "v_mfma_f32_16x16x32_f16 v[72:75], v[112:115], a[28:31], v[72:75]\n\t" \
+    "v_fma_f32 v20, v140, v52, v20\n\t" \
+    "v_fma_f32 v21, v140, v53, v21\n\t" \
+    "v_mfma_f32_16x16x32_f16 v[60:63], v[108:111], a[16:19], v[60:63]\n\t" \
+    "ds_read_b128 v[124:127], v156 offset:12288\n\t" \
+    "v_fma_f32 v22, v140, v54, v22\n\t" \
+    "v_mfma_f32_16x16x32_f16 v[64:67], v[108:111], a[24:27], v[64:67]\n\t" \
+    "v_fma_f32 v23, v140, v55, v23\n\t" \
+    "v_fma_f32 v24, v144, v56, v24\n\t" \
+    "v_mfma_f32_16x16x32_f16 v[68:71], v[112:115], a[16:19], v[68:71]\n\t" \
+    "ds_read_b128 v[128:131], v156 offset:13312\n\t" \
+    "v_fma_f32 v25, v144, v57, v25\n\t" \
+    "v_mfma_f32_16x16x32_f16 v[72:75], v[112:115], a[24:27], v[72:75]\n\t" \
+    "v_fma_f32 v26, v144, v58, v26\n\t" \
+    "v_fma_f32 v27, v144, v59, v27\n\t" \
+    "s_waitcnt lgkmcnt(3)\n\t" \
+    "v_mfma_f32_16x16x32_f16 v[60:63], v[132:135], a[0:3], v[60:63]\n\t" \
+    "v_fma_f32 v28, v141, v44, v28\n\t" \
+    "v_mfma_f32_16x16x32_f16 v[64:67], v[132:135], a[8:11], v[64:67]\n\t" \
+    "v_fma_f32 v29, v141, v45, v29\n\t" \
+    "v_fma_f32 v30, v141, v46, v30\n\t" \
+    "s_waitcnt lgkmcnt(2)\n\t" \
+    "v_mfma_f32_16x16x32_f16 v[68:71], v[136:139], a[0:3], v[68:71]\n\t" \
+    "ds_read_b128 v[84:87], v157 offset:2048\n\t" \
+    "v_fma_f32 v31, v141, v47, v31\n\t" \
+    "v_mfma_f32_16x16x32_f16 v[72:75], v[136:139], a[8:11], v[72:75]\n\t" \
+    "v_fma_f32 v32, v145, v48, v32\n\t" \
+    "v_fma_f32 v33, v145, v49, v33\n\t" \
+    "s_waitcnt lgkmcnt(2)\n\t" \
+    "v_mfma_f32_16x16x32_f16 v[60:63], v[124:127], a[4:7], v[60:63]\n\t" \
+    "ds_read_b128 v[88:91], v157 offset:3072\n\t" \
+    "v_fma_f32 v34, v145, v50, v34\n\t" \
+    "v_mfma_f32_16x16x32_f16 v[64:67], v[124:127], a[12:15], v[64:67]\n\t" \
+    "v_fma_f32 v35, v145, v51, v35\n\t" \
+    "v_fma_f32 v36, v141, v52, v36\n\t" \
+    "s_waitcnt lgkmcnt(2)\n\t" \
+    "v_mfma_f32_16x16x32_f16 v[68:71], v[128:131], a[4:7], v[68:71]\n\t" \
+    "v_fma_f32 v37, v141, v53, v37\n\t" \
+    "v_mfma_f32_16x16x32_f16 v[72:75], v[128:131], a[12:15], v[72:75]\n\t" \
+    "v_fma_f32 v38, v141, v54, v38\n\t" \
+    "v_fma_f32 v39, v141, v55, v39\n\t" \
+    "v_mfma_f32_16x16x32_f16 v[60:63], v[124:127], a[0:3], v[60:63]\n\t" \
+    "ds_read_b128 v[76:79], v157 offset:0\n\t" \
+    "v_fma_f32 v40, v145, v56, v40\n\t" \
+    "v_mfma_f32_16x16x32_f16 v[64:67], v[124:127], a[8:11], v[64:67]\n\t" \
+    "v_fma_f32 v41, v145, v57, v41\n\t" \
+    "v_fma_f32 v42, v145, v58, v42\n\t" \
+    "v_mfma_f32_16x16x32_f16 v[68:71], v[128:131], a[0:3], v[68:71]\n\t" \
+    "ds_read_b128 v[80:83], v157 offset:1024\n\t" \
+    "v_fma_f32 v43, v145, v59, v43\n\t" \
+    "s_mov_b32 s50, s45\n\t" \
+    "s_mov_b32 s45, s46\n\t" \
+    "s_mov_b32 s46, s72\n\t" \
+    "v_mfma_f32_16x16x32_f16 v[72:75], v[128:131], a[8:11], v[72:75]\n\t" \
+    "s_mov_b32 s72, s47\n\t" \
+    "s_mov_b32 s47, s50\n\t" \
+    "v_add_u32 v158, s45, %[lane16]\n\t" \
+    "v_add_u32 v159, s46, %[lane16]\n\t" \
+    "s_barrier\n\t" \
+    "s_sub_u32 s42, s42, 1\n\t" \
+    "s_cmp_eq_u32 s42, 0\n\t" \
+    "s_cbranch_scc1 2f\n\t" \
+    "s_waitcnt lgkmcnt(3)\n\t" \
+    "v_mfma_f32_16x16x32_f16 v[44:47], v[84:87], a[0:3], 0\n\t" \
+    "s_min_u32 s50, s43, s44\n\t" \
+    "s_mul_i32 s51, s50, 16384\n\t" \
+    "s_add_u32 s60, s52, s51\n\t" \
+    "v_mfma_f32_16x16x32_f16 v[48:51], v[84:87], a[8:11], 0\n\t" \
+    "s_addc_u32 s61, s53, 0\n\t" \
+    "s_add_u32 s43, s43, 1\n\t" \
+    "s_waitcnt lgkmcnt(2)\n\t" \
+    "v_mfma_f32_16x16x32_f16 v[52:55], v[88:91], a[0:3], 0\n\t" \
+    "ds_read_b128 v[100:103], v158 offset:6144\n\t" \
+    "s_add_u32 m0, s47, s74\n\t" \
+    "s_nop 0\n\t" \
+    "global_load_lds_dwordx4 %[io0], s[60:61]\n\t" \
+    "v_fma_f32 v12, -v141, v60, v12\n\t" \
+    "v_fma_f32 v13, -v141, v61, v13\n\t" \
+    "v_mfma_f32_16x16x32_f16 v[56:59], v[88:91], a[8:11], 0\n\t" \
+    "v_fma_f32 v14, -v141, v62, v14\n\t" \
+    "v_fma_f32 v15, -v141, v63, v15\n\t" \
+    "s_waitcnt lgkmcnt(2)\n\t" \
+    "v_mfma_f32_16x16x32_f16 v[44:47], v[76:79], a[4:7], v[44:47]\n\t" \
+    "ds_read_b128 v[104:107], v158 offset:7168\n\t" \
+    "v_fma_f32 v16, -v145, v64, v16\n\t" \
+    "v_mfma_f32_16x16x32_f16 v[48:51], v[76:79], a[12:15], v[48:51]\n\t" \
+    "v_fma_f32 v17, -v145, v65, v17\n\t" \
+    "v_fma_f32 v18, -v145, v66, v18\n\t" \
+    "s_waitcnt lgkmcnt(2)\n\t" \
+    "v_mfma_f32_16x16x32_f16 v[52:55], v[80:83], a[4:7], v[52:55]\n\t" \
+    "v_fma_f32 v19, -v145, v67, v19\n\t" \
+    "v_mfma_f32_16x16x32_f16 v[56:59], v[80:83], a[12:15], v[56:59]\n\t" \
+    "v_fma_f32 v20, -v141, v68, v20\n\t" \
+    "v_fma_f32 v21, -v141, v69, v21\n\t" \
+    "v_mfma_f32_16x16x32_f16 v[44:47], v[76:79], a[0:3], v[44:47]\n\t" \
+    "ds_read_b128 v[92:95], v158 offset:4096\n\t" \
+    "v_fma_f32 v22, -v141, v70, v22\n\t" \
+    "v_mfma_f32_16x16x32_f16 v[48:51], v[76:79], a[8:11], v[48:51]\n\t" \
+    "v_fma_f32 v23, -v141, v71, v23\n\t" \
+    "v_fma_f32 v24, -v145, v72, v24\n\t" \
+    "v_mfma_f32_16x16x32_f16 v[52:55], v[80:83], a[0:3], v[52:55]\n\t" \
+    "ds_read_b128 v[96:99], v158 offset:5120\n\t" \
+    "s_add_u32 m0, m0, 1024\n\t" \
+    "s_nop 0\n\t" \
+    "global_load_lds_dwordx4 %[io1], s[60:61]\n\t" \
+    "v_fma_f32 v25, -v145, v73, v25\n\t" \
+    "v_mfma_f32_16x16x32_f16 v[56:59], v[80:83], a[8:11], v[56:59]\n\t" \
+    "v_fma_f32 v26, -v145, v74, v26\n\t" \
+    "v_fma_f32 v27, -v145, v75, v27\n\t" \
+    "s_waitcnt lgkmcnt(3)\n\t" \
+    "v_mfma_f32_16x16x32_f16 v[44:47], v[100:103], a[16:19], v[44:47]\n\t" \
+    "v_fma_f32 v28, v140, v60, v28\n\t" \
+    "v_mfma_f32_16x16x32_f16 v[48:51], v[100:103], a[24:27], v[48:51]\n\t" \
+    "v_fma_f32 v29, v140, v61, v29\n\t" \
+    "v_fma_f32 v30, v140, v62, v30\n\t" \
+    "s_waitcnt lgkmcnt(2)\n\t" \
+    "v_mfma_f32_16x16x32_f16 v[52:55], v[104:107], a[16:19], v[52:55]\n\t" \
+    "ds_read_b128 v[116:119], v158 offset:10240\n\t" \
+    "v_fma_f32 v31, v140, v63, v31\n\t" \
+    "v_mfma_f32_16x16x32_f16 v[56:59], v[104:107], a[24:27], v[56:59]\n\t" \
+    "v_fma_f32 v32, v144, v64, v32\n\t" \
+    "v_fma_f32 v33, v144, v65, v33\n\t" \
+    "s_waitcnt lgkmcnt(2)\n\t" \
+    "v_mfma_f32_16x16x32_f16 v[44:47], v[92:95], a[20:23], v[44:47]\n\t" \
+    "ds_read_b128 v[120:123], v158 offset:11264\n\t" \
+    "v_fma_f32 v34, v144, v66, v34\n\t" \
+    "v_mfma_f32_16x16x32_f16 v[48:51], v[92:95], a[28:31], v[48:51]\n\t" \
+    "v_fma_f32 v35, v144, v67, v35\n\t" \
+    "v_fma_f32 v36, v140, v68, v36\n\t" \
+    "s_waitcnt lgkmcnt(2)\n\t" \
+    "v_mfma_f32_16x16x32_f16 v[52:55], v[96:99], a[20:23], v[52:55]\n\t" \
+    "s_add_u32 m0, m0, 1024\n\t" \
+    "s_nop 0\n\t" \
+    "global_load_lds_dwordx4 %[io2], s[60:61]\n\t" \
+    "v_fma_f32 v37, v140, v69, v37\n\t" \
+    "v_mfma_f32_16x16x32_f16 v[56:59], v[96:99], a[28:31], v[56:59]\n\t" \
+    "v_fma_f32 v38, v140, v70, v38\n\t" \
+    "v_fma_f32 v39, v140, v71, v39\n\t" \
+    "v_mfma_f32_16x16x32_f16 v[44:47], v[92:95], a[16:19], v[44:47]\n\t" \
+    "ds_read_b128 v[108:111], v158 offset:8192\n\t" \
+    "v_fma_f32 v40, v144, v72, v40\n\t" \
+    "v_mfma_f32_16x16x32_f16 v[48:51], v[92:95], a[24:27], v[48:51]\n\t" \
+    "v_fma_f32 v41, v144, v73, v41\n\t" \
+    "v_fma_f32 v42, v144, v74, v42\n\t" \
+    "v_mfma_f32_16x16x32_f16 v[52:55], v[96:99], a[16:19], v[52:55]\n\t" \
+    "ds_read_b128 v[112:115], v158 offset:9216\n\t" \
+    "v_fma_f32 v43, v144, v75, v43\n\t" \
+    "v_mfma_f32_16x16x32_f16 v[56:59], v[96:99], a[24:27], v[56:59]\n\t" \
+    "s_waitcnt lgkmcnt(3)\n\t" \
+    "v_mfma_f32_16x16x32_f16 v[60:63], v[116:119], a[16:19], 0\n\t" \
+    "v_mfma_f32_16x16x32_f16 v[64:67], v[116:119], a[24:27], 0\n\t" \
+    "s_waitcnt lgkmcnt(2)\n\t" \
+    "v_mfma_f32_16x16x32_f16 v[68:71], v[120:123], a[16:19], 0\n\t" \
+    "ds_read_b128 v[132:135], v158 offset:14336\n\t" \
+    "s_add_u32 m0, m0, 1024\n\t" \
+    "s_nop 0\n\t" \
+    "global_load_lds_dwordx4 %[io3], s[60:61]\n\t" \
+    "s_waitcnt vmcnt(4)\n\t" \
+    "v_fma_f32 v12, v148, v44, v12\n\t" \
+    "v_fma_f32 v13, v148, v45, v13\n\t" \
+    "v_mfma_f32_16x16x32_f16 v[72:75], v[120:123], a[24:27], 0\n\t" \
+    "v_fma_f32 v14, v148, v46, v14\n\t" \
+    "v_fma_f32 v15, v148, v47, v15\n\t" \
+    "s_waitcnt lgkmcnt(2)\n\t" \
+    "v_mfma_f32_16x16x32_f16 v[60:63], v[108:111], a[20:23], v[60:63]\n\t" \
+    "ds_read_b128 v[136:139], v158 offset:15360\n\t" \
+    "global_load_dwordx4 v[140:143], %[po], s[64:65]\n\t" \
+    "global_load_dwordx4 v[144:147], %[po], s[64:65] offset:256\n\t" \
+    "v_fma_f32 v16, v152, v48, v16\n\t" \
+    "v_mfma_f32_16x16x32_f16 v[64:67], v[108:111], a[28:31], v[64:67]\n\t" \
+    "s_add_u32 s40, s64, s58\n\t" \
+    "s_addc_u32 s41, s65, 0\n\t" \
+    "v_fma_f32 v17, v152, v49, v17\n\t" \
+    "v_fma_f32 v18, v152, v50, v18\n\t" \
+    "s_waitcnt lgkmcnt(2)\n\t" \
+    "v_mfma_f32_16x16x32_f16 v[68:71], v[112:115], a[20:23], v[68:71]\n\t" \
+    "v_fma_f32 v19, v152, v51, v19\n\t" \
+    "v_mfma_f32_16x16x32_f16 v[72:75], v[112:115], a[28:31], v[72:75]\n\t" \
+    "v_fma_f32 v20, v148, v52, v20\n\t" \
+    "v_fma_f32 v21, v148, v53, v21\n\t" \
+    "v_mfma_f32_16x16x32_f16 v[60:63], v[108:111], a[16:19], v[60:63]\n\t" \
+    "ds_read_b128 v[124:127], v158 offset:12288\n\t" \
+    "v_fma_f32 v22, v148, v54, v22\n\t" \
+    "v_mfma_f32_16x16x32_f16 v[64:67], v[108:111], a[24:27], v[64:67]\n\t" \
+    "v_fma_f32 v23, v148, v55, v23\n\t" \
+    "v_fma_f32 v24, v152, v56, v24\n\t" \
+    "v_mfma_f32_16x16x32_f16 v[68:71], v[112:115], a[16:19], v[68:71]\n\t" \
+    "ds_read_b128 v[128:131], v158 offset:13312\n\t" \
+    "v_fma_f32 v25, v152, v57, v25\n\t" \
+    "v_mfma_f32_16x16x32_f16 v[72:75], v[112:115], a[24:27], v[72:75]\n\t" \
+    "v_fma_f32 v26, v152, v58, v26\n\t" \
+    "v_fma_f32 v27, v152, v59, v27\n\t" \
+    "s_waitcnt lgkmcnt(3)\n\t" \
+    "v_mfma_f32_16x16x32_f16 v[60:63], v[132:135], a[0:3], v[60:63]\n\t" \
+    "v_fma_f32 v28, v149, v44, v28\n\t" \
+    "v_mfma_f32_16x16x32_f16 v[64:67], v[132:135], a[8:11], v[64:67]\n\t" \
+    "v_fma_f32 v29, v149, v45, v29\n\t" \
+    "v_fma_f32 v30, v149, v46, v30\n\t" \
+    "s_waitcnt lgkmcnt(2)\n\t" \
+    "v_mfma_f32_16x16x32_f16 v[68:71], v[136:139], a[0:3], v[68:71]\n\t" \
+    "ds_read_b128 v[84:87], v159 offset:2048\n\t" \
+    "v_fma_f32 v31, v149, v47, v31\n\t" \
+    "v_mfma_f32_16x16x32_f16 v[72:75], v[136:139], a[8:11], v[72:75]\n\t" \
+    "v_fma_f32 v32, v153, v48, v32\n\t" \
+    "v_fma_f32 v33, v153, v49, v33\n\t" \
+    "s_waitcnt lgkmcnt(2)\n\t" \
+    "v_mfma_f32_16x16x32_f16 v[60:63], v[124:127], a[4:7], v[60:63]\n\t" \
+    "ds_read_b128 v[88:91], v159 offset:3072\n\t" \
+    "v_fma_f32 v34, v153, v50, v34\n\t" \
+    "v_mfma_f32_16x16x32_f16 v[64:67], v[124:127], a[12:15], v[64:67]\n\t" \
+    "v_fma_f32 v35, v153, v51, v35\n\t" \
+    "v_fma_f32 v36, v149, v52, v36\n\t" \
+    "s_waitcnt lgkmcnt(2)\n\t" \
+    "v_mfma_f32_16x16x32_f16 v[68:71], v[128:131], a[4:7], v[68:71]\n\t" \
+    "v_fma_f32 v37, v149, v53, v37\n\t" \
+    "v_mfma_f32_16x16x32_f16 v[72:75], v[128:131], a[12:15], v[72:75]\n\t" \
+    "v_fma_f32 v38, v149, v54, v38\n\t" \
+    "v_fma_f32 v39, v149, v55, v39\n\t" \
+    "v_mfma_f32_16x16x32_f16 v[60:63], v[124:127], a[0:3], v[60:63]\n\t" \
+    "ds_read_b128 v[76:79], v159 offset:0\n\t" \
+    "v_fma_f32 v40, v153, v56, v40\n\t" \
+    "v_mfma_f32_16x16x32_f16 v[64:67], v[124:127], a[8:11], v[64:67]\n\t" \
+    "v_fma_f32 v41, v153, v57, v41\n\t" \
+    "v_fma_f32 v42, v153, v58, v42\n\t" \
+    "v_mfma_f32_16x16x32_f16 v[68:71], v[128:131], a[0:3], v[68:71]\n\t" \
+    "ds_read_b128 v[80:83], v159 offset:1024\n\t" \
+    "v_fma_f32 v43, v153, v59, v43\n\t" \
+    "s_mov_b32 s50, s45\n\t" \
+    "s_mov_b32 s45, s46\n\t" \
+    "s_mov_b32 s46, s72\n\t" \
+    "v_mfma_f32_16x16x32_f16 v[72:75], v[128:131], a[8:11], v[72:75]\n\t" \
+    "s_mov_b32 s72, s47\n\t" \
+    "s_mov_b32 s47, s50\n\t" \
+    "v_add_u32 v156, s45, %[lane16]\n\t" \
+    "v_add_u32 v157, s46, %[lane16]\n\t" \
+    "s_barrier\n\t" \
+    "s_sub_u32 s42, s42, 1\n\t" \
+    "s_cmp_lg_u32 s42, 0\n\t" \
+    "s_cbranch_scc1 1b\n\t" \
+    "s_waitcnt vmcnt(0)\n\t" \
+    "s_nop 15\n\t" \
+    "s_nop 15\n\t" \
+    "v_fma_f32 v12, -v149, v60, v12\n\t" \
+    "v_fma_f32 v13, -v149, v61, v13\n\t" \
+    "v_fma_f32 v14, -v149, v62, v14\n\t" \
+    "v_fma_f32 v15, -v149, v63, v15\n\t" \
+    "v_fma_f32 v16, -v153, v64, v16\n\t" \
+    "v_fma_f32 v17, -v153, v65, v17\n\t" \
+    "v_fma_f32 v18, -v153, v66, v18\n\t" \
+    "v_fma_f32 v19, -v153, v67, v19\n\t" \
+    "v_fma_f32 v20, -v149, v68, v20\n\t" \
+    "v_fma_f32 v21, -v149, v69, v21\n\t" \
+    "v_fma_f32 v22, -v149, v70, v22\n\t" \
+    "v_fma_f32 v23, -v149, v71, v23\n\t" \
+    "v_fma_f32 v24, -v153, v72, v24\n\t" \
+    "v_fma_f32 v25, -v153, v73, v25\n\t" \
+    "v_fma_f32 v26, -v153, v74, v26\n\t" \
+    "v_fma_f32 v27, -v153, v75, v27\n\t" \
+    "v_fma_f32 v28, v148, v60, v28\n\t" \
+    "v_fma_f32 v29, v148, v61, v29\n\t" \
+    "v_fma_f32 v30, v148, v62, v30\n\t" \
+    "v_fma_f32 v31, v148, v63, v31\n\t" \
+    "v_fma_f32 v32, v152, v64, v32\n\t" \
+    "v_fma_f32 v33, v152, v65, v33\n\t" \
+    "v_fma_f32 v34, v152, v66, v34\n\t" \
+    "v_fma_f32 v35, v152, v67, v35\n\t" \
+    "v_fma_f32 v36, v148, v68, v36\n\t" \
+    "v_fma_f32 v37, v148, v69, v37\n\t" \
+    "v_fma_f32 v38, v148, v70, v38\n\t" \
+    "v_fma_f32 v39, v148, v71, v39\n\t" \
+    "v_fma_f32 v40, v152, v72, v40\n\t" \
+    "v_fma_f32 v41, v152, v73, v41\n\t" \
+    "v_fma_f32 v42, v152, v74, v42\n\t" \
+    "v_fma_f32 v43, v152, v75, v43\n\t" \
+    "s_branch 3f\n\t" \
+    "2:\n\t" \
+    "s_waitcnt vmcnt(0)\n\t" \
+    "s_nop 15\n\t" \
+    "s_nop 15\n\t" \
+    "v_fma_f32 v12, -v141, v60, v12\n\t" \
+    "v_fma_f32 v13, -v141, v61, v13\n\t" \
+    "v_fma_f32 v14, -v141, v62, v14\n\t" \
+    "v_fma_f32 v15, -v141, v63, v15\n\t" \
+    "v_fma_f32 v16, -v145, v64, v16\n\t" \
+    "v_fma_f32 v17, -v145, v65, v17\n\t" \
+    "v_fma_f32 v18, -v145, v66, v18\n\t" \
+    "v_fma_f32 v19, -v145, v67, v19\n\t" \
+    "v_fma_f32 v20, -v141, v68, v20\n\t" \
+    "v_fma_f32 v21, -v141, v69, v21\n\t" \
+    "v_fma_f32 v22, -v141, v70, v22\n\t" \
+    "v_fma_f32 v23, -v141, v71, v23\n\t" \
+    "v_fma_f32 v24, -v145, v72, v24\n\t" \
+    "v_fma_f32 v25, -v145, v73, v25\n\t" \
+    "v_fma_f32 v26, -v145, v74, v26\n\t" \
+    "v_fma_f32 v27, -v145, v75, v27\n\t" \
+    "v_fma_f32 v28, v140, v60, v28\n\t" \
+    "v_fma_f32 v29, v140, v61, v29\n\t" \
+    "v_fma_f32 v30, v140, v62, v30\n\t" \
+    "v_fma_f32 v31, v140, v63, v31\n\t" \
+    "v_fma_f32 v32, v144, v64, v32\n\t" \
+    "v_fma_f32 v33, v144, v65, v33\n\t" \
+    "v_fma_f32 v34, v144, v66, v34\n\t" \
+    "v_fma_f32 v35, v144, v67, v35\n\t" \
+    "v_fma_f32 v36, v140, v68, v36\n\t" \
+    "v_fma_f32 v37, v140, v69, v37\n\t" \
+    "v_fma_f32 v38, v140, v70, v38\n\t" \
+    "v_fma_f32 v39, v140, v71, v39\n\t" \
+    "v_fma_f32 v40, v144, v72, v40\n\t" \
+    "v_fma_f32 v41, v144, v73, v41\n\t" \
+    "v_fma_f32 v42, v144, v74, v42\n\t" \
+    "v_fma_f32 v43, v144, v75, v43\n\t" \
+    "3:\n\t" \
+    "s_barrier\n\t" \
+    "ds_write_b128 %[accaddr], v[12:15] offset:0\n\t" \
+    "ds_write_b128 %[accaddr], v[16:19] offset:1024\n\t" \
+    "ds_write_b128 %[accaddr], v[20:23] offset:2048\n\t" \
+    "ds_write_b128 %[accaddr], v[24:27] offset:3072\n\t" \
+    "ds_write_b128 %[accaddr], v[28:31] offset:4096\n\t" \
+    "ds_write_b128 %[accaddr], v[32:35] offset:5120\n\t" \
+    "ds_write_b128 %[accaddr], v[36:39] offset:6144\n\t" \
+    "ds_write_b128 %[accaddr], v[40:43] offset:7168\n\t" \
+    "s_waitcnt lgkmcnt(0)\n\t" \
+    "s_mov_b32 m0, s73\n\t" \
+    ""
+#define GSDR_MFMA_RING16P4F_CLOBBERS \
+    "v12", "v13", "v14", "v15", "v16", "v17", "v18", "v19", "v20", "v21", "v22", "v23", \
+    "v24", "v25", "v26", "v27", "v28", "v29", "v30", "v31", "v32", "v33", "v34", "v35", \
+    "v36", "v37", "v38", "v39", "v40", "v41", "v42", "v43", "v44", "v45", "v46", "v47", \
+    "v48", "v49", "v50", "v51", "v52", "v53", "v54", "v55", "v56", "v57", "v58", "v59", \
+    "v60", "v61", "v62", "v63", "v64", "v65", "v66", "v67", "v68", "v69", "v70", "v71", \
+    "v72", "v73", "v74", "v75", "v76", "v77", "v78", "v79", "v80", "v81", "v82", "v83", \
+    "v84", "v85", "v86", "v87", "v88", "v89", "v90", "v91", "v92", "v93", "v94", "v95", \
+    "v96", "v97", "v98", "v99", "v100", "v101", "v102", "v103", "v104", "v105", "v106", "v107", \
+    "v108", "v109", "v110", "v111", "v112", "v113", "v114", "v115", "v116", "v117", "v118", "v119", \
+    "v120", "v121", "v122", "v123", "v124", "v125", "v126", "v127", "v128", "v129", "v130", "v131", \
+    "v132", "v133", "v134", "v135", "v136", "v137", "v138", "v139", "v140", "v141", "v142", "v143", \
+    "v144", "v145", "v146", "v147", "v148", "v149", "v150", "v151", "v152", "v153", "v154", "v155", \
+    "v156", "v157", "v158", "v159", "a0", "a1", "a2", "a3", "a4", "a5", "a6", "a7", \
+    "a8", "a9", "a10", "a11", "a12", "a13", "a14", "a15", "a16", "a17", "a18", "a19", \
+    "a20", "a21", "a22", "a23", "a24", "a25", "a26", "a27", "a28", "a29", "a30", "a31", \
+    "s36", "s37", "s38", "s39", "s40", "s41", "s42", "s43", "s44", "s45", "s46", "s47", \
+    "s48", "s49", "s50", "s51", "s52", "s53", "s54", "s55", "s56", "s57", "s58", "s59", \
+    "s60", "s61", "s62", "s63", "s64", "s65", "s66", "s67", "s68", "s69", "s70", "s71", \
+    "s72", "s73", "s74", "s75", "s76", "s77", "s78", "s79", "vcc", "scc", "memory"
diff --git a/gpu_sdr_amd/csrc/demod.cpp b/gpu_sdr_amd/csrc/demod.cpp
--- a/gpu_sdr_amd/csrc/demod.cpp
+++ b/gpu_sdr_amd/csrc/demod.cpp
@@ -70,6 +70,7 @@
     s.mfma_3m = env("GSDR_MFMA_3M", -1);
     s.mfma_3m_rot = env("GSDR_MFMA_3M_ROT", -1);
     s.mfma_fold = env("GSDR_MFMA_FOLD", -1);
+    s.mfma_fold_products = env("GSDR_MFMA_FOLD_PRODUCTS", -1);
     s.mfma_timing = env("GSDR_MFMA_TIMING", 0);
     s.noise_fft = env("GSDR_NOISE_FFT", 1) != 0;
     s.tones_fft = env("GSDR_TONES_FFT", 1) != 0;
@@ -155,6 +156,7 @@
     bool mac3 = false;
     bool rot2 = false;
     bool fold = false;
+    int fold_products = 0;
     gsdr::DevBuf<uint4> d_bfrag3;
     gsdr::DevBuf<float4> d_ptab3;
     gsdr::DevBuf<uint4> d_bfrag;
@@ -391,6 +393,13 @@
     return rot2 && (h->sw.mfma_fold == 1 || (h->sw.mfma_fold < 0 && nhi >= kFoldMinBlocks));
 }
 
+constexpr int kFoldProductsDefault = 4;
+int fold_products_chosen(const gsdr_demod *h, bool fold) {
+    if (!fold) return 0;
+    const int p = h->sw.mfma_fold_products;
+    return p == 3 || p == 4 ? p : kFoldProductsDefault;
+}
+
 int setup_mfma(gsdr_demod *h, bool direct, const std::vector<long long> &tone) {
     const int F = h->F, M = h->M;
     const unsigned rate = h->nco_rate;
@@ -480,10 +489,13 @@
         h->mac3 = want && mac3;
         h->rot2 = rot2_chosen(h, h->mac3, nhi);
         h->fold = fold_chosen(h, h->rot2, nhi);
+        h->fold_products = fold_products_chosen(h, h->fold);
         if (h->mac3) {
             std::vector<uint4> bfrag3;
             std::vector<float4> ptab3;
-            if (h->fold)
+            if (h->fold_products == 4)
+                gsdr::mfma_build_tables4f(pl, fmod, bfrag3, ptab3);
+            else if (h->fold)
                 gsdr::mfma_build_tables3f(pl, fmod, bfrag3, ptab3);
             else
                 gsdr::mfma_build_tables3(pl, h->rot2 ? 2 : 1, fmod, bfrag3, ptab3);
@@ -677,7 +689,7 @@
     if (record_begin(h, st, &stop)) return -1;
     gsdr::MfmaKernel kind = h->mf_kind;
     if (h->mac3) {
-        kind = h->fold ? gsdr::MfmaKernel::AsmRing16P3F
+        kind = h->fold ? (h->fold_products == 4 ? gsdr::MfmaKernel::AsmRing16P4F : gsdr::MfmaKernel::AsmRing16P3F)
                        : (h->rot2 ? gsdr::MfmaKernel::AsmRing16P3R2 : gsdr::MfmaKernel::AsmRing16P3);
         a.img = h->d_img[hs];
         a.bfrag3 = h->d_bfrag3;
@@ -1727,6 +1739,7 @@
     s += ", \"rotation_min_blocks\": " + std::to_string(kRot2MinBlocks);
     s += ", \"fold\": " + std::to_string(h->mfma && h->mac3 && h->rot2 && h->fold ? 1 : 0);
     s += ", \"fold_min_blocks\": " + std::to_string(kFoldMinBlocks);
+    s += ", \"fold_products\": " + std::to_string(h->mfma && h->mac3 && h->rot2 && h->fold ? h->fold_products : 0);
     s += ", \"pipeline_streams\": " + std::to_string(h->sw.pipe_streams);
     s += ", \"frame_average\": " + std::to_string(h->avg_k);
     s += std::string(", \"frame_average_kind\": \"") + (h->avg_kind == GSDR_AVERAGE_POWER ? "power" : "complex") + "\"";
```

New measurement: 12870 (median of 6 runs). 1.08x the previous value.
